# may-/joeys2t

Measured on AMD Instinct MI355X. Metric: audio frames/sec (train step, 80-mel, 15 s utt, bs32 per GPU), higher is better.
Workload: dtype bf16; 1 GPU; configs/librispeech_100h.yaml ASR train step on synthetic 16 kHz waveforms; global_batch=32, frames_per_utt=1498, encoder_len=375, lengths=fixed 15 s, vocab=5000, batch_multiplier=1, parallelism=dp1, launch=hipGraph replay

## Files before the change

include/joeys2t_hip.h:

```cpp
#ifndef JOEYS2T_HIP_H
#define JOEYS2T_HIP_H

#include <stdint.h>

#ifdef __cplusplus
extern "C" {
#endif

typedef void* js2t_stream;

enum { JS2T_F32 = 0, JS2T_BF16 = 1, JS2T_FP8_E4M3 = 2  };
enum { JS2T_ACT_NONE = 0, JS2T_ACT_RELU = 1, JS2T_ACT_GELU = 2, JS2T_ACT_SWISH = 3, JS2T_ACT_TANH = 4, JS2T_ACT_HARDSWISH = 5 };
enum { JS2T_OK = 0, JS2T_ERR_INVALID = -1, JS2T_ERR_LAUNCH = -2, JS2T_ERR_UNSUPPORTED = -3 };

int js2t_abi_version(void);
const char* js2t_last_error(void);

typedef struct js2t_gemm_desc {
  int32_t M, N, K;
  int32_t batch, batch_inner;
  int32_t dtype_ab, dtype_c;
  int32_t trans_a, trans_b;
  const void* A; int64_t lda, a_stride_o, a_stride_i;
  const void* B; int64_t ldb, b_stride_o, b_stride_i;
  void* C;       int64_t ldc, c_stride_o, c_stride_i;
  float alpha;
  const float* alpha_dev;
  const float* bias;
  int32_t act;
  void* preact;
  float dropout_p;
  const uint64_t* rng_state;
  uint32_t rng_stream;
  const void* residual;
  int64_t ldr;
  float res_scale;
  const void* gate;
  int64_t ldg;
  float gate_scale;
  float beta;
  int32_t conv, conv_tin, conv_tout, conv_c, conv_stride, conv_pad;
  int32_t split_k;
  float* a_rowsum;
  const float* ln_partial;
  float ln_eps;
  float* ln_mean;
  float* ln_rstd;
  float* rs_partial;
  uint8_t* c8;
  int64_t ldc8;
  float* c8_state;
  const float* c8_mul;
  float* c8_scale_out;
  float* fp8_state;
  const void* dot_src;
  int64_t ld_dot;
  float* dot_partial;
  float* sumsq_partial;
} js2t_gemm_desc;

int js2t_gemm(const js2t_gemm_desc* d, js2t_stream stream);
#define JS2T_GEMM_GROUP_MAX 32
int js2t_gemm_grouped(const js2t_gemm_desc* d, int32_t count, const void* const* A, const void* const* B, void* const* C,
                      float* const* a_rowsum, js2t_stream stream);
int64_t js2t_gemm_grouped_blocks(int32_t M, int32_t N, int32_t count);
void js2t_gemm_force_regstage(int on);
void js2t_gemm_force_w256(int on);
void js2t_gemm_p192_mode(int mode);
void js2t_gemm_wg256_mode(int mode);
void js2t_gemm_p192_ring(int nst);
void js2t_gemm_panel_mode(int mode);


int js2t_axpby(const void* x, float a, const void* y, float b, void* out, int64_t n, int dt, js2t_stream stream);

int js2t_cast(const void* src, int src_dt, void* dst, int dst_dt, int64_t n, js2t_stream stream);

int js2t_fold_ln_weights(const int64_t* table, int32_t n_entries, int32_t max_rows, js2t_stream stream);

int js2t_absmax(const void* x, int dt, int64_t n, float* out, js2t_stream stream);
int js2t_quantize_fp8(const void* x, int dt, void* y, int64_t n, const float* amax, const float* mul, float* scale_out,
                      js2t_stream stream);
int js2t_quantize_fp8_delayed(const void* x, int dt, void* y, int64_t n, float* state, const float* mul, float* scale_out,
                              js2t_stream stream);

int js2t_glu_fwd(const void* x, void* y, int64_t rows, int64_t C, int dt, js2t_stream stream);
int js2t_glu_bwd(const void* x, const void* dy, void* dx, int64_t rows, int64_t C, int dt, js2t_stream stream);
int js2t_glu_fwd_crop(const void* x, void* y, int64_t rows, int64_t C, int64_t T, const int64_t* valid_t, int dt, js2t_stream stream);
int js2t_glu_bwd_crop(const void* x, const void* dy, void* dx, int64_t rows, int64_t C, int64_t T, const int64_t* valid_t, int dt,
                      js2t_stream stream);

int js2t_transpose_groups(const void* src, void* dst, const int64_t* table, int32_t n_groups, int64_t total_tiles, js2t_stream stream);

int js2t_add_pe_dropout(const void* x, const float* pe, const void* extra, void* y, int64_t B, int64_t T,
                        int64_t D, int dt, float p, const uint64_t* rng_state, uint32_t rng_stream,
                        js2t_stream stream);

int js2t_dropout_bwd(const void* dy, void* dx, int64_t rows, int64_t cols, int dt, float p,
                     const uint64_t* rng_state, uint32_t rng_stream, js2t_stream stream);

int js2t_act_bwd(const void* dh, const void* z, void* dz, int64_t n, int act, int dt, float scale,
                 js2t_stream stream);

int js2t_embed_fwd(const int64_t* ids, const void* table, int table_dt, void* out, int out_dt,
                   int64_t n_ids, int64_t D, int64_t vocab, float scale, js2t_stream stream);
int js2t_embed_bwd(const int64_t* ids, const void* dout, int dout_dt, float* dtable, int64_t n_ids,
                   int64_t D, int64_t vocab, float scale, int64_t pad_idx, js2t_stream stream);

int64_t js2t_colsum_partial_rows(int64_t rows);
int js2t_colsum(const void* x, int dt, float* out, float* partial, int64_t rows, int64_t cols, int accumulate,
                js2t_stream stream);

int js2t_pack_rows(const void* src, void* dst, const int32_t* seg, int32_t B, int32_t T, int64_t rows_out, int64_t row_bytes,
                   int pack, js2t_stream stream);

int js2t_conv_weight_pack(const float* w, void* wp, int wp_dt, int64_t cout, int64_t cin, int64_t k,
                          js2t_stream stream);
int js2t_conv_weight_unpack_grad(const float* dwp_t, float* dw, int64_t cout, int64_t cin, int64_t k,
                                 int accumulate, js2t_stream stream);
int js2t_im2col(const void* x, void* col, int64_t B, int64_t tin, int64_t tout, int64_t C, int64_t K,
                int64_t stride, int64_t pad, int dt, js2t_stream stream);
int js2t_col2im(const void* dcol, void* dx, int64_t B, int64_t tin, int64_t tout, int64_t C, int64_t K,
                int64_t stride, int64_t pad, int dt, js2t_stream stream);

int js2t_subsample_lengths_mask(const int64_t* lengths, int64_t* out_lengths, uint8_t* mask, int64_t B,
                                int64_t T_out, const int32_t* kernel_sizes, int32_t n_layers,
                                js2t_stream stream);

int js2t_layernorm_fwd(const void* x, const float* gamma, const float* beta, void* y, float* mean,
                       float* rstd, int64_t rows, int64_t D, float eps, int dt, js2t_stream stream);
int js2t_layernorm_fwd_fp8(const void* x, const float* gamma, const float* beta, void* y, void* y8, float* q_state,
                           const float* q_mul, float* q_scale_out, float* mean, float* rstd, int64_t rows, int64_t D, float eps,
                           int dt, js2t_stream stream);
int js2t_layernorm_bwd(const void* dy, const void* x, const float* gamma, const float* mean,
                       const float* rstd, void* dx, const void* add, float add_scale, float* dgamma,
                       float* dbeta, float* partial, int accumulate, int64_t rows, int64_t D, int dt,
                       js2t_stream stream);
int js2t_layernorm_bwd_dropout(const void* dy, const void* x, const float* gamma, const float* mean,
                               const float* rstd, void* dx, const void* add, float add_scale, float* dgamma,
                               float* dbeta, float* partial, int accumulate, int64_t rows, int64_t D, int dt,
                               void* dx_dropped, float drop_p, const uint64_t* rng_state, uint32_t rng_stream,
                               int32_t acc_copies, int64_t acc_copy_stride, js2t_stream stream);
int js2t_layernorm_bwd_fused(const void* dy, const void* x, const float* gamma, const float* mean,
                             const float* rstd, void* dx, const void* add, float add_scale, float* dgamma,
                             float* dbeta, float* partial, int accumulate, int64_t rows, int64_t D, int dt,
                             void* dx_dropped, float drop_p, const uint64_t* rng_state, uint32_t rng_stream,
                             int32_t acc_copies, int64_t acc_copy_stride, const float* beta, void* n_out, js2t_stream stream);
int js2t_fold_copies(float* ws, const int64_t* table, int32_t n_entries, int32_t copies, int64_t copy_stride,
                     js2t_stream stream);

int js2t_softmax_fwd(const void* S, const uint8_t* mask, void* P, void* Pd, int64_t B, int64_t H,
                     int64_t Tq, int64_t Tk, int64_t ld, int64_t mask_sb, int64_t mask_sq, int dt,
                     float p, const uint64_t* rng_state, uint32_t rng_stream, js2t_stream stream);
int js2t_softmax_bwd(const void* P, const void* dPd, void* dS, int64_t Z, int64_t Tq, int64_t Tk,
                     int64_t ld, int dt, float p, const uint64_t* rng_state, uint32_t rng_stream,
                     js2t_stream stream);
int js2t_attn_head_mean(const void* P, float* out, int64_t B, int64_t H, int64_t Tq, int64_t Tk,
                        int64_t ld, int dt, js2t_stream stream);

int js2t_rel_bias_add(void* S, const float* rel_bias, int64_t B, int64_t H, int64_t Tq, int64_t Tk, int64_t ld, int32_t R,
                      int dt, js2t_stream stream);
int js2t_rel_bias_grad(const void* dS, float* d_rel_bias, int64_t B, int64_t H, int64_t Tq, int64_t Tk, int64_t ld, int32_t R,
                       int dt, js2t_stream stream);


int js2t_row_lse(const void* x, float* lse, int64_t* argmax, int64_t rows, int64_t V, int dt, js2t_stream stream);

int js2t_ctc_collapse(const int64_t* best, const int64_t* in_len, int64_t* out_ids, int64_t* out_len, int64_t B,
                      int64_t T, int64_t blank, int64_t pad, js2t_stream stream);
int js2t_log_softmax(const void* x, int dt, void* y, int y_dt, int64_t rows, int64_t V, js2t_stream stream);

int js2t_xent_fwd(const void* logits, int dt, const int64_t* trg, float* loss_rows, float* correct_rows,
                  float* lse, int64_t rows, int64_t V, int64_t pad_idx, float smoothing, js2t_stream stream);
int js2t_xent_bwd(const void* logits, int dt, const int64_t* trg, const float* lse, const float* g_dev,
                  float scale, void* dlogits, int64_t rows, int64_t V, int64_t pad_idx, float smoothing,
                  js2t_stream stream);
int js2t_xent_bwd_as(const void* logits, int dt, const int64_t* trg, const float* lse, const float* g_dev, float scale,
                     void* dlogits, int out_dt, int64_t rows, int64_t V, int64_t pad_idx, float smoothing, js2t_stream stream);

int js2t_train_stats(double* stats6, const float* total, const float* nll, const float* ctc, const int64_t* n_correct,
                     double inv_norm, double nseqs, double ntokens, float* norm_out, js2t_stream stream);

int js2t_sum_f32(const float* x, int64_t n, float* out, js2t_stream stream);

int js2t_ctc_alpha(const void* logits, int dt, const float* lse, const int64_t* targets, const int64_t* in_len,
                   const int64_t* tgt_len, float* alpha, float* beta, float* nll, float* loss_rows, int64_t B, int64_t T,
                   int64_t V, int64_t Lmax, int64_t blank, int zero_infinity, const int32_t* row_offsets, js2t_stream stream);
int js2t_ctc_bwd(const void* logits, int dt, const float* lse, const int64_t* targets, const int64_t* in_len,
                 const int64_t* tgt_len, const float* alpha, float* beta, const float* nll, const float* g_dev,
                 float scale, void* dlogits, int64_t B, int64_t T, int64_t V, int64_t Lmax, int64_t blank,
                 int zero_infinity, int beta_ready, const int32_t* row_offsets, int64_t packed_rows, js2t_stream stream);

int js2t_attn_decode(const void* q, int64_t ldq, const void* k, const void* v, int64_t ldkv, const int32_t* idx, int32_t idx_ld,
                     int32_t Tmax, int32_t len, const int32_t* len_dev, const uint8_t* key_mask, void* out, int64_t ldo, int32_t rows,
                     int32_t H, int32_t dh, float scale, int32_t group, int dt, js2t_stream stream);

int js2t_dwconv_outer_fwd(const void* x, const float* w, const float* bias, void* y, int64_t L, int64_t N, int64_t C, int K, int dt,
                          js2t_stream stream);
int js2t_dwconv_outer_bwd(const void* dy, const void* x, const float* w, void* dx, float* dw, int64_t L, int64_t N, int64_t C, int K,
                          int dt, js2t_stream stream);
int js2t_bn_act_fwd(const void* x, const float* gamma, const float* beta, float* running_mean, float* running_var, float* mean,
                    float* invstd, void* y, float* ws, int64_t rows, int64_t C, float eps, float momentum, int train, int act, int dt,
                    js2t_stream stream);
int js2t_bn_act_bwd(const void* dy, const void* x, const float* gamma, const float* beta, const float* mean, const float* invstd,
                    void* dx, float* dgamma, float* dbeta, float* ws, int64_t rows, int64_t C, int train, int act, int dt,
                    js2t_stream stream);


int js2t_fbank(const float* wave, const int64_t* sample_off, const int64_t* frame_off, int32_t U,
               int64_t total_frames, const float* window, const float* tw_re, const float* tw_im,
               const int32_t* mel_start, const int32_t* mel_len, const int32_t* mel_woff, const float* mel_w,
               float* out, int32_t win_len, int32_t shift, int32_t n_fft, int32_t n_mel, float scale, float preemph,
               float log_floor, js2t_stream stream);

int js2t_cmvn_stats(const float* feat, const int64_t* frame_off, int32_t U, int32_t F, float* mean, float* istd,
                    float* fill, int32_t norm_means, int32_t norm_vars, int64_t max_frames, js2t_stream stream);
int64_t js2t_cmvn_stats_workspace(int32_t U, int32_t F);
int js2t_cmvn_stats_ws(const float* feat, const int64_t* frame_off, int32_t U, int32_t F, float* mean, float* istd, float* fill,
                       int32_t norm_means, int32_t norm_vars, int64_t max_frames, double* workspace, js2t_stream stream);

int js2t_feature_finalize(const float* feat, const int64_t* frame_off, const float* mean, const float* istd,
                          const float* fill, const int32_t* masks, void* out, int out_dt, int64_t U, int64_t Tmax,
                          int32_t F, float pad_value, js2t_stream stream);
int js2t_feature_finalize_crop(const float* feat, const int64_t* frame_off, const float* mean, const float* istd,
                               const float* fill, const int32_t* masks, void* out, int out_dt, int64_t U, int64_t Tmax,
                               int32_t F, float pad_value, const int64_t* crop_t, js2t_stream stream);

int js2t_feature_transform(float* feat, const int64_t* frame_off, int32_t U, int32_t F, const float* mean, const float* istd,
                           const float* fill, const int32_t* masks, int32_t n_freq, int32_t n_time, js2t_stream stream);

typedef struct js2t_ctx_s* js2t_ctx;
enum {
  JS2T_CTX_DETERMINISTIC = 0,
  JS2T_CTX_GEMM_P192_MODE = 1,
  JS2T_CTX_GEMM_P192_RING = 2,
  JS2T_CTX_GEMM_WG256_MODE = 3,
  JS2T_CTX_GEMM_PANEL_MODE = 4,
  JS2T_CTX_NKEYS = 5
};
js2t_ctx js2t_ctx_create(void);
void js2t_ctx_destroy(js2t_ctx ctx);
int js2t_ctx_set(js2t_ctx ctx, int32_t key, int32_t value);
int js2t_ctx_get(js2t_ctx ctx, int32_t key);
js2t_ctx js2t_ctx_bind(js2t_ctx ctx);
int js2t_ctx_effective(int32_t key);
void js2t_set_deterministic(int on);
int js2t_get_deterministic(void);


int64_t js2t_sumsq_partials(int64_t n);
int js2t_grad_norm_clip(const float* g, int64_t n, float max_norm, float* partial, float* out2, js2t_stream stream);
int js2t_sumsq_ranges(const float* g, const int64_t* table, int32_t n_ranges, int64_t n_blocks, float* partial, js2t_stream stream);
int js2t_norm_clip(const float* partial, int64_t n_partial, float max_norm, float* out2, js2t_stream stream);

int js2t_adamw(float* p, float* g, float* exp_avg, float* exp_avg_sq, void* lp_bf16, int64_t n, float lr,
               float beta1, float beta2, float eps, float weight_decay, int64_t step, const float* gscale_dev,
               float gscale, int zero_grad, const float* lr_dev, const int64_t* step_dev, js2t_stream stream);

int js2t_adamw_items(float* p, float* g, float* exp_avg, float* exp_avg_sq, void* lp_bf16, void* lp_t_bf16,
                     const int64_t* items, int32_t n_items, int64_t n_units, const int64_t* folds, float lr, float beta1,
                     float beta2, float eps, float weight_decay, int64_t step, const float* gscale_dev, float gscale,
                     int zero_grad, const float* lr_dev, const int64_t* step_dev, js2t_stream stream);
void js2t_adamw_items_geometry(int32_t* flat_unit, int32_t* rows, int32_t* cols);

int js2t_beam_step(const float* logits, const float* beam_log_probs, float* out_scores, int64_t* out_ids,
                   float* out_lse, int64_t n_batch, int32_t beam, int64_t V, const int32_t* forbid_ids,
// ... 59 lines not shown
```

joeys2t_amd/builders.py:

```python
from typing import Callable

from torch import nn


class ConfigurationError(Exception):
    """Custom exception for misspecifications of configuration (reference config.py:22)."""


class _Tanh(nn.Module):
    def forward(self, x):
        raise RuntimeError("placeholder activation module: the HIP GEMM epilogue applies tanh")


_ACTIVATIONS = {"relu": nn.ReLU, "gelu": nn.GELU, "tanh": _Tanh, "swish": nn.SiLU}


def build_activation(activation: str = "relu") -> Callable:
    try:
        return _ACTIVATIONS[activation]
    except KeyError:
        raise ConfigurationError("Invalid activation function. Valid options: " + ", ".join(repr(k) for k in _ACTIVATIONS) + ".") from None


import ctypes as _C
# ... 23 lines not shown

def _off(t, lo: int):
    return None if t is None else _C.c_void_p(t.data_ptr() + lo * t.element_size())


import os as _os

FUSED_UPDATE = _os.environ.get("JS2T_FUSED_UPDATE", "1") != "0"


class SumsqCollector:

    def __init__(self, grad: torch.Tensor, total: int):
        from joeys2t_amd._lib import lib
        self.grad, self.total = grad, total
        self.per_block = int(total // max(1, lib().js2t_sumsq_partials(_C.c_int64(total)))) or 1
        cap = 2 * int(lib().js2t_sumsq_partials(_C.c_int64(total))) + 8192
        self.partial = torch.zeros((cap, ), dtype=torch.float32, device=grad.device)
        self.pos, self.covered = 0, []
        self._tables: Dict[tuple, tuple] = {}

    def reset(self):
        self.pos, self.covered = 0, []

    def segment(self, n_blocks: int, spans):
        if self.pos + n_blocks > self.partial.numel():
            raise RuntimeError("SumsqCollector: partial buffer exhausted")
        seg = self.partial[self.pos:self.pos + n_blocks]
        self.pos += n_blocks
        self.covered.extend(spans)
        return seg

    def finish(self, max_norm: float, out2: torch.Tensor):
        from joeys2t_amd import ops
        from joeys2t_amd._lib import check, lib
        from joeys2t_amd.runtime import RangeSet
        key = (self.pos, tuple(sorted(self.covered)))
        hit = self._tables.get(key)
        if hit is None:
            if torch.cuda.is_current_stream_capturing():
                raise RuntimeError("SumsqCollector: a new coverage pattern during capture - run one eager step first")
            rest = RangeSet([(0, self.total)]).minus(self.covered)
            rows, pb = [], self.pos
            for lo, hi in rest:
                rows.append([lo, hi - lo, pb])
                pb += int(lib().js2t_sumsq_partials(_C.c_int64(hi - lo)))
            if pb > self.partial.numel():
                raise RuntimeError("SumsqCollector: partial buffer exhausted")
            table = torch.tensor(rows, dtype=torch.int64, device=self.grad.device) if rows else None
            hit = self._tables[key] = (table, len(rows), pb - self.pos, pb)
        table, n_ranges, n_blocks, n_partial = hit
        if n_ranges:
            check(lib().js2t_sumsq_ranges(ops._p(self.grad), ops._p(table), _C.c_int32(n_ranges), _C.c_int64(n_blocks), ops._p(self.partial),
                                          ops._stream()), "js2t_sumsq_ranges")
        check(lib().js2t_norm_clip(ops._p(self.partial), _C.c_int64(n_partial), _C.c_float(max_norm), ops._p(out2), ops._stream()),
              "js2t_norm_clip")
        self.reset()


class FlatAdamW:

    def __init__(self, store, lr: float = 3e-4, betas=(0.9, 0.999), eps: float = 1e-8, weight_decay: float = 0.0):
        self.store = store
        self.param_groups = [{"lr": float(lr), "betas": tuple(betas), "eps": float(eps), "weight_decay": float(weight_decay)}]
        self.exp_avg = torch.zeros_like(store.flat)
        self.exp_avg_sq = torch.zeros_like(store.flat)
        self.t = 0
        self._retired_plans = []
        self.plan_generation = 0
        from joeys2t_amd._lib import lib
        n = store.total
        self._partial = torch.empty((max(1, lib().js2t_sumsq_partials(_C.c_int64(n))), ), dtype=torch.float32,
                                    device=store.device)
        self.norm_clip = torch.ones((2, ), dtype=torch.float32, device=store.device)
        self.lr_dev = torch.full((1, ), float(lr), dtype=torch.float32, device=store.device)
        self.step_dev = torch.zeros((1, ), dtype=torch.int64, device=store.device)
        self.device_schedule = False
        self.update_ranges = trainable_ranges(store)
        self._plan_key, self._plan = None, None
        self.keep = None
        self.collector: Optional[SumsqCollector] = None


    def clip_and_step(self, max_norm: Optional[float], grad_scale: float = 1.0, zero_grad: bool = True):
        from joeys2t_amd import ops
        from joeys2t_amd._lib import check, lib
        st, g = self.store, self.param_groups[0]
        coef = None
        if max_norm is not None and max_norm > 0:
            if self.collector is not None and self.collector.covered:
                self.collector.finish(max_norm, self.norm_clip)
            else:
                check(lib().js2t_grad_norm_clip(ops._p(st.flat_grad), _C.c_int64(st.total), _C.c_float(max_norm),
                                                ops._p(self._partial), ops._p(self.norm_clip), ops._stream()), "js2t_grad_norm_clip")
            coef = self.norm_clip[1:2]
        if self.collector is not None:
            self.collector.reset()
        self.t += 1
        lp = st.flat_lp
        lr_dev = step_dev = None
        if self.device_schedule:
            self.step_dev.add_(1)
            lr_dev, step_dev = self.lr_dev, self.step_dev
        plan = self._fused_plan()
        if plan is not None:
            args = (_C.c_float(g["lr"]), _C.c_float(g["betas"][0]), _C.c_float(g["betas"][1]), _C.c_float(g["eps"]),
                    _C.c_float(g["weight_decay"]), _C.c_int64(self.t), ops._p(coef), _C.c_float(grad_scale), int(zero_grad),
                    ops._p(lr_dev), ops._p(step_dev), ops._stream())
            for table, n_items, n_units in plan["launches"]:
                check(lib().js2t_adamw_items(ops._p(st.flat), ops._p(st.flat_grad), ops._p(self.exp_avg), ops._p(self.exp_avg_sq),
                                             ops._p(lp), ops._p(st.flat_lp_t if lp is not None else None), ops._p(table),
                                             _C.c_int32(n_items), _C.c_int64(n_units), ops._p(plan["folds"]), *args), "js2t_adamw_items")
            ops.WEIGHT_VERSION += 1
            st.dirty = lp is None and st.dirty
            if plan["left_folds"] is not None:
                ops.fold_ln_weights(plan["left_folds"], plan["left_folds"].shape[0], plan["left_max_rows"])
            return
        for lo, hi in self.update_ranges:
            check(lib().js2t_adamw(_off(st.flat, lo), _off(st.flat_grad, lo), _off(self.exp_avg, lo), _off(self.exp_avg_sq, lo),
                                   _off(lp, lo), _C.c_int64(hi - lo), _C.c_float(g["lr"]), _C.c_float(g["betas"][0]),
                                   _C.c_float(g["betas"][1]), _C.c_float(g["eps"]), _C.c_float(g["weight_decay"]), _C.c_int64(self.t),
                                   ops._p(coef), _C.c_float(grad_scale), int(zero_grad), ops._p(lr_dev), ops._p(step_dev),
                                   ops._stream()), "js2t_adamw")
        ops.WEIGHT_VERSION += 1
        st.dirty = lp is None and st.dirty
        if lp is not None and st.flat_lp_t is not None:
            st.refresh_t()
        if lp is not None:
            st.refresh_folds()

    def _fused_plan(self):
        st = self.store
        if not FUSED_UPDATE or self.update_ranges != [(0, st.total)]:
            return None
        key = (len(st._fold_rows), st.flat_lp is not None, st.flat_lp_t is not None, None if self.keep is None else self.keep.version)
        if self._plan_key == key:
            return self._plan
        if torch.cuda.is_current_stream_capturing():
            raise RuntimeError("FlatAdamW: the store changed (new LayerNorm folds / shadows) after the last eager update: "
                               "run one eager step before capturing")
        if self._plan is not None:
            self._retired_plans.append(self._plan)
            self.plan_generation += 1
        self._plan_key, self._plan = key, None
        from joeys2t_amd._lib import lib
        geo = [_C.c_int32() for _ in range(3)]
        lib().js2t_adamw_items_geometry(*[_C.byref(v) for v in geo])
        flat_unit, unit_rows, unit_cols = (int(v.value) for v in geo)
        mats = sorted((off, R, Cc) for off, R, Cc, _ in st._tgroups)
        if any(Cc % 4 or off % 4 for off, R, Cc in mats):
            return None
        base = st.flat.data_ptr()
        fold_of, left = {}, []
        for i, row in enumerate(st._fold_rows):
            hit = [(off, R, Cc) for off, R, Cc in mats if base + 4 * off == row[0] and R == row[6] and Cc == row[7]]
            if hit and row[7] <= unit_cols and hit[0][0] not in fold_of:
                fold_of[hit[0][0]] = i
            else:
                left.append(row)
        small, big, pos = [], [], 0
        for off, R, Cc in mats:
            if off > pos:
                small.append([0, pos, off - pos, 1, 0, -1, 0, 0])
            kept = int(self.keep is not None and self.keep.contains(off, off + R * Cc))
            big.append([1, off, R, Cc, 0, fold_of.get(off, -1), kept, 0])
            pos = off + R * Cc
        if st.total > pos:
            small.append([0, pos, st.total - pos, 1, 0, -1, 0, 0])
        launches = []
        for items in (small, big):
            if not items:
                continue
            units = 0
            for it in items:
                it[4] = units
                units += -(-it[2] // flat_unit) if it[0] == 0 else -(-it[2] // unit_rows) * -(-it[3] // unit_cols)
            launches.append((torch.tensor(items, dtype=torch.int64, device=st.device), len(items), units))
        folds = torch.tensor(st._fold_rows, dtype=torch.int64, device=st.device) if st._fold_rows else None
        self._plan = {"launches": launches, "folds": folds,
                      "left_folds": torch.tensor(left, dtype=torch.int64, device=st.device) if left else None,
                      "left_max_rows": max((r[6] for r in left), default=0)}
        return self._plan

    def state_dict(self) -> Dict:
        return {"t": self.t, "exp_avg": self.exp_avg, "exp_avg_sq": self.exp_avg_sq, "param_groups": self.param_groups}
# ... 73 lines not shown
```

joeys2t_amd/csrc/elementwise.hip:

```cpp
#include "common.hpp"

namespace {

constexpr int EW_THREADS = 256;
inline int ew_grid(int64_t work_items) {
  int64_t g = (work_items + EW_THREADS - 1) / EW_THREADS;
  if (g < 1) g = 1;
  if (g > 4096) g = 4096;
  return (int)g;
}

template <typename T> struct vec4;
template <> struct vec4<float> {
  static __device__ __forceinline__ void ld(const float* p, float (&v)[4]) {
    const float4 x = *(const float4*)p; v[0] = x.x; v[1] = x.y; v[2] = x.z; v[3] = x.w;
  }
  static __device__ __forceinline__ void st(float* p, const float (&v)[4]) {
    *(float4*)p = make_float4(v[0], v[1], v[2], v[3]);
  }
};
template <> struct vec4<uint16_t> {
  static __device__ __forceinline__ void ld(const uint16_t* p, float (&v)[4]) {
    const uint2 x = *(const uint2*)p;
    v[0] = __uint_as_float(x.x << 16); v[1] = __uint_as_float(x.x & 0xffff0000u);
    v[2] = __uint_as_float(x.y << 16); v[3] = __uint_as_float(x.y & 0xffff0000u);
  }
  static __device__ __forceinline__ void st(uint16_t* p, const float (&v)[4]) {
    uint2 x;
    x.x = pack_bf16x2(v[0], v[1]);
    x.y = pack_bf16x2(v[2], v[3]);
    *(uint2*)p = x;
  }
};

template <typename S, typename D>
__global__ void cast_kernel(const S* __restrict__ src, D* __restrict__ dst, int64_t n) {
  const int64_t n4 = n >> 2;
  for (int64_t i = blockIdx.x * (int64_t)blockDim.x + threadIdx.x; i < n4; i += (int64_t)gridDim.x * blockDim.x) {
    float v[4];
    vec4<S>::ld(src + 4 * i, v);
    vec4<D>::st(dst + 4 * i, v);
  }
  for (int64_t i = (n4 << 2) + blockIdx.x * (int64_t)blockDim.x + threadIdx.x; i < n; i += (int64_t)gridDim.x * blockDim.x)
    io<D>::st(dst + i, io<S>::ld(src + i));
}

template <typename T>
__global__ void axpby_kernel(const T* __restrict__ x, float a, const T* __restrict__ y, float b, T* __restrict__ out,
                             int64_t n) {
  for (int64_t i = blockIdx.x * (int64_t)blockDim.x + threadIdx.x; i < n; i += (int64_t)gridDim.x * blockDim.x) {
    float v = a * io<T>::ld(x + i);
    if (y) v += b * io<T>::ld(y + i);
    io<T>::st(out + i, v);
  }
}

template <typename T>
__global__ void glu_fwd_kernel(const T* __restrict__ x, T* __restrict__ y, int64_t rows, int64_t C, int64_t T_,
                               const int64_t* __restrict__ valid_t) {
  const int64_t total = rows * C, vt = valid_t ? *valid_t : T_;
  for (int64_t i = blockIdx.x * (int64_t)blockDim.x + threadIdx.x; i < total; i += (int64_t)gridDim.x * blockDim.x) {
    const int64_t r = i / C, c = i - r * C;
    const float a = io<T>::ld(x + r * 2 * C + c), b = io<T>::ld(x + r * 2 * C + C + c);
    io<T>::st(y + i, (r % T_) < vt ? a / (1.f + __expf(-b)) : 0.f);
  }
}
template <typename T>
__global__ void glu_bwd_kernel(const T* __restrict__ x, const T* __restrict__ dy, T* __restrict__ dx, int64_t rows,
                               int64_t C, int64_t T_, const int64_t* __restrict__ valid_t) {
  const int64_t total = rows * C, vt = valid_t ? *valid_t : T_;
  for (int64_t i = blockIdx.x * (int64_t)blockDim.x + threadIdx.x; i < total; i += (int64_t)gridDim.x * blockDim.x) {
    const int64_t r = i / C, c = i - r * C;
    const float a = io<T>::ld(x + r * 2 * C + c), b = io<T>::ld(x + r * 2 * C + C + c);
    const float g = (r % T_) < vt ? io<T>::ld(dy + i) : 0.f;
    const float s = 1.f / (1.f + __expf(-b));
    io<T>::st(dx + r * 2 * C + c, g * s);
    io<T>::st(dx + r * 2 * C + C + c, g * a * s * (1.f - s));
  }
}

template <typename T>
__global__ void add_pe_dropout_kernel(const T* __restrict__ x, const float* __restrict__ pe, const T* __restrict__ extra,
                                      T* __restrict__ y, int64_t B, int64_t T_, int64_t D, float p,
                                      const uint64_t* rng, uint32_t stream) {
  const int64_t D4 = D >> 2, total = B * T_ * D4;
  const float sc = p > 0.f ? 1.f / (1.f - p) : 1.f;
  const uint32_t dkey = p > 0.f ? dropout_key(rng, stream) : 0u;
  for (int64_t i = blockIdx.x * (int64_t)blockDim.x + threadIdx.x; i < total; i += (int64_t)gridDim.x * blockDim.x) {
    const int64_t row = i / D4, c4 = i - row * D4, t = row % T_;
    float v[4], e[4];
    vec4<T>::ld(x + row * D + 4 * c4, v);
    if (pe) {
      const float4 pv = *(const float4*)(pe + t * D + 4 * c4);
      v[0] += pv.x; v[1] += pv.y; v[2] += pv.z; v[3] += pv.w;
    }
    if (extra) {
      vec4<T>::ld(extra + row * D + 4 * c4, e);
#pragma unroll
      for (int k = 0; k < 4; ++k) v[k] += e[k];
    }
    if (p > 0.f) {
      const uint32_t keep = dropout_keep4_key(dkey, (uint32_t)row, (uint32_t)c4, p);
#pragma unroll
      for (int k = 0; k < 4; ++k) v[k] = ((keep >> k) & 1u) ? v[k] * sc : 0.f;
    }
    vec4<T>::st(y + row * D + 4 * c4, v);
  }
}

template <typename T>
__global__ void dropout_bwd_kernel(const T* __restrict__ dy, T* __restrict__ dx, int64_t rows, int64_t cols, float p,
                                   const uint64_t* rng, uint32_t stream) {
  const int64_t c4n = (cols + 3) >> 2, total = rows * c4n;
  const float sc = 1.f / (1.f - p);
  const uint32_t dkey = dropout_key(rng, stream);
  for (int64_t i = blockIdx.x * (int64_t)blockDim.x + threadIdx.x; i < total; i += (int64_t)gridDim.x * blockDim.x) {
    const int64_t row = i / c4n, c4 = i - row * c4n;
    const uint32_t keep = dropout_keep4_key(dkey, (uint32_t)row, (uint32_t)c4, p);
#pragma unroll
    for (int k = 0; k < 4; ++k) {
      const int64_t c = 4 * c4 + k;
      if (c < cols) {
        const float g = io<T>::ld(dy + row * cols + c);
        io<T>::st(dx + row * cols + c, ((keep >> k) & 1u) ? g * sc : 0.f);
      }
    }
  }
}

template <typename T>
__global__ void act_bwd_kernel(const T* __restrict__ dh, const T* __restrict__ z, T* __restrict__ dz, int64_t n, int act,
                               float scale) {
  for (int64_t i = blockIdx.x * (int64_t)blockDim.x + threadIdx.x; i < n; i += (int64_t)gridDim.x * blockDim.x)
    io<T>::st(dz + i, io<T>::ld(dh + i) * act_grad(io<T>::ld(z + i), act) * scale);
}

template <typename TT, typename TO>
__global__ void embed_fwd_kernel(const int64_t* __restrict__ ids, const TT* __restrict__ table, TO* __restrict__ out,
                                 int64_t n_ids, int64_t D, int64_t vocab, float scale) {
  const int64_t total = n_ids * D;
  for (int64_t i = blockIdx.x * (int64_t)blockDim.x + threadIdx.x; i < total; i += (int64_t)gridDim.x * blockDim.x) {
    const int64_t r = i / D, c = i - r * D;
    const int64_t id = ids[r];
    const float v = (id >= 0 && id < vocab) ? io<TT>::ld(table + id * D + c) * scale : 0.f;
    io<TO>::st(out + i, v);
  }
}
template <typename T>
__global__ void embed_bwd_kernel(const int64_t* __restrict__ ids, const T* __restrict__ dout, float* __restrict__ dtable,
                                 int64_t n_ids, int64_t D, int64_t vocab, float scale, int64_t pad_idx) {
  const int64_t total = n_ids * D;
  for (int64_t i = blockIdx.x * (int64_t)blockDim.x + threadIdx.x; i < total; i += (int64_t)gridDim.x * blockDim.x) {
    const int64_t r = i / D, c = i - r * D;
    const int64_t id = ids[r];
    if (id < 0 || id >= vocab || id == pad_idx) continue;
    atomicAdd(dtable + id * D + c, scale * io<T>::ld(dout + i));
  }
}

template <typename T>
__global__ __launch_bounds__(256) void embed_bwd_ordered_kernel(const int64_t* __restrict__ ids, const T* __restrict__ dout,
                                                                float* __restrict__ dtable, int64_t n_ids, int64_t D, int64_t vocab,
                                                                float scale, int64_t pad_idx) {
  __shared__ int earlier;
  const int64_t r = blockIdx.x, id = ids[r];
  if (id < 0 || id >= vocab || id == pad_idx) return;
  if (threadIdx.x == 0) earlier = 0;
  __syncthreads();
  for (int64_t q = threadIdx.x; q < r; q += blockDim.x)
    if (ids[q] == id) earlier = 1;
  __syncthreads();
  if (earlier) return;
  for (int64_t c = threadIdx.x; c < D; c += blockDim.x) {
    float acc = dtable[id * D + c];
    for (int64_t q = r; q < n_ids; ++q)
      if (ids[q] == id) acc += scale * io<T>::ld(dout + q * D + c);
    dtable[id * D + c] = acc;
  }
}

constexpr int CS_ROWS_PER_BLOCK = 64;
template <typename T>
__global__ __launch_bounds__(256) void colsum_partial_kernel(const T* __restrict__ x, float* __restrict__ partial, int64_t rows,
                                                             int64_t cols) {
  __shared__ float sh[4][64];
  const int cl = threadIdx.x & 63, sub = threadIdx.x >> 6;
  const int64_t c = (int64_t)blockIdx.x * 64 + cl;
  const int64_t r0 = (int64_t)blockIdx.y * CS_ROWS_PER_BLOCK, r1 = min(rows, r0 + CS_ROWS_PER_BLOCK);
  float s = 0.f;
  if (c < cols)
    for (int64_t r = r0 + sub; r < r1; r += 4) s += io<T>::ld(x + r * cols + c);
  sh[sub][cl] = s;
  __syncthreads();
  if (sub == 0 && c < cols) partial[(int64_t)blockIdx.y * cols + c] = (sh[0][cl] + sh[1][cl]) + (sh[2][cl] + sh[3][cl]);
}
__global__ __launch_bounds__(256) void colsum_partial_vec_kernel(const uint16_t* __restrict__ x, float* __restrict__ partial,
                                                                 int64_t rows, int64_t cols) {
  __shared__ float sh[4][64][9];
  const int cl = threadIdx.x & 63, sub = threadIdx.x >> 6;
  const int64_t c = ((int64_t)blockIdx.x * 64 + cl) * 8;
  const int64_t r0 = (int64_t)blockIdx.y * CS_ROWS_PER_BLOCK, r1 = min(rows, r0 + CS_ROWS_PER_BLOCK);
  float s[8] = {0.f, 0.f, 0.f, 0.f, 0.f, 0.f, 0.f, 0.f};
  if (c < cols)
    for (int64_t r = r0 + sub; r < r1; r += 4) {
      const uint4 v = *(const uint4*)(x + r * cols + c);
      const uint32_t vv[4] = {v.x, v.y, v.z, v.w};
#pragma unroll
      for (int i = 0; i < 4; ++i) {
        s[2 * i] += __uint_as_float(vv[i] << 16);
        s[2 * i + 1] += __uint_as_float(vv[i] & 0xffff0000u);
      }
    }
#pragma unroll
  for (int i = 0; i < 8; ++i) sh[sub][cl][i] = s[i];
  __syncthreads();
  if (sub == 0 && c < cols) {
#pragma unroll
    for (int i = 0; i < 8; ++i)
      partial[(int64_t)blockIdx.y * cols + c + i] = (sh[0][cl][i] + sh[1][cl][i]) + (sh[2][cl][i] + sh[3][cl][i]);
  }
}
__global__ __launch_bounds__(256) void colsum_final_kernel(const float* __restrict__ partial, float* __restrict__ out, int64_t nparts,
                                                           int64_t cols, int accumulate) {
  __shared__ float sh[4][64];
  const int cl = threadIdx.x & 63, sub = threadIdx.x >> 6;
  const int64_t c = (int64_t)blockIdx.x * 64 + cl;
  float s0 = 0.f, s1 = 0.f;
  if (c < cols) {
    int64_t p = sub;
    for (; p + 4 < nparts; p += 8) {
      s0 += partial[p * cols + c];
      s1 += partial[(p + 4) * cols + c];
    }
    for (; p < nparts; p += 4) s0 += partial[p * cols + c];
  }
  sh[sub][cl] = s0 + s1;
  __syncthreads();
  if (sub == 0 && c < cols) {
    const float tot = (sh[0][cl] + sh[1][cl]) + (sh[2][cl] + sh[3][cl]);
    out[c] = accumulate ? out[c] + tot : tot;
  }
}

template <typename D>
__global__ void conv_pack_kernel(const float* __restrict__ w, D* __restrict__ wp, int64_t cout, int64_t cin, int64_t k) {
  const int64_t total = cout * cin * k;
  for (int64_t i = blockIdx.x * (int64_t)blockDim.x + threadIdx.x; i < total; i += (int64_t)gridDim.x * blockDim.x) {
    const int64_t o = i / (k * cin), rem = i - o * k * cin, kw = rem / cin, c = rem - kw * cin;
    io<D>::st(wp + i, w[(o * cin + c) * k + kw]);
  }
}
__global__ void conv_unpack_grad_kernel(const float* __restrict__ dwp_t, float* __restrict__ dw, int64_t cout, int64_t cin,
                                        int64_t k, int accumulate) {
  const int64_t total = cout * cin * k;
  for (int64_t i = blockIdx.x * (int64_t)blockDim.x + threadIdx.x; i < total; i += (int64_t)gridDim.x * blockDim.x) {
    const int64_t o = i / (cin * k), rem = i - o * cin * k, c = rem / k, kw = rem - c * k;
    const float v = dwp_t[(kw * cin + c) * cout + o];
    dw[i] = accumulate ? dw[i] + v : v;
  }
// ... 85 lines not shown
    if (table[mid * 4 + 3] <= bid) lo = mid; else hi = mid - 1;
  }
  const int64_t off = table[lo * 4], R = table[lo * 4 + 1], Cc = table[lo * 4 + 2], t0 = table[lo * 4 + 3];
  const int64_t tiles_c = (Cc + 63) >> 6;
  const int64_t tr = (bid - t0) / tiles_c, tc = (bid - t0) - tr * tiles_c;
  if (((R | Cc | off) & 7) == 0 && ((((uintptr_t)src) | ((uintptr_t)dst)) & 15) == 0) {
#pragma unroll
    for (int k = 0; k < 2; ++k) {
      const int o = threadIdx.x + 256 * k, r = o >> 3, c8 = (o & 7) << 3;
      const int64_t rr = tr * 64 + r, cc = tc * 64 + c8;
      if (rr < R && cc < Cc) {
        const uint4 q = *(const uint4*)(src + off + rr * Cc + cc);
        uint32_t* d = (uint32_t*)&tile[r][c8];
        d[0] = q.x, d[1] = q.y, d[2] = q.z, d[3] = q.w;
      }
    }
    __syncthreads();
#pragma unroll
    for (int k = 0; k < 2; ++k) {
      const int o = threadIdx.x + 256 * k, c = o >> 3, r8 = (o & 7) << 3;
      const int64_t cc = tc * 64 + c, rr = tr * 64 + r8;
      if (rr < R && cc < Cc) {
        uint32_t w[4];
#pragma unroll
        for (int j = 0; j < 4; ++j) w[j] = (uint32_t)tile[r8 + 2 * j][c] | ((uint32_t)tile[r8 + 2 * j + 1][c] << 16);
        *(uint4*)(dst + off + cc * R + rr) = make_uint4(w[0], w[1], w[2], w[3]);
      }
    }
    return;
  }
  const int tx = threadIdx.x & 63, ty = threadIdx.x >> 6;
  for (int r = ty; r < 64; r += 4) {
    const int64_t rr = tr * 64 + r, cc = tc * 64 + tx;
    if (rr < R && cc < Cc) tile[r][tx] = src[off + rr * Cc + cc];
  }
  __syncthreads();
  for (int c = ty; c < 64; c += 4) {
    const int64_t cc = tc * 64 + c, rr = tr * 64 + tx;
    if (rr < R && cc < Cc) dst[off + cc * R + rr] = tile[tx][c];
  }
}

}

#define DISPATCH_DT(dt, T, ...)                                  \
  do {                                                           \
    if ((dt) == JS2T_F32) { typedef float T; __VA_ARGS__; }      \
    else if ((dt) == JS2T_BF16) { typedef uint16_t T; __VA_ARGS__; } \
    else { js2t_set_error("bad dtype %d", (int)(dt)); return JS2T_ERR_INVALID; } \
  } while (0)

extern "C" int js2t_cast(const void* src, int src_dt, void* dst, int dst_dt, int64_t n, js2t_stream stream) {
  if (n == 0) return JS2T_OK;
  JS2T_CHECK(src && dst && n > 0, "cast: bad arguments");
  hipStream_t s = (hipStream_t)stream;
  const int g = ew_grid(n / 4 + 1);
  DISPATCH_DT(src_dt, S, DISPATCH_DT(dst_dt, D, hipLaunchKernelGGL((cast_kernel<S, D>), dim3(g), dim3(EW_THREADS), 0, s,
                                                                    (const S*)src, (D*)dst, n)));
  JS2T_LAUNCH_CHECK();
  return JS2T_OK;
}

extern "C" int js2t_axpby(const void* x, float a, const void* y, float b, void* out, int64_t n, int dt, js2t_stream stream) {
  if (n == 0) return JS2T_OK;
  JS2T_CHECK(x && out && n > 0, "axpby: bad arguments");
  DISPATCH_DT(dt, T, hipLaunchKernelGGL((axpby_kernel<T>), dim3(ew_grid(n)), dim3(EW_THREADS), 0, (hipStream_t)stream,
                                        (const T*)x, a, (const T*)y, b, (T*)out, n));
  JS2T_LAUNCH_CHECK();
  return JS2T_OK;
}

extern "C" int js2t_glu_fwd_crop(const void* x, void* y, int64_t rows, int64_t C, int64_t T_, const int64_t* valid_t, int dt,
                                 js2t_stream stream) {
  if (rows * C == 0) return JS2T_OK;
  JS2T_CHECK(x && y && rows > 0 && C > 0 && T_ > 0 && rows % T_ == 0, "glu_fwd: bad arguments");
  DISPATCH_DT(dt, T, hipLaunchKernelGGL((glu_fwd_kernel<T>), dim3(ew_grid(rows * C)), dim3(EW_THREADS), 0,
                                        (hipStream_t)stream, (const T*)x, (T*)y, rows, C, T_, valid_t));
  JS2T_LAUNCH_CHECK();
  return JS2T_OK;
}
extern "C" int js2t_glu_fwd(const void* x, void* y, int64_t rows, int64_t C, int dt, js2t_stream stream) {
  return js2t_glu_fwd_crop(x, y, rows, C, rows > 0 ? rows : 1, nullptr, dt, stream);
}
extern "C" int js2t_glu_bwd_crop(const void* x, const void* dy, void* dx, int64_t rows, int64_t C, int64_t T_, const int64_t* valid_t,
                                 int dt, js2t_stream stream) {
  if (rows * C == 0) return JS2T_OK;
  JS2T_CHECK(x && dy && dx && rows > 0 && C > 0 && T_ > 0 && rows % T_ == 0, "glu_bwd: bad arguments");
  DISPATCH_DT(dt, T, hipLaunchKernelGGL((glu_bwd_kernel<T>), dim3(ew_grid(rows * C)), dim3(EW_THREADS), 0,
                                        (hipStream_t)stream, (const T*)x, (const T*)dy, (T*)dx, rows, C, T_, valid_t));
  JS2T_LAUNCH_CHECK();
  return JS2T_OK;
}
extern "C" int js2t_glu_bwd(const void* x, const void* dy, void* dx, int64_t rows, int64_t C, int dt, js2t_stream stream) {
  return js2t_glu_bwd_crop(x, dy, dx, rows, C, rows > 0 ? rows : 1, nullptr, dt, stream);
}

extern "C" int js2t_add_pe_dropout(const void* x, const float* pe, const void* extra, void* y, int64_t B, int64_t T_,
                                   int64_t D, int dt, float p, const uint64_t* rng_state, uint32_t rng_stream,
                                   js2t_stream stream) {
  if (B * T_ * D == 0) return JS2T_OK;
  JS2T_CHECK(x && y, "add_pe_dropout: null pointer");
  JS2T_CHECK(D % 4 == 0, "add_pe_dropout: D must be a multiple of 4 (got %lld)", (long long)D);
  JS2T_CHECK(p >= 0.f && p < 1.f && (p == 0.f || rng_state), "add_pe_dropout: bad dropout arguments");
  DISPATCH_DT(dt, T, hipLaunchKernelGGL((add_pe_dropout_kernel<T>), dim3(ew_grid(B * T_ * D / 4)), dim3(EW_THREADS), 0,
                                        (hipStream_t)stream, (const T*)x, pe, (const T*)extra, (T*)y, B, T_, D, p,
                                        rng_state, rng_stream));
  JS2T_LAUNCH_CHECK();
  return JS2T_OK;
}

extern "C" int js2t_dropout_bwd(const void* dy, void* dx, int64_t rows, int64_t cols, int dt, float p,
                                const uint64_t* rng_state, uint32_t rng_stream, js2t_stream stream) {
  if (rows * cols == 0) return JS2T_OK;
  JS2T_CHECK(dy && dx && rng_state && p > 0.f && p < 1.f, "dropout_bwd: bad arguments");
  DISPATCH_DT(dt, T, hipLaunchKernelGGL((dropout_bwd_kernel<T>), dim3(ew_grid(rows * ((cols + 3) / 4))), dim3(EW_THREADS),
                                        0, (hipStream_t)stream, (const T*)dy, (T*)dx, rows, cols, p, rng_state, rng_stream));
  JS2T_LAUNCH_CHECK();
  return JS2T_OK;
}

extern "C" int js2t_act_bwd(const void* dh, const void* z, void* dz, int64_t n, int act, int dt, float scale,
                            js2t_stream stream) {
  if (n == 0) return JS2T_OK;
  JS2T_CHECK(dh && z && dz && n > 0, "act_bwd: bad arguments");
  DISPATCH_DT(dt, T, hipLaunchKernelGGL((act_bwd_kernel<T>), dim3(ew_grid(n)), dim3(EW_THREADS), 0, (hipStream_t)stream,
                                        (const T*)dh, (const T*)z, (T*)dz, n, act, scale));
  JS2T_LAUNCH_CHECK();
  return JS2T_OK;
}

extern "C" int js2t_embed_fwd(const int64_t* ids, const void* table, int table_dt, void* out, int out_dt, int64_t n_ids,
                              int64_t D, int64_t vocab, float scale, js2t_stream stream) {
  if (n_ids * D == 0) return JS2T_OK;
  JS2T_CHECK(ids && table && out, "embed_fwd: null pointer");
  DISPATCH_DT(table_dt, TT, DISPATCH_DT(out_dt, TO, hipLaunchKernelGGL((embed_fwd_kernel<TT, TO>), dim3(ew_grid(n_ids * D)),
                                                                       dim3(EW_THREADS), 0, (hipStream_t)stream, ids,
                                                                       (const TT*)table, (TO*)out, n_ids, D, vocab, scale)));
  JS2T_LAUNCH_CHECK();
  return JS2T_OK;
}
extern "C" int js2t_embed_bwd(const int64_t* ids, const void* dout, int dout_dt, float* dtable, int64_t n_ids, int64_t D,
                              int64_t vocab, float scale, int64_t pad_idx, js2t_stream stream) {
  if (n_ids * D == 0) return JS2T_OK;
  JS2T_CHECK(ids && dout && dtable, "embed_bwd: null pointer");
  if (g_js2t_deterministic) {
    DISPATCH_DT(dout_dt, T, hipLaunchKernelGGL((embed_bwd_ordered_kernel<T>), dim3((unsigned)n_ids), dim3(256), 0, (hipStream_t)stream, ids,
                                               (const T*)dout, dtable, n_ids, D, vocab, scale, pad_idx));
    JS2T_LAUNCH_CHECK();
    return JS2T_OK;
  }
  DISPATCH_DT(dout_dt, T, hipLaunchKernelGGL((embed_bwd_kernel<T>), dim3(ew_grid(n_ids * D)), dim3(EW_THREADS), 0,
                                             (hipStream_t)stream, ids, (const T*)dout, dtable, n_ids, D, vocab, scale, pad_idx));
  JS2T_LAUNCH_CHECK();
  return JS2T_OK;
}

extern "C" int64_t js2t_colsum_partial_rows(int64_t rows) { return (rows + CS_ROWS_PER_BLOCK - 1) / CS_ROWS_PER_BLOCK; }

extern "C" int js2t_colsum(const void* x, int dt, float* out, float* partial, int64_t rows, int64_t cols, int accumulate,
                           js2t_stream stream) {
  if (cols == 0) return JS2T_OK;
  if (rows == 0) {
    JS2T_CHECK(out, "colsum: bad arguments");
    if (!accumulate) {
      hipError_t e = hipMemsetAsync(out, 0, sizeof(float) * cols, (hipStream_t)stream);
      JS2T_CHECK(e == hipSuccess, "colsum: memset failed: %s", hipGetErrorString(e));
    }
    return JS2T_OK;
  }
  JS2T_CHECK(x && out && partial && rows > 0, "colsum: bad arguments");
  const int64_t nparts = js2t_colsum_partial_rows(rows);
  JS2T_CHECK(nparts <= 65535, "colsum: too many rows");
  hipStream_t s = (hipStream_t)stream;
  if (dt == JS2T_BF16 && cols % 8 == 0 && (((uintptr_t)x) & 15) == 0) {
    hipLaunchKernelGGL(colsum_partial_vec_kernel, dim3(cdiv(cols, 512), (unsigned)nparts), dim3(256), 0, s, (const uint16_t*)x,
                       partial, rows, cols);
  } else {
    const dim3 g1(cdiv(cols, 64), (unsigned)nparts);
    DISPATCH_DT(dt, T, hipLaunchKernelGGL((colsum_partial_kernel<T>), g1, dim3(256), 0, s, (const T*)x, partial, rows, cols));
  }
  JS2T_LAUNCH_CHECK();
  hipLaunchKernelGGL(colsum_final_kernel, dim3(cdiv(cols, 64)), dim3(256), 0, s, partial, out, nparts, cols, accumulate);
  JS2T_LAUNCH_CHECK();
  return JS2T_OK;
}

extern "C" int js2t_conv_weight_pack(const float* w, void* wp, int wp_dt, int64_t cout, int64_t cin, int64_t k,
                                     js2t_stream stream) {
  JS2T_CHECK(w && wp && cout > 0 && cin > 0 && k > 0, "conv_weight_pack: bad arguments");
  DISPATCH_DT(wp_dt, D, hipLaunchKernelGGL((conv_pack_kernel<D>), dim3(ew_grid(cout * cin * k)), dim3(EW_THREADS), 0,
                                           (hipStream_t)stream, w, (D*)wp, cout, cin, k));
  JS2T_LAUNCH_CHECK();
  return JS2T_OK;
}
extern "C" int js2t_conv_weight_unpack_grad(const float* dwp_t, float* dw, int64_t cout, int64_t cin, int64_t k,
                                            int accumulate, js2t_stream stream) {
  JS2T_CHECK(dwp_t && dw && cout > 0 && cin > 0 && k > 0, "conv_weight_unpack_grad: bad arguments");
  hipLaunchKernelGGL(conv_unpack_grad_kernel, dim3(ew_grid(cout * cin * k)), dim3(EW_THREADS), 0, (hipStream_t)stream, dwp_t,
                     dw, cout, cin, k, accumulate);
  JS2T_LAUNCH_CHECK();
  return JS2T_OK;
}
extern "C" int js2t_col2im(const void* dcol, void* dx, int64_t B, int64_t tin, int64_t tout, int64_t C, int64_t K,
                           int64_t stride, int64_t pad, int dt, js2t_stream stream) {
  if (B * tin * C == 0) return JS2T_OK;
  JS2T_CHECK(dcol && dx && stride > 0 && K > 0, "col2im: bad arguments");
  if (dt == JS2T_BF16 && (C & 7) == 0 && ((((uintptr_t)dcol) | ((uintptr_t)dx)) & 15) == 0) {
    hipLaunchKernelGGL(col2im_vec_kernel, dim3(ew_grid(B * tin * (C >> 3))), dim3(EW_THREADS), 0, (hipStream_t)stream,
                       (const uint16_t*)dcol, (uint16_t*)dx, B, tin, tout, C, K, stride, pad);
    JS2T_LAUNCH_CHECK();
    return JS2T_OK;
  }
  DISPATCH_DT(dt, T, hipLaunchKernelGGL((col2im_kernel<T>), dim3(ew_grid(B * tin * C)), dim3(EW_THREADS), 0,
                                        (hipStream_t)stream, (const T*)dcol, (T*)dx, B, tin, tout, C, K, stride, pad));
  JS2T_LAUNCH_CHECK();
  return JS2T_OK;
}

extern "C" int js2t_im2col(const void* x, void* col, int64_t B, int64_t tin, int64_t tout, int64_t C, int64_t K, int64_t stride,
                           int64_t pad, int dt, js2t_stream stream) {
  if (B * tout * C * K == 0) return JS2T_OK;
  JS2T_CHECK(x && col && stride > 0 && K > 0 && tin > 0, "im2col: bad arguments");
  JS2T_CHECK(dt == JS2T_F32 || dt == JS2T_BF16, "im2col: bad dtype");
  const int vec = dt == JS2T_BF16 ? 8 : 4;
  JS2T_CHECK(C % vec == 0 && ((((uintptr_t)x) | ((uintptr_t)col)) & 15) == 0, "im2col: channels must fill 16-byte pieces, buffers 16-byte aligned");
  const int64_t work = B * tout * K * (C / vec);
  if (dt == JS2T_BF16)
    hipLaunchKernelGGL((im2col_kernel<uint16_t, 8>), dim3(ew_grid(work)), dim3(EW_THREADS), 0, (hipStream_t)stream, (const uint16_t*)x,
                       (uint16_t*)col, B, tin, tout, C, K, stride, pad);
  else
    hipLaunchKernelGGL((im2col_kernel<float, 4>), dim3(ew_grid(work)), dim3(EW_THREADS), 0, (hipStream_t)stream, (const float*)x,
                       (float*)col, B, tin, tout, C, K, stride, pad);
  JS2T_LAUNCH_CHECK();
  return JS2T_OK;
}

namespace {
// ... 239 lines not shown
```

joeys2t_amd/csrc/loss.hip:

```cpp
#include "common.hpp"

namespace {

constexpr int LB = 256;

__device__ __forceinline__ float logaddexp(float a, float b) {
  if (a == -INFINITY) return b;
  if (b == -INFINITY) return a;
  const float m = fmaxf(a, b);
  return m + log1pf(__expf(-fabsf(a - b)));
}

__device__ __forceinline__ float logaddexp_fast(float a, float b) {
  const float m = fmaxf(a, b);
  const float d = -fabsf(a - b);
  const float r = m + __logf(1.f + __expf(d));
  return (m == -INFINITY) ? -INFINITY : r;
}

template <typename T>
__global__ __launch_bounds__(LB) void row_lse_kernel(const T* __restrict__ x, float* __restrict__ lse,
                                                     int64_t* __restrict__ argmax, int64_t rows, int64_t V) {
  __shared__ float red[LB / 64];
  __shared__ int redi[LB / 64];
// ... 185 lines not shown
  sx = wave_sum(sx);
  int cand = (m == bmx) ? mi : 0x7fffffff;
#pragma unroll
  for (int o = 32; o > 0; o >>= 1) cand = min(cand, __shfl_xor(cand, o, 64));
  if (lane == 0) {
    const int64_t g = trg[r];
    const float lse = bmx + __logf(s);
    lse_out[r] = lse;
    float loss = 0.f, ok = 0.f;
    if (g != pad && g >= 0 && g < V) {
      const float lpg = xr[g] - lse;
      if (eps > 0.f) {
        const float u = eps / (float)(V - 2);
        const float lpp = (pad >= 0 && pad < V) ? xr[pad] - lse : 0.f;
        const float sum_lp = sx - (float)V * lse;
        const float cent = (1.f - eps) * __logf(1.f - eps) + eps * __logf(u);
        loss = cent - ((1.f - eps) * lpg + u * (sum_lp - lpg - lpp));
      } else {
        loss = -lpg;
      }
      ok = (cand == (int)g) ? 1.f : 0.f;
    }
    loss_rows[r] = loss;
    correct_rows[r] = ok;
  }
}
template <typename TO>
__global__ __launch_bounds__(256) void xent_bwd_flat_kernel(const float* __restrict__ x, const int64_t* __restrict__ trg,
                                                            const float* __restrict__ lse, const float* __restrict__ g_dev, float scale,
                                                            TO* __restrict__ dx, int rows, int n8, int64_t V, int64_t pad, float eps) {
  const int64_t chunk = (int64_t)blockIdx.x * 256 + threadIdx.x;
  if (chunk >= (int64_t)rows * n8) return;
  const int r = (int)(chunk / n8), c = (int)(chunk - (int64_t)r * n8);
  const int64_t g = trg[r];
  const bool dead = g == pad || g < 0 || g >= V;
  float o[8] = {0.f, 0.f, 0.f, 0.f, 0.f, 0.f, 0.f, 0.f};
  if (!dead) {
    const float4 qa = ((const float4*)x)[2 * chunk], qb = ((const float4*)x)[2 * chunk + 1];
    const float gs = scale * (g_dev ? *g_dev : 1.f), l = lse[r];
    const float u = eps > 0.f ? eps / (float)(V - 2) : 0.f, tg = eps > 0.f ? 1.f - eps : 1.f;
    const float f[8] = {qa.x, qa.y, qa.z, qa.w, qb.x, qb.y, qb.z, qb.w};
    const int gi = (int)g - 8 * c, pi = (pad >= 0 && pad < V) ? (int)pad - 8 * c : -1;
#pragma unroll
    for (int i = 0; i < 8; ++i) o[i] = gs * (__expf(f[i] - l) - (i == gi ? tg : (i == pi ? 0.f : u)));
  }
  if constexpr (sizeof(TO) == 4) {
    ((float4*)dx)[2 * chunk] = make_float4(o[0], o[1], o[2], o[3]);
    ((float4*)dx)[2 * chunk + 1] = make_float4(o[4], o[5], o[6], o[7]);
  } else {
    ((uint4*)dx)[chunk] = make_uint4(pack_bf16x2(o[0], o[1]), pack_bf16x2(o[2], o[3]), pack_bf16x2(o[4], o[5]), pack_bf16x2(o[6], o[7]));
  }
}

template <typename T, typename TO = T>
__global__ __launch_bounds__(LB) void xent_bwd_kernel(const T* __restrict__ x, const int64_t* __restrict__ trg,
                                                      const float* __restrict__ lse, const float* __restrict__ g_dev,
                                                      float scale, TO* __restrict__ dx, int64_t rows, int64_t V, int64_t pad,
                                                      float eps) {
  const int64_t r = blockIdx.x;
  const int64_t g = trg[r];
  const float gs = scale * (g_dev ? *g_dev : 1.f);
  const T* xr = x + r * V;
  TO* dr = dx + r * V;
  if (g == pad || g < 0 || g >= V) {
    for (int64_t v = threadIdx.x; v < V; v += LB) io<TO>::st(dr + v, 0.f);
    return;
  }
  const float l = lse[r];
  const float u = eps > 0.f ? eps / (float)(V - 2) : 0.f;
  const float tg = eps > 0.f ? 1.f - eps : 1.f;
  for (int64_t v = threadIdx.x; v < V; v += LB) {
    const float sm = __expf(io<T>::ld(xr + v) - l);
    const float t = (v == g) ? tg : ((v == pad) ? 0.f : u);
    io<TO>::st(dr + v, gs * (sm - t));
  }
}

__global__ __launch_bounds__(1024) void sum_f32_kernel(const float* __restrict__ x, int64_t n, float* __restrict__ out) {
  __shared__ float red[16];
  float s = 0.f;
  for (int64_t i = threadIdx.x; i < n; i += 1024) s += x[i];
  s = block_sum(s, red);
  if (threadIdx.x == 0) out[0] = s;
}

constexpr int CTC_THREADS = 256;
constexpr int CTC_MAX_S = 1024;
constexpr int CTC_CHUNK_FLOATS = 8192;

template <typename T, bool BACKWARD>
__device__ __forceinline__ void ctc_recursion_body(
    float (&a)[2][CTC_MAX_S + 2], int (&ext)[CTC_MAX_S], float (&em)[CTC_CHUNK_FLOATS],
    const T* __restrict__ x, const float* __restrict__ lse, const int64_t* __restrict__ targets,
    const int64_t* __restrict__ in_len, const int64_t* __restrict__ tgt_len, float* __restrict__ out ,
    float* __restrict__ nll, int64_t Tmax, int64_t V, int64_t Lmax, int64_t Smax, int64_t blank, const int32_t* __restrict__ rowoff) {
  const int b = blockIdx.x, tid = threadIdx.x;
  const int64_t Tb = min(in_len[b], Tmax);
  const int L = (int)min(tgt_len[b], Lmax);
  const int S = 2 * L + 1;
  const int64_t r0 = rowoff ? (int64_t)rowoff[b] : (int64_t)b * Tmax;
  for (int s = tid; s < S; s += CTC_THREADS) ext[s] = (s & 1) ? (int)targets[b * Lmax + (s >> 1)] : (int)blank;
  float* ob = out + (int64_t)b * Tmax * Smax;
  for (int64_t i = Tb * Smax + tid; i < Tmax * Smax; i += CTC_THREADS) ob[i] = -INFINITY;
  __syncthreads();
  if (Tb <= 0) {
    if (!BACKWARD && tid == 0) nll[b] = INFINITY;
    return;
  }
  const int chunk_T = max(1, min(64, CTC_CHUNK_FLOATS / S));
  int cur = 0;
  for (int64_t c0 = 0; c0 < Tb; c0 += chunk_T) {
    const int nt = (int)min((int64_t)chunk_T, Tb - c0);
    for (int i = tid; i < nt * S; i += CTC_THREADS) {
      const int tt = i / S, s = i - tt * S;
      const int64_t t = BACKWARD ? (Tb - 1 - (c0 + tt)) : (c0 + tt);
      const int lab = ext[s];
      const float v = (lab >= 0 && lab < V) ? io<T>::ld(x + (r0 + t) * V + lab) - lse[r0 + t] : -INFINITY;
      em[i] = v;
    }
    __syncthreads();
    for (int tt = 0; tt < nt; ++tt) {
      const int64_t step = c0 + tt;
      const int64_t t = BACKWARD ? (Tb - 1 - step) : step;
      const float* prev = a[cur ^ 1];
      float* now = a[cur];
      for (int s = tid; s < S; s += CTC_THREADS) {
        const float e = em[tt * S + s];
        float v;
        if (step == 0) {
          const bool start = BACKWARD ? (s >= S - 2) : (s < 2);
          v = start ? e : -INFINITY;
        } else if (!BACKWARD) {
          float acc = prev[s];
          if (s >= 1) acc = logaddexp(acc, prev[s - 1]);
          if (s >= 2 && ext[s] != (int)blank && ext[s] != ext[s - 2]) acc = logaddexp(acc, prev[s - 2]);
          v = acc + e;
        } else {
          float acc = prev[s];
          if (s + 1 < S) acc = logaddexp(acc, prev[s + 1]);
          if (s + 2 < S && ext[s + 2] != (int)blank && ext[s + 2] != ext[s]) acc = logaddexp(acc, prev[s + 2]);
          v = acc + e;
        }
        now[s] = v;
        ob[t * Smax + s] = v;
      }
      __syncthreads();
      cur ^= 1;
    }
  }
  if (!BACKWARD && tid == 0) {
    const float* last = a[cur ^ 1];
    float ll = last[S - 1];
    if (S > 1) ll = logaddexp(ll, last[S - 2]);
    nll[b] = -ll;
  }
}

template <typename T, bool BACKWARD>
__global__ __launch_bounds__(CTC_THREADS) void ctc_recursion_kernel(
    const T* __restrict__ x, const float* __restrict__ lse, const int64_t* __restrict__ targets,
    const int64_t* __restrict__ in_len, const int64_t* __restrict__ tgt_len, float* __restrict__ out, float* __restrict__ nll,
    int64_t Tmax, int64_t V, int64_t Lmax, int64_t Smax, int64_t blank, const int32_t* __restrict__ rowoff) {
  __shared__ float a[2][CTC_MAX_S + 2];
  __shared__ int ext[CTC_MAX_S];
  __shared__ float em[CTC_CHUNK_FLOATS];
  ctc_recursion_body<T, BACKWARD>(a, ext, em, x, lse, targets, in_len, tgt_len, out, nll, Tmax, V, Lmax, Smax, blank, rowoff);
// ... 272 lines not shown
  if (dt == JS2T_BF16 && (V & 7) == 0 && V <= 8 * LB * RL_CH && (((uintptr_t)x) & 15) == 0) {
    hipLaunchKernelGGL(row_lse_vec_kernel, dim3((unsigned)rows), dim3(LB), 0, (hipStream_t)stream, (const uint16_t*)x, lse, argmax, rows, V);
    JS2T_LAUNCH_CHECK();
    return JS2T_OK;
  }
  DISPATCH_DT(dt, T, hipLaunchKernelGGL((row_lse_kernel<T>), dim3((unsigned)rows), dim3(LB), 0, (hipStream_t)stream,
                                        (const T*)x, lse, argmax, rows, V));
  JS2T_LAUNCH_CHECK();
  return JS2T_OK;
}

extern "C" int js2t_ctc_collapse(const int64_t* best, const int64_t* in_len, int64_t* out_ids, int64_t* out_len, int64_t B, int64_t T,
                                 int64_t blank, int64_t pad, js2t_stream stream) {
  if (B == 0) return JS2T_OK;
  JS2T_CHECK(best && in_len && out_ids && out_len && B > 0 && T > 0, "ctc_collapse: bad arguments");
  hipLaunchKernelGGL(ctc_collapse_kernel, dim3((unsigned)B), dim3(64), 0, (hipStream_t)stream, best, in_len, out_ids, out_len, T, blank,
                     pad);
  JS2T_LAUNCH_CHECK();
  return JS2T_OK;
}

extern "C" int js2t_log_softmax(const void* x, int dt, void* y, int y_dt, int64_t rows, int64_t V, js2t_stream stream) {
  if (rows == 0) return JS2T_OK;
  JS2T_CHECK(x && y && rows > 0 && V > 0, "log_softmax: bad arguments");
  DISPATCH_DT(dt, T, DISPATCH_DT(y_dt, TO, hipLaunchKernelGGL((log_softmax_kernel<T, TO>), dim3((unsigned)rows), dim3(LB), 0,
                                                              (hipStream_t)stream, (const T*)x, (TO*)y, rows, V)));
  JS2T_LAUNCH_CHECK();
  return JS2T_OK;
}

extern "C" int js2t_xent_fwd(const void* logits, int dt, const int64_t* trg, float* loss_rows, float* correct_rows, float* lse,
                             int64_t rows, int64_t V, int64_t pad_idx, float smoothing, js2t_stream stream) {
  if (rows == 0) return JS2T_OK;
  JS2T_CHECK(logits && trg && loss_rows && correct_rows && lse && V > 2, "xent_fwd: bad arguments");
  if (dt == JS2T_F32 && (V & 3) == 0 && V < (int64_t(1) << 31) && (((uintptr_t)logits) & 15) == 0) {
    hipLaunchKernelGGL(xent_fwd_wave_kernel, dim3((unsigned)cdiv(rows, 4)), dim3(256), 0, (hipStream_t)stream, (const float*)logits, trg,
                       loss_rows, correct_rows, lse, rows, V, pad_idx, smoothing);
    JS2T_LAUNCH_CHECK();
    return JS2T_OK;
  }
  DISPATCH_DT(dt, T, hipLaunchKernelGGL((xent_fwd_kernel<T>), dim3((unsigned)rows), dim3(LB), 0, (hipStream_t)stream,
                                        (const T*)logits, trg, loss_rows, correct_rows, lse, rows, V, pad_idx, smoothing));
  JS2T_LAUNCH_CHECK();
  return JS2T_OK;
}

extern "C" int js2t_xent_bwd(const void* logits, int dt, const int64_t* trg, const float* lse, const float* g_dev, float scale,
                             void* dlogits, int64_t rows, int64_t V, int64_t pad_idx, float smoothing, js2t_stream stream) {
  if (rows == 0) return JS2T_OK;
  JS2T_CHECK(logits && trg && lse && dlogits && V > 2, "xent_bwd: bad arguments");
  if (dt == JS2T_F32 && (V & 7) == 0 && V < (int64_t(1) << 31) && rows < (int64_t(1) << 31) && rows * (V >> 3) < (int64_t(1) << 31) * 256 &&
      ((((uintptr_t)logits) | ((uintptr_t)dlogits)) & 15) == 0) {
    hipLaunchKernelGGL((xent_bwd_flat_kernel<float>), dim3((unsigned)cdiv(rows * (V >> 3), 256)), dim3(256), 0, (hipStream_t)stream,
                       (const float*)logits, trg, lse, g_dev, scale, (float*)dlogits, (int)rows, (int)(V >> 3), V, pad_idx, smoothing);
    JS2T_LAUNCH_CHECK();
    return JS2T_OK;
  }
  DISPATCH_DT(dt, T, hipLaunchKernelGGL((xent_bwd_kernel<T>), dim3((unsigned)rows), dim3(LB), 0, (hipStream_t)stream,
                                        (const T*)logits, trg, lse, g_dev, scale, (T*)dlogits, rows, V, pad_idx, smoothing));
  JS2T_LAUNCH_CHECK();
  return JS2T_OK;
}

extern "C" int js2t_xent_bwd_as(const void* logits, int dt, const int64_t* trg, const float* lse, const float* g_dev, float scale,
                                void* dlogits, int out_dt, int64_t rows, int64_t V, int64_t pad_idx, float smoothing, js2t_stream stream) {
  if (out_dt == dt) return js2t_xent_bwd(logits, dt, trg, lse, g_dev, scale, dlogits, rows, V, pad_idx, smoothing, stream);
  if (rows == 0) return JS2T_OK;
  JS2T_CHECK(logits && trg && lse && dlogits && V > 2, "xent_bwd_as: bad arguments");
  JS2T_CHECK(dt == JS2T_F32 && out_dt == JS2T_BF16, "xent_bwd_as: f32 logits -> bf16 gradient, or equal types");
  if ((V & 7) == 0 && V < (int64_t(1) << 31) && rows < (int64_t(1) << 31) && rows * (V >> 3) < (int64_t(1) << 31) * 256 &&
      ((((uintptr_t)logits) | ((uintptr_t)dlogits)) & 15) == 0) {
    hipLaunchKernelGGL((xent_bwd_flat_kernel<uint16_t>), dim3((unsigned)cdiv(rows * (V >> 3), 256)), dim3(256), 0, (hipStream_t)stream,
                       (const float*)logits, trg, lse, g_dev, scale, (uint16_t*)dlogits, (int)rows, (int)(V >> 3), V, pad_idx, smoothing);
    JS2T_LAUNCH_CHECK();
    return JS2T_OK;
  }
  hipLaunchKernelGGL((xent_bwd_kernel<float, uint16_t>), dim3((unsigned)rows), dim3(LB), 0, (hipStream_t)stream, (const float*)logits, trg,
                     lse, g_dev, scale, (uint16_t*)dlogits, rows, V, pad_idx, smoothing);
  JS2T_LAUNCH_CHECK();
  return JS2T_OK;
}

__global__ void train_stats_kernel(double* __restrict__ stats, const float* total, const float* nll, const float* ctc,
                                   const int64_t* n_correct, double inv_norm, double nseqs, double ntokens, float* norm_out) {
  if (threadIdx.x != 0 || blockIdx.x != 0) return;
  const double t = (double)total[0] * inv_norm;
  stats[0] += t;
  if (nll) stats[1] += (double)nll[0] * inv_norm;
  if (ctc) stats[2] += (double)ctc[0] * inv_norm;
  if (n_correct) stats[3] += (double)n_correct[0];
  stats[4] += nseqs;
  stats[5] += ntokens;
  if (norm_out) norm_out[0] = (float)t;
}
extern "C" int js2t_train_stats(double* stats6, const float* total, const float* nll, const float* ctc, const int64_t* n_correct,
                                double inv_norm, double nseqs, double ntokens, float* norm_out, js2t_stream stream) {
  JS2T_CHECK(stats6 && total, "train_stats: null pointer");
  hipLaunchKernelGGL(train_stats_kernel, dim3(1), dim3(64), 0, (hipStream_t)stream, stats6, total, nll, ctc, n_correct, inv_norm, nseqs,
                     ntokens, norm_out);
  JS2T_LAUNCH_CHECK();
  return JS2T_OK;
}

extern "C" int js2t_sum_f32(const float* x, int64_t n, float* out, js2t_stream stream) {
  JS2T_CHECK(x && out && n >= 0, "sum_f32: bad arguments");
  hipLaunchKernelGGL(sum_f32_kernel, dim3(1), dim3(1024), 0, (hipStream_t)stream, x, n, out);
  JS2T_LAUNCH_CHECK();
  return JS2T_OK;
}

extern "C" int js2t_ctc_alpha(const void* logits, int dt, const float* lse, const int64_t* targets, const int64_t* in_len,
                              const int64_t* tgt_len, float* alpha, float* beta, float* nll, float* loss_rows, int64_t B,
                              int64_t T_, int64_t V, int64_t Lmax, int64_t blank, int zero_infinity, const int32_t* row_offsets,
                              js2t_stream stream) {
  if (B == 0) return JS2T_OK;
  JS2T_CHECK(logits && lse && targets && in_len && tgt_len && alpha && nll && loss_rows, "ctc_alpha: null pointer");
  JS2T_CHECK(2 * Lmax + 1 <= CTC_MAX_S, "ctc_alpha: target length %lld exceeds %d", (long long)Lmax, (CTC_MAX_S - 1) / 2);
  const int64_t Smax = 2 * Lmax + 1;
  hipStream_t s = (hipStream_t)stream;
  if (Smax <= CTCW_S) {
    DISPATCH_DT(dt, T, hipLaunchKernelGGL((ctc_wave_kernel<T>), dim3((unsigned)B, beta ? 2 : 1), dim3(256), 0, s, (const T*)logits, lse,
                                          targets, in_len, tgt_len, alpha, beta, nll, T_, V, Lmax, Smax, blank, row_offsets));
  } else if (beta) {
    DISPATCH_DT(dt, T, hipLaunchKernelGGL((ctc_both_kernel<T>), dim3((unsigned)B, 2), dim3(CTC_THREADS), 0, s, (const T*)logits, lse,
                                          targets, in_len, tgt_len, alpha, beta, nll, T_, V, Lmax, Smax, blank, row_offsets));
  } else {
    DISPATCH_DT(dt, T, hipLaunchKernelGGL((ctc_recursion_kernel<T, false>), dim3((unsigned)B), dim3(CTC_THREADS), 0, s,
                                          (const T*)logits, lse, targets, in_len, tgt_len, alpha, nll, T_, V, Lmax, Smax, blank, row_offsets));
  }
  JS2T_LAUNCH_CHECK();
  hipLaunchKernelGGL(ctc_loss_rows_kernel, dim3(cdiv(B, 256)), dim3(256), 0, s, nll, loss_rows, B, zero_infinity);
  JS2T_LAUNCH_CHECK();
  return JS2T_OK;
}

extern "C" int js2t_ctc_bwd(const void* logits, int dt, const float* lse, const int64_t* targets, const int64_t* in_len,
                            const int64_t* tgt_len, const float* alpha, float* beta, const float* nll, const float* g_dev,
                            float scale, void* dlogits, int64_t B, int64_t T_, int64_t V, int64_t Lmax, int64_t blank,
                            int zero_infinity, int beta_ready, const int32_t* row_offsets, int64_t packed_rows, js2t_stream stream) {
  if (B == 0) return JS2T_OK;
  JS2T_CHECK(logits && lse && targets && in_len && tgt_len && alpha && beta && nll && dlogits, "ctc_bwd: null pointer");
  JS2T_CHECK(2 * Lmax + 1 <= CTC_MAX_S, "ctc_bwd: target length %lld exceeds %d", (long long)Lmax, (CTC_MAX_S - 1) / 2);
  JS2T_CHECK(V * 4 <= 160 * 1024 - 10 * 1024, "ctc_bwd: vocabulary %lld too large for the LDS-staged gradient row", (long long)V);
  const int64_t Smax = 2 * Lmax + 1;
  hipStream_t s = (hipStream_t)stream;
  if (!beta_ready) {
    DISPATCH_DT(dt, T, hipLaunchKernelGGL((ctc_recursion_kernel<T, true>), dim3((unsigned)B), dim3(CTC_THREADS), 0, s,
                                          (const T*)logits, lse, targets, in_len, tgt_len, beta, (float*)nullptr, T_, V, Lmax,
                                          Smax, blank, row_offsets));
    JS2T_LAUNCH_CHECK();
  }
  const size_t lds = (size_t)V * sizeof(float);
  if (dt == JS2T_F32) {
    if (lds > 48 * 1024) hipFuncSetAttribute((const void*)ctc_grad_kernel<float>, hipFuncAttributeMaxDynamicSharedMemorySize, (int)lds);
    hipLaunchKernelGGL((ctc_grad_kernel<float>), dim3((unsigned)(B * T_)), dim3(LB), lds, s, (const float*)logits, lse, alpha,
                       beta, nll, targets, in_len, tgt_len, g_dev, scale, (float*)dlogits, T_, V, Lmax, Smax, blank,
                       zero_infinity, g_js2t_deterministic, row_offsets, packed_rows);
  } else {
    if (lds > 48 * 1024) hipFuncSetAttribute((const void*)ctc_grad_kernel<uint16_t>, hipFuncAttributeMaxDynamicSharedMemorySize, (int)lds);
    hipLaunchKernelGGL((ctc_grad_kernel<uint16_t>), dim3((unsigned)(B * T_)), dim3(LB), lds, s, (const uint16_t*)logits, lse,
                       alpha, beta, nll, targets, in_len, tgt_len, g_dev, scale, (uint16_t*)dlogits, T_, V, Lmax, Smax, blank,
                       zero_infinity, g_js2t_deterministic, row_offsets, packed_rows);
  }
  JS2T_LAUNCH_CHECK();
  return JS2T_OK;
}
```

joeys2t_amd/decoders.py:

```python
from typing import Optional

import torch
from torch import Tensor, nn

from joeys2t_amd import functional as Fn
from joeys2t_amd.helpers import freeze_params, subsequent_mask
from joeys2t_amd.runtime import runtime_of
from joeys2t_amd.transformer_layers import PositionalEncoding, TransformerDecoderLayer


class Decoder(nn.Module):

    @property
    def output_size(self):
        return self._output_size


PACK_MEMORY = True


class TransformerDecoder(Decoder):
    def __init__(self, num_layers: int = 4, num_heads: int = 8, hidden_size: int = 512, ff_size: int = 2048,
                 dropout: float = 0.1, emb_dropout: float = 0.1, vocab_size: int = 1, freeze: bool = False, **kwargs):
        super().__init__()
        self._hidden_size = hidden_size
        self._output_size = vocab_size
        self.layers = nn.ModuleList([
            TransformerDecoderLayer(size=hidden_size, ff_size=ff_size, num_heads=num_heads, dropout=dropout,
                                    alpha=kwargs.get("alpha", 1.0), layer_norm=kwargs.get("layer_norm", "post"),
                                    activation=kwargs.get("activation", "relu")) for _ in range(num_layers)
        ])
        self.pe = PositionalEncoding(hidden_size)
        self.layer_norm = nn.LayerNorm(hidden_size, eps=1e-6) if kwargs.get("layer_norm", "post") == "pre" else None
        self.emb_dropout = nn.Dropout(p=emb_dropout)
        self.output_layer = nn.Linear(hidden_size, vocab_size, bias=False)
        if freeze:
            freeze_params(self)
        self.ctc_output_layer = None
        encoder_output_size = kwargs.get("encoder_output_size_for_ctc", None)
        if encoder_output_size is not None:
            self.ctc_output_layer = nn.Linear(encoder_output_size, vocab_size, bias=False)

    def _cross_kv_params(self):
        atts = [layer.src_trg_att for layer in self.layers]
        return ([p for a in atts for p in (a.k_layer.weight, a.v_layer.weight)],
                [p for a in atts for p in (a.k_layer.bias, a.v_layer.bias)])

    def fuse_groups(self):
        return list(self._cross_kv_params())

    def memory_kv(self, memory: Tensor) -> Optional[Tensor]:
        rt = runtime_of(self)
        if not Fn.GROUP_MEMORY_KV or len(self.layers) < 2 or rt.store is None or memory.dim() != 3:
            return None
        ws, bs = self._cross_kv_params()
        if any(b is None for b in bs):
            return None
        w, b = rt.store.view(ws, rt.compute_dtype), rt.store.view(bs, torch.float32)
        if w is None or b is None:
            return None
        memory = rt.act_in(memory)
        need_grad = torch.is_grad_enabled() and (memory.requires_grad or any(p.requires_grad for p in ws + bs))
        if need_grad and not Fn.chain_active():
            return None
        wts = {"w_kv": w, "b_kv": b, "w_kv_t": rt.weight_t(ws), "sink": rt.sinks({"w_kv": ws, "b_kv": bs}), "notify": rt.grads_ready}
        return Fn.MemoryKVFn.apply(memory, wts, *ws, *bs)

    def project(self, layer: nn.Linear, x: Tensor, out_dtype) -> Tensor:
        rt = runtime_of(self)
        x = rt.act_in(x)
        bias = None if layer.bias is None else layer.bias
        smap = {"w": [layer.weight]}
        if bias is not None:
            smap["b"] = [bias]
        sk = rt.sinks(smap)
        if sk is not None:
            sk["_w_t"] = rt.weight_t([layer.weight])
        return Fn.LinearFn.apply(x, rt.weight([layer.weight]), layer.weight, bias, out_dtype, sk, rt.grads_ready)

    def forward(self, trg_embed: Tensor, encoder_output: Tensor, encoder_hidden: Tensor, src_mask: Tensor,
                unroll_steps: int, hidden: Tensor, trg_mask: Tensor, **kwargs):
        assert trg_mask is not None, "trg_mask required for Transformer"
        rt = runtime_of(self)
        x = self.pe(trg_embed, extra=kwargs.get("trg_prompt_mask", None), dropout=self.emb_dropout.p,
                    training=self.training)
        L = trg_embed.size(1)
        trg_mask = (trg_mask & subsequent_mask(L, device=trg_mask.device)).contiguous()
        last_layer = len(self.layers) - 1
        return_attention = kwargs.get("return_attention", False)
        att = None
        mem_pack = kwargs.get("memory_pack")
        kv_all = None
        if (mem_pack is not None and not return_attention and Fn.USE_FLASH and rt.compute_dtype == torch.bfloat16 and PACK_MEMORY and
                encoder_output.dim() == 3 and (mem_pack.B, mem_pack.T) == tuple(encoder_output.shape[:2]) and
                (self._hidden_size // self.layers[0].src_trg_att.num_heads) in (64, 128)):
            kv_all = self.memory_kv(Fn.PackRowsFn.apply(rt.act_in(encoder_output), mem_pack))
        if kv_all is None:
            mem_pack = None
            kv_all = self.memory_kv(encoder_output)
        d2 = 2 * self._hidden_size
        for i, layer in enumerate(self.layers):
            x, att = layer(x=x, memory=encoder_output, src_mask=src_mask, trg_mask=trg_mask,
                           return_attention=(return_attention and i == last_layer),
                           memory_kv=None if kv_all is None else (kv_all, i * d2), mem_pack=mem_pack)
        if self.layer_norm is not None:
            sk = rt.sinks({"g": [self.layer_norm.weight], "b": [self.layer_norm.bias]})
            x = Fn.LayerNormFn.apply(x, self.layer_norm.weight, self.layer_norm.bias, None if sk is None else (sk["g"], sk["b"], sk.get("_copies")),
                                     rt.grads_ready)
        out = self.project(self.output_layer, x[:, -1:].contiguous() if kwargs.get("last_only", False) else x, torch.float32)
        ctc_output = None
        if self.ctc_output_layer is not None and kwargs.get("compute_ctc", True):
            ctc_pack = kwargs.get("ctc_pack")
            ctc_in = encoder_output if ctc_pack is None else Fn.PackRowsFn.apply(rt.act_in(encoder_output), ctc_pack)
            ctc_output = self.project(self.ctc_output_layer, ctc_in, rt.compute_dtype)
        return out, x, att, None, ctc_output

    def __repr__(self):
        return (f"{self.__class__.__name__}(num_layers={len(self.layers)}, "
                f"num_heads={self.layers[0].trg_trg_att.num_heads}, alpha={self.layers[0].alpha}, "
                f'layer_norm="{self.layers[0]._layer_norm_position}", ctc_layer={self.ctc_output_layer is not None})')
```

joeys2t_amd/encoders.py:

```python
import os
from typing import List, Tuple

import torch
from torch import Tensor, nn

from joeys2t_amd import functional as Fn
from joeys2t_amd import ops
from joeys2t_amd.helpers import freeze_params, lengths_to_padding_mask, pad
from joeys2t_amd.runtime import runtime_of
from joeys2t_amd.transformer_layers import ConformerEncoderLayer, PositionalEncoding, TransformerEncoderLayer


PACK_RAGGED = os.environ.get("JS2T_PACKED_ENCODER", "1") != "0"
PACK_MIN_SAVING = 0.04
PACK_ROUND = 64
_PACK_CACHE: dict = {}


class Encoder(nn.Module):

    @property
    def output_size(self):
        return self._output_size


class Conv1dSubsampler(nn.Module):

    def __init__(self, in_channels: int, mid_channels: int, out_channels: int = None, kernel_sizes: List[int] = (3, 3)):
        super().__init__()
        self.kernel_sizes = list(kernel_sizes)
        self.n_layers = len(self.kernel_sizes)
        self.conv_layers = nn.ModuleList(
            nn.Conv1d(in_channels if i == 0 else mid_channels // 2,
                      mid_channels if i < self.n_layers - 1 else out_channels * 2, k, stride=2, padding=k // 2)
            for i, k in enumerate(self.kernel_sizes))

    def get_out_seq_lens_tensor(self, in_seq_lens_tensor: Tensor) -> Tensor:
        out = in_seq_lens_tensor.long()
        for k in self.kernel_sizes:
            out = torch.div(out + 2 * (k // 2) - k, 2, rounding_mode="floor") + 1
        return out

    def out_len(self, t_in: int) -> int:
        for k in self.kernel_sizes:
            t_in = Fn.conv_out_len(t_in, k)
        return t_in

    def forward(self, src_tokens: Tensor, src_lengths: Tensor, crop: Tensor = None) -> Tuple[Tensor, Tensor, Tensor]:
        rt = runtime_of(self)
        if not src_lengths.is_cuda:
            max_len = int(src_lengths.max())
            assert max_len > 0, "empty batch!"
            if src_tokens.size(1) != max_len:
                src_tokens = src_tokens[:, :max_len, :]
            src_lengths = src_lengths.to(src_tokens.device)
        x = rt.act_in(src_tokens.contiguous())
        for i, conv in enumerate(self.conv_layers):
            valid = crop[i:i + 1] if (crop is not None and i + 1 < self.n_layers) else None
            x = Fn.Conv1dGluFn.apply(x, conv.weight, conv.bias, rt.compute_dtype,
                                     rt.sinks({"w": [conv.weight], "b": [conv.bias]}), rt.grads_ready, valid)
        out_lens, mask = ops.subsample_lengths_mask(src_lengths, x.size(1), self.kernel_sizes)
        mask.js2t_row_sums = out_lens
        return x, out_lens, mask


class TransformerEncoder(Encoder):

    def __init__(self, hidden_size: int = 512, ff_size: int = 2048, num_layers: int = 8, num_heads: int = 4,
                 dropout: float = 0.1, emb_dropout: float = 0.1, freeze: bool = False, **kwargs):
        super().__init__()
        self._output_size = hidden_size
        self.layers = nn.ModuleList([
            TransformerEncoderLayer(size=hidden_size, ff_size=ff_size, num_heads=num_heads, dropout=dropout,
                                    alpha=kwargs.get("alpha", 1.0), layer_norm=kwargs.get("layer_norm", "pre"),
                                    activation=kwargs.get("activation", "relu")) for _ in range(num_layers)
        ])
        self.pe = PositionalEncoding(hidden_size)
        self.emb_dropout = nn.Dropout(p=emb_dropout)
        self.layer_norm = nn.LayerNorm(hidden_size, eps=1e-6) if kwargs.get("layer_norm", "post") == "pre" else None
        if freeze:
            freeze_params(self)
        self.subsample = kwargs.get("subsample", False)
        if self.subsample:
            self.subsampler = Conv1dSubsampler(kwargs["in_channels"], kwargs["conv_channels"], hidden_size,
                                               kwargs.get("conv_kernel_sizes", [3, 3]))
            self.pad_index = kwargs.get("pad_index", 1)
            assert self.pad_index is not None

    def forward(self, src_embed: Tensor, src_length: Tensor, mask: Tensor = None, **kwargs):
        if self.subsample:
            src_embed, src_length, ss_mask = self.subsampler(src_embed, src_length, kwargs.get("src_crop", None))
            if mask is None:
                mask = ss_mask
        if mask is None:
            mask = lengths_to_padding_mask(src_length, src_embed.size(1)).unsqueeze(1)
        x = self.pe(src_embed, extra=kwargs.get("src_prompt_mask", None), dropout=self.emb_dropout.p,
                    training=self.training)
        pack = self._packing(x, mask, kwargs)
        self.last_pack = pack
        if pack is not None:
            x = Fn.PackRowsFn.apply(x, pack)
        for layer in self.layers:
            x = layer(x, mask) if pack is None else layer(x, mask, pack=pack)
        if self.layer_norm is not None:
            rt = runtime_of(self)
            sk = rt.sinks({"g": [self.layer_norm.weight], "b": [self.layer_norm.bias]})
            x = Fn.LayerNormFn.apply(x, self.layer_norm.weight, self.layer_norm.bias, None if sk is None else (sk["g"], sk["b"], sk.get("_copies")),
                                     rt.grads_ready)
        if pack is not None:
            x = Fn.UnpackRowsFn.apply(x, pack)
        if kwargs.get("repad", False) and "src_max_len" in kwargs and self.subsample:
            x, mask = self._repad(x, mask, kwargs["src_max_len"])
        assert src_length.size() == (x.size(0), ), (src_length.size(), x.size())
        assert mask.size() == (x.size(0), 1, x.size(1)), (mask.size(), x.size())
        return x, None, mask

    def _packing(self, x: Tensor, mask: Tensor, kwargs):
        if not (PACK_RAGGED and self.subsample and type(self) is TransformerEncoder and x.is_cuda and x.dtype == torch.bfloat16 and Fn.USE_FLASH):
            return None
        B, T, d = x.shape
        dh = d // self.layers[0].src_src_att.num_heads
        if dh not in (64, 128) or (d * 2) % 16 or mask is None or tuple(mask.shape) != (B, 1, T):
            return None
        pack = kwargs.get("src_pack", None)
        if pack is None:
            host = kwargs.get("src_length_host", None)
            if host is None or len(host) != B:
                return None
            lens = [min(self.subsampler.out_len(int(n)), T) for n in host]
            if sum(lens) > (1.0 - PACK_MIN_SAVING) * B * T:
                return None
            key = (tuple(lens), T, str(x.device))
            pack = _PACK_CACHE.get(key)
            if pack is None:
                if torch.cuda.is_current_stream_capturing():
                    return None
                pack = ops.PackedRows.from_lengths(lens, T, x.device, round_to=PACK_ROUND)
                if len(_PACK_CACHE) >= 16:
                    _PACK_CACHE.pop(next(iter(_PACK_CACHE)))
                _PACK_CACHE[key] = pack
        if pack.B != B or pack.T != T:
            raise ops.Js2tError(f"packed encoder: {pack.B} x {pack.T} prepared for a [{B}, {T}, {d}] batch")
        return pack

    def _repad(self, x, mask, src_max_len):
        src_max_len = self.subsampler.out_len(int(src_max_len))
        return pad(x, src_max_len, pad_index=self.pad_index, dim=1), pad(mask, src_max_len, pad_index=self.pad_index, dim=-1)

    def __repr__(self):
        return (f"{self.__class__.__name__}(num_layers={len(self.layers)}, "
                f"num_heads={self.layers[0].src_src_att.num_heads}, alpha={self.layers[0].alpha}, "
                f'layer_norm="{self.layers[0]._layer_norm_position}", subsample={self.subsample})')


class ConformerEncoder(TransformerEncoder):

    def __init__(self, hidden_size: int = 512, ff_size: int = 2048, num_layers: int = 8, num_heads: int = 4, dropout: float = 0.1,
                 emb_dropout: float = 0.1, freeze: bool = False, **kwargs):
        super().__init__()
        self._output_size = hidden_size
        self.layers = nn.ModuleList([
            ConformerEncoderLayer(size=hidden_size, ff_size=ff_size, num_heads=num_heads, dropout=dropout,
                                  alpha=kwargs.get("alpha", 1.0), layer_norm=kwargs.get("layer_norm", "pre"),
                                  depthwise_conv_kernel_size=kwargs.get("depthwise_conv_kernel_size", 31),
                                  rel_pos_clip=kwargs.get("rel_pos_clip")) for _ in range(num_layers)
        ])
        self.pe = PositionalEncoding(hidden_size)
        self.emb_dropout = nn.Dropout(p=emb_dropout)
        self.linear = nn.Linear(hidden_size, hidden_size)
        if freeze:
            freeze_params(self)
        self.subsampler = Conv1dSubsampler(kwargs["in_channels"], kwargs["conv_channels"], hidden_size,
                                           kwargs.get("conv_kernel_sizes", [3, 3]))
        self.pad_index = kwargs.get("pad_index", 1)
        assert self.pad_index is not None

    def forward(self, src_embed: Tensor, src_length: Tensor, mask: Tensor = None, **kwargs):
        rt = runtime_of(self)
        x, src_length, mask = self.subsampler(src_embed, src_length)
        x = self.pe(x)
# ... 13 lines not shown
```

joeys2t_amd/functional.py:

```python
import math
from typing import List, Optional

import os

import torch

from joeys2t_amd import ops
from joeys2t_amd.ops import DropoutRng

LN_EPS = 1e-6


def _row_major_2d(t: torch.Tensor) -> torch.Tensor:
    if t.dim() != 2 or t.stride(1) != 1:
        raise ops.Js2tError(f"expected a row-major 2-D tensor, got shape {tuple(t.shape)} strides {t.stride()}")
    return t


FP8_FORWARD = os.environ.get("JS2T_FP8_FORWARD", "0") == "1"
FP8_SEPARATE_PASS = os.environ.get("JS2T_FP8_SEPARATE_PASS", "0") == "1"
_FP8_WEIGHTS = {}
_FP8_STATES = {}
FP8_DELAYED = os.environ.get("JS2T_FP8_DELAYED", "1") != "0"

# ... 674 lines not shown
    @staticmethod
    def backward(ctx, dy):
        x2, gamma, mean, rstd = ctx.saved_tensors
        dy2 = dy.reshape(x2.shape)
        if not dy2.is_contiguous():
            dy2 = dy2.contiguous()
        sink = ctx.sink
        dx, dg, db = ops.layernorm_bwd(dy2, x2, gamma, mean, rstd, grad_out=None if sink is None else sink[:2],
                                       copies=sink[2] if sink is not None and len(sink) > 2 else None)
        if ctx.sink is not None:
            if ctx.notify is not None:
                ctx.notify(ctx.leaves)
            dg = db = None
        return dx.view(ctx.shape), dg, db, None, None


class CutFn(torch.autograd.Function):

    @staticmethod
    def forward(ctx, x):
        return x.view_as(x)

    @staticmethod
    def backward(ctx, dy):
        return dy


class LinearFn(torch.autograd.Function):

    @staticmethod
    def forward(ctx, x, w_compute, weight, bias, out_dtype, sink=None, notify=None):
        shape = x.shape
        x2 = x.reshape(-1, shape[-1])
        y = linear_fwd(x2, w_compute, bias, out_dtype=out_dtype)
        ctx.x2, ctx.w = x2, w_compute
        ctx.has_bias = bias is not None
        ctx.shape = shape
        ctx.sink, ctx.notify, ctx.leaves = sink, notify, (weight, bias)
        if y.dtype != x2.dtype and any(ctx.needs_input_grad):
            if len(LOGIT_GRAD_DTYPE) > 16:
                LOGIT_GRAD_DTYPE.clear()
            LOGIT_GRAD_DTYPE[y.data_ptr()] = x2.dtype
            ctx.y_ptr = y.data_ptr()
        return y.view(*shape[:-1], w_compute.shape[0])

    @staticmethod
    def backward(ctx, dy):
        x2, w = ctx.x2, ctx.w
        ready = LOGIT_GRAD_READY.pop(ctx.y_ptr, None) if getattr(ctx, "y_ptr", None) is not None else None
        if ready is not None:
            d_lp, ph = ready
            is_placeholder = dy.data_ptr() == ph.data_ptr() and dy.shape == ph.shape and all(st == 0 for st in dy.stride())
            if is_placeholder and d_lp.dtype == x2.dtype:
                dy = d_lp.view(dy.shape)
            else:
                raise ops.Js2tError("LinearFn.backward: the loss handed its logit gradient over in the projection's compute type, but autograd "
                                    "delivered a different tensor - the logits have another consumer or a copy sits between projection and loss")
        dy2 = dy.reshape(-1, dy.shape[-1])
        if not dy2.is_contiguous():
            dy2 = dy2.contiguous()
        if dy2.dtype != x2.dtype:
            dy2 = ops.cast(dy2, x2.dtype)
        sink = ctx.sink or {}
        dx, dw, db = linear_bwd(dy2, x2, w, need_dx=ctx.needs_input_grad[0], need_dw=ctx.needs_input_grad[2],
                                need_db=ctx.has_bias and ctx.needs_input_grad[3], dw_out=sink.get("w"), db_out=sink.get("b"),
                                queue=sink.get("_wq"), w_t=sink.get("_w_t"))
        if sink and ctx.notify is not None:
            ctx.notify(ctx.leaves)
        return (None if dx is None else dx.view(ctx.shape)), None, dw, db, None, None, None


class AddPeDropoutFn(torch.autograd.Function):

    @staticmethod
    def forward(ctx, x, pe, extra, p, rng):
        site = rng.next_site() if (rng is not None and p > 0) else 0
        y = ops.add_pe_dropout(x.contiguous(), pe, None if extra is None else extra.contiguous(), p, rng, site)
        ctx.p, ctx.rng, ctx.site = p, rng, site
        ctx.has_extra = extra is not None
        return y

    @staticmethod
    def backward(ctx, dy):
        dx = ops.dropout_bwd(dy, ctx.p, ctx.rng, ctx.site) if ctx.p > 0 else dy
        return dx, None, (dx if ctx.has_extra else None), None, None


class EmbedFn(torch.autograd.Function):

    @staticmethod
    def forward(ctx, ids, table, scale, pad_idx, out_dtype, sink=None, notify=None):
        ctx.ids, ctx.scale, ctx.pad_idx, ctx.vocab = ids, scale, pad_idx, table.shape[0]
        ctx.sink, ctx.notify, ctx.leaf = sink, notify, table
        return ops.embed_fwd(ids, table, scale, out_dtype)

    @staticmethod
    def backward(ctx, dout):
        dt = ops.embed_bwd(ctx.ids, dout, ctx.vocab, ctx.scale, ctx.pad_idx, out=ctx.sink)
        if ctx.sink is not None:
            if ctx.notify is not None:
                ctx.notify((ctx.leaf, ))
            dt = None
        return None, dt, None, None, None, None, None


class AxpbyFn(torch.autograd.Function):

    @staticmethod
    def forward(ctx, x, a, y, b):
        ctx.ab = (a, b)
        return ops.axpby(x.contiguous(), a, y.contiguous(), b)

    @staticmethod
    def backward(ctx, g):
        a, b = ctx.ab
        g = g.contiguous()

        def part(c, wanted):
            return None if not wanted else (g if c == 1.0 else ops.axpby(g, c))

        return part(a, ctx.needs_input_grad[0]), None, part(b, ctx.needs_input_grad[2]), None


class ConvModuleFn(torch.autograd.Function):

    @staticmethod
    def forward(ctx, x, w1, b1, wd, bd, gamma, beta, running_mean, running_var, w2, b2, p, rng, training, compute_dtype,
                w1_lp=None, w2_lp=None, sink=None, notify=None):
        B, T, Cc = x.shape
        x2 = x.reshape(B * T, Cc)
        if x2.dtype != compute_dtype:
            x2 = ops.cast(x2, compute_dtype)
        w1c = w1.reshape(w1.shape[0], Cc)
        w2c = w2.reshape(w2.shape[0], -1)
        if compute_dtype != torch.float32:
            w1c = w1_lp.reshape(w1.shape[0], Cc) if w1_lp is not None else ops.cast(w1c, compute_dtype)
            w2c = w2_lp.reshape(w2.shape[0], -1) if w2_lp is not None else ops.cast(w2c, compute_dtype)
        h = linear_fwd(x2, w1c, b1)
        u = ops.glu_fwd(h)
        wd2 = wd.reshape(wd.shape[0], wd.shape[-1]).contiguous()
        v = ops.dwconv_outer_fwd(u.view(B, T, -1), wd2, bd)
        v2 = v.view(B * T, -1)
        z, mean, invstd = ops.bn_act_fwd(v2, gamma, beta, running_mean, running_var, 1e-5, 0.1, training, "hardswish")
        site = rng.next_site() if (training and p > 0) else 0
        y = linear_fwd(z, w2c, b2, dropout_p=p if training else 0.0, rng=rng, site=site)
        ctx.saved = (x2, w1c, h, u, wd2, v2, gamma, beta, mean, invstd, z, w2c)
        ctx.cfg = (B, T, Cc, p if training else 0.0, rng, site, training, x.dtype)
        ctx.sink, ctx.notify, ctx.leaves = sink, notify, (w1, b1, w2, b2)
        return y.view(B, T, -1).to(x.dtype) if y.dtype != x.dtype else y.view(B, T, -1)

    @staticmethod
    def backward(ctx, dy):
        x2, w1c, h, u, wd2, v2, gamma, beta, mean, invstd, z, w2c = ctx.saved
        B, T, Cc, p, rng, site, training, in_dtype = ctx.cfg
        dy2 = dy.reshape(B * T, -1)
        if dy2.dtype != z.dtype:
            dy2 = ops.cast(dy2.contiguous(), z.dtype)
        if not dy2.is_contiguous():
            dy2 = dy2.contiguous()
        if p > 0:
            dy2 = ops.dropout_bwd(dy2, p, rng, site)
        sink = ctx.sink or {}

        def sv(name, like):
            t = sink.get(name)
            return None if t is None else t.view(like.shape)

        dz, dw2, db2 = linear_bwd(dy2, z, w2c, dw_out=sv("w2", w2c), db_out=sink.get("b2"), queue=sink.get("_wq"))
        dv, dgamma, dbeta = ops.bn_act_bwd(dz, v2, gamma, beta, mean, invstd, training, "hardswish")
        du, dwd = ops.dwconv_outer_bwd(dv.view(B, T, -1), u.view(B, T, -1), wd2)
        dbd = ops.colsum(dv)
        dh = ops.glu_bwd(h, du.view(B * T, -1))
        dx, dw1, db1 = linear_bwd(dh, x2, w1c, dw_out=sv("w1", w1c), db_out=sink.get("b1"), queue=sink.get("_wq"))
        if sink and ctx.notify is not None:
            ctx.notify(ctx.leaves)
        dx = dx.view(B, T, Cc)
        if dx.dtype != in_dtype:
            dx = dx.to(in_dtype)
        return (dx, None if dw1 is None else dw1.view(dw1.shape[0], Cc, 1), db1, dwd.view(dwd.shape[0], 1, -1), dbd, dgamma, dbeta, None, None,
                None if dw2 is None else dw2.view(dw2.shape[0], -1, 1), db2, None, None, None, None, None, None, None, None)


def conv_out_len(t_in: int, k: int, stride: int = 2) -> int:
    return (t_in + 2 * (k // 2) - (k - 1) - 1) // stride + 1


class Conv1dGluFn(torch.autograd.Function):

    @staticmethod
    def forward(ctx, x, weight, bias, compute_dtype, sink=None, notify=None, valid_t=None):
        ctx.sink, ctx.notify, ctx.leaves = sink, notify, (weight, bias)
        ctx.valid_t = valid_t
        B, T, Cin = x.shape
        Cout, _, K = weight.shape
        stride, pad = 2, K // 2
        Tout = conv_out_len(T, K, stride)
        x = x.contiguous()
        wp = ops.conv_weight_pack(weight, compute_dtype)
        M = B * Tout
        pre = torch.empty((M, Cout), dtype=compute_dtype, device=x.device)
        conv = (T, Tout, Cin, stride, pad)
        vec = 8 if x.dtype == torch.bfloat16 else 4
        if Cin % vec == 0:
            col = ops.im2col(x, K, stride, pad, Tout)
            ops.gemm(col, wp, pre, M=M, N=Cout, K=K * Cin, lda=K * Cin, ldb=K * Cin, ldc=Cout, bias=bias)
        else:
            col = None
            ops.gemm(x, wp, pre, M=M, N=Cout, K=K * Cin, lda=stride * Cin, ldb=K * Cin, ldc=Cout, bias=bias, conv=conv)
        y = ops.glu_fwd(pre, Tout, valid_t)
        ctx.x, ctx.wp, ctx.pre, ctx.conv, ctx.col = (x if col is None else None), wp, pre, conv, col
        ctx.dims = (B, T, Cin, Cout, K, Tout)
        return y.view(B, Tout, Cout // 2)

    @staticmethod
    def backward(ctx, dy):
        B, T, Cin, Cout, K, Tout = ctx.dims
        M = B * Tout
        x, wp, pre, conv = ctx.x, ctx.wp, ctx.pre, ctx.conv
        dy2 = dy.reshape(M, Cout // 2)
        if not dy2.is_contiguous():
            dy2 = dy2.contiguous()
        dpre = ops.glu_bwd(pre, dy2, Tout, ctx.valid_t)
        sink = ctx.sink or {}
        db = ops.colsum(dpre, out=sink.get("b"), accumulate=True) if sink else ops.colsum(dpre)
        sk = wgrad_split(K * Cin, Cout, M)
        dwp_t = (torch.zeros if sk > 1 else torch.empty)((K * Cin, Cout), dtype=torch.float32, device=dpre.device)
        if ctx.col is not None:
            ops.gemm(ctx.col, dpre, dwp_t, M=K * Cin, N=Cout, K=M, lda=K * Cin, ldb=Cout, ldc=Cout, trans_a=True, trans_b=True, split_k=sk)
        else:
            ops.gemm(x, dpre, dwp_t, M=K * Cin, N=Cout, K=M, lda=conv[3] * Cin, ldb=Cout, ldc=Cout, trans_a=True, trans_b=True,
                     conv=conv, split_k=sk)
        dw = ops.conv_weight_unpack_grad(dwp_t, Cout, Cin, K, out=sink.get("w"))
        if sink:
            if ctx.notify is not None:
                ctx.notify(ctx.leaves)
            dw = db = None
        dx = None
        if ctx.needs_input_grad[0]:
            dcol = torch.empty((M, K * Cin), dtype=pre.dtype, device=pre.device)
            ops.gemm(dpre, wp, dcol, M=M, N=K * Cin, K=Cout, lda=Cout, ldb=K * Cin, ldc=K * Cin, trans_b=True)
            dx = ops.col2im(dcol, B, T, Tout, Cin, K, conv[3], conv[4])
        return dx, dw, db, None, None, None, None
```

joeys2t_amd/loss.py:

```python
from typing import Tuple

import torch
from torch import Tensor, nn

from joeys2t_amd import ops


_NAN = {}


class _XentFn(torch.autograd.Function):
    @staticmethod
    def forward(ctx, logits, trg, pad_index, smoothing):
        V = logits.shape[-1]
        l2 = logits.reshape(-1, V)
        if not l2.is_contiguous():
            l2 = l2.contiguous()
        t1 = trg.reshape(-1).contiguous()
        loss_rows, correct_rows, lse = ops.xent_fwd(l2, t1, pad_index, smoothing)
        ctx.l2, ctx.t1, ctx.lse = l2, t1, lse
        ctx.pad_index, ctx.smoothing, ctx.shape = pad_index, smoothing, logits.shape
        loss = ops.sum_f32(loss_rows)
        n_correct = ops.sum_f32(correct_rows)
        ctx.mark_non_differentiable(n_correct)
        return loss, n_correct

    @staticmethod
    def backward(ctx, g, _g2):
        g = g.contiguous().float()
        from joeys2t_amd import functional as Fn
        want = Fn.LOGIT_GRAD_DTYPE.pop(ctx.l2.data_ptr(), None)
        if want is not None and want != ctx.l2.dtype and ctx.l2.dtype == torch.float32:
            d = ops.xent_bwd(ctx.l2, ctx.t1, ctx.lse, g, 1.0, ctx.pad_index, ctx.smoothing, out_dtype=want)
            nan = _NAN.get(ctx.l2.device)
            if nan is None:
                nan = _NAN[ctx.l2.device] = torch.full((), float("nan"), dtype=ctx.l2.dtype, device=ctx.l2.device)
            ph = nan.expand(ctx.shape)
            if len(Fn.LOGIT_GRAD_READY) > 16:
                Fn.LOGIT_GRAD_READY.clear()
            Fn.LOGIT_GRAD_READY[ctx.l2.data_ptr()] = (d, ph)
            return ph, None, None, None
        d = ops.xent_bwd(ctx.l2, ctx.t1, ctx.lse, g, 1.0, ctx.pad_index, ctx.smoothing)
        return d.view(ctx.shape), None, None, None


class _CtcFn(torch.autograd.Function):

    @staticmethod
    def forward(ctx, logits, targets, in_len, tgt_len, blank, zero_infinity, pack=None):
        ctx.pack, ctx.shape = pack, tuple(logits.shape)
        if pack is None:
            B, T, V = logits.shape
            l3 = logits.contiguous()
        else:
            V = logits.shape[-1]
            B, T = pack.B, pack.T
            l3 = logits.reshape(-1, V).contiguous()
        from joeys2t_amd import functional as Fn
        Fn.LOGIT_GRAD_DTYPE.pop(logits.data_ptr(), None)
        targets = targets.contiguous()
        in_len = in_len.to(torch.int64).contiguous()
        tgt_len = tgt_len.to(torch.int64).contiguous()
        lse, _ = ops.row_lse(l3.view(-1, V))
        alpha, nll, loss_rows, beta = ops.ctc_alpha(l3, lse, targets, in_len, tgt_len, blank, zero_infinity,
                                                    with_beta=logits.requires_grad, pack=pack)
        ctx.saved = (l3, lse, targets, in_len, tgt_len, alpha, nll, beta)
        ctx.blank, ctx.zero_infinity = blank, zero_infinity
        return ops.sum_f32(loss_rows)

    @staticmethod
    def backward(ctx, g):
        l3, lse, targets, in_len, tgt_len, alpha, nll, beta = ctx.saved
        g = g.contiguous().float()
        d = ops.ctc_bwd(l3, lse, targets, in_len, tgt_len, alpha, nll, g, 1.0, ctx.blank, ctx.zero_infinity, beta=beta, pack=ctx.pack)
        return d.view(ctx.shape), None, None, None, None, None, None


class XentLoss(nn.Module):

    def __init__(self, pad_index: int, smoothing: float = 0.0):
        super().__init__()
        self.smoothing = smoothing
        self.pad_index = pad_index
        self.require_ctc_layer = False
        self.takes_logits = True

    def xent(self, logits: Tensor, trg: Tensor) -> Tuple[Tensor, Tensor]:
        return _XentFn.apply(logits, trg, int(self.pad_index), float(max(self.smoothing, 0.0)))

    def forward(self, logits: Tensor, **kwargs) -> Tuple[Tensor]:
        assert "trg" in kwargs
        loss, _ = self.xent(logits, kwargs["trg"])
        return (loss, )

    def __repr__(self):
        return f"{self.__class__.__name__}(criterion=hip_ls_xent, smoothing={self.smoothing})"


class XentCTCLoss(XentLoss):

    def __init__(self, pad_index: int, bos_index: int, smoothing: float = 0.0, zero_infinity: bool = True,
                 ctc_weight: float = 0.3):
        super().__init__(pad_index=pad_index, smoothing=smoothing)
        self.require_ctc_layer = True
        self.bos_index = bos_index
        self.ctc_weight = ctc_weight
        self.zero_infinity = zero_infinity

    def ctc(self, ctc_logits: Tensor, trg: Tensor, input_lengths: Tensor, target_lengths: Tensor, pack=None) -> Tensor:
        return _CtcFn.apply(ctc_logits, trg, input_lengths, target_lengths, int(self.bos_index), bool(self.zero_infinity), pack)

    def forward(self, logits: Tensor, **kwargs) -> Tuple[Tensor, Tensor, Tensor]:
        assert "trg" in kwargs and "trg_length" in kwargs and "src_mask" in kwargs and "ctc_logits" in kwargs
        xent_loss, _ = self.xent(logits, kwargs["trg"])
        in_len = kwargs.get("ctc_input_lengths")
        if in_len is None:
            in_len = kwargs["src_mask"].squeeze(1).sum(dim=1)
        ctc_loss = self.ctc(kwargs["ctc_logits"], kwargs["trg"], in_len, kwargs["trg_length"])
        total_loss = ops.LinComb2Fn.apply(xent_loss, ctc_loss, 1.0 - self.ctc_weight, self.ctc_weight)
        return total_loss, xent_loss, ctc_loss

    def __repr__(self):
        return (f"{self.__class__.__name__}(criterion=hip_ls_xent, smoothing={self.smoothing}, "
                f"ctc=hip_ctc, ctc_weight={self.ctc_weight})")
```

joeys2t_amd/model.py:

```python
from typing import Dict, Optional, Tuple

import torch
from torch import Tensor, nn

from joeys2t_amd import ops
from joeys2t_amd.builders import ConfigurationError
from joeys2t_amd.decoders import Decoder, TransformerDecoder
from joeys2t_amd.embeddings import Embeddings
from joeys2t_amd.encoders import ConformerEncoder, Encoder, TransformerEncoder
from joeys2t_amd.initialization import initialize_model
from joeys2t_amd.loss import XentCTCLoss, XentLoss
from joeys2t_amd.runtime import ParamStore, Runtime, install_runtime


def _mask_row_sums(src_mask: Tensor) -> Tensor:
    known = getattr(src_mask, "js2t_row_sums", None)
    return known if known is not None else src_mask.squeeze(1).sum(dim=1)


PACK_CTC = True


class Model(nn.Module):
    def __init__(self, encoder: Encoder, decoder: Decoder, src_embed: nn.Module, trg_embed: Embeddings, src_vocab,
                 trg_vocab, task: str = "S2T") -> None:
        super().__init__()
        self.src_embed = src_embed
        self.trg_embed = trg_embed
        self.encoder = encoder
        self.decoder = decoder
        self.src_vocab = src_vocab
        self.trg_vocab = trg_vocab
        self.pad_index = trg_vocab.pad_index
        self.bos_index = trg_vocab.bos_index
        self.eos_index = trg_vocab.eos_index
        self.sep_index = trg_vocab.sep_index
        self.unk_index = trg_vocab.unk_index
        self.specials = [trg_vocab.lookup(t) for t in trg_vocab.specials]
        self.lang_tags = [trg_vocab.lookup(t) for t in trg_vocab.lang_tags]
        self._loss_function = None
        self.task = task
        if self.task == "S2T":
            assert isinstance(self.encoder, TransformerEncoder)
            assert isinstance(self.decoder, TransformerDecoder)
        self._rt_obj: Optional[Runtime] = None
        self._cut_tensor = None
        self.overlap_ctc = False

    def finalize(self, device, compute_dtype: torch.dtype = torch.float32, seed: int = 42) -> "Model":
        device = torch.device(device)
        if device.type != "cuda":
            raise ops.Js2tError("Model.finalize: the HIP path needs a cuda (ROCm) device")
        if compute_dtype not in (torch.float32, torch.bfloat16):
            raise ops.Js2tError(f"compute dtype must be float32 or bfloat16, got {compute_dtype}")
        for name, buf in list(self.named_buffers()):
            mod = self
            *path, leaf = name.split(".")
            for part in path:
                mod = getattr(mod, part)
            mod._buffers[leaf] = buf.to(device)
        rt = Runtime(device, compute_dtype)
        rt.store = ParamStore(self, device)
        rt.rng.seed(seed)
        install_runtime(self, rt)
        object.__setattr__(self, "_rt_obj", rt)
        if compute_dtype == torch.bfloat16:
            rt.store.refresh(force=True)
        return self

    def load_state_dict(self, state_dict, strict: bool = True, **kwargs):
        out = super().load_state_dict(state_dict, strict=strict, **kwargs)
        ops.WEIGHT_VERSION += 1
        if self._rt_obj is not None and self._rt_obj.store is not None:
            self._rt_obj.store.mark_dirty()
        return out

    @property
    def runtime(self) -> Runtime:
        if self._rt_obj is None:
            raise ops.Js2tError("Model.finalize(device, compute_dtype) must be called before use")
        return self._rt_obj

    def _prepare_step(self):
        rt = self.runtime
        if rt.compute_dtype == torch.bfloat16:
            rt.store.refresh(force=self.training and rt.store.auto_refresh)

    @property
    def loss_function(self):
        return self._loss_function

    @loss_function.setter
    def loss_function(self, cfg: Tuple):
        loss_type, label_smoothing, ctc_weight = cfg
        if loss_type == "crossentropy-ctc":
            loss_function = XentCTCLoss(pad_index=self.pad_index, bos_index=self.bos_index,
                                        smoothing=label_smoothing, ctc_weight=ctc_weight)
        elif loss_type == "crossentropy":
            loss_function = XentLoss(pad_index=self.pad_index, smoothing=label_smoothing)
            self.decoder.ctc_output_layer = None
        else:
            raise ConfigurationError(f"unknown loss type {loss_type}")
        self._loss_function = loss_function

    _ctc_pack = None

    def forward(self, return_type: str = None, **kwargs) -> Tuple[Tensor, Tensor, Tensor, Tensor]:
        if return_type is None:
            raise ValueError("Please specify return_type: {`loss`, `loss_probs`, `encode`, `decode`, `decode_ctc`}.")
        self._prepare_step()
        if not torch.is_grad_enabled():
            from joeys2t_amd import functional as _Fn
            _Fn.reset_handover()
        if return_type.startswith("loss"):
            assert self.loss_function is not None
            assert "trg" in kwargs and "trg_mask" in kwargs
            lf = self.loss_function
            ctc_loss = None
            if (self.overlap_ctc and return_type == "loss" and lf.require_ctc_layer and kwargs["src"].is_cuda and
                    getattr(self.decoder, "ctc_output_layer", None) is not None):
                out, ctc_out, src_mask, ctc_loss = self._encode_decode_ctc_aside(lf, **kwargs)
            else:
                out, ctc_out, src_mask = self._encode_decode(pack_ctc=(return_type == "loss" and lf.require_ctc_layer), **kwargs)
            xent_loss, n_correct = lf.xent(out, kwargs["trg"])
            ret = [None, None, None, None]
            if lf.require_ctc_layer and isinstance(ctc_out, Tensor):
                if ctc_loss is None:
                    in_len = _mask_row_sums(src_mask)
                    ctc_loss = lf.ctc(ctc_out, kwargs["trg"], in_len, kwargs["trg_length"], pack=self._ctc_pack)
                else:
                    torch.cuda.current_stream().wait_stream(self.runtime.side_stream())
                    ctc_loss.record_stream(torch.cuda.current_stream())
                ret[0] = ops.LinComb2Fn.apply(xent_loss, ctc_loss, 1.0 - lf.ctc_weight, lf.ctc_weight)
                ret[1], ret[2] = xent_loss, ctc_loss
            else:
                ret[0] = xent_loss
            ret[3] = n_correct.long()
            if return_type == "loss_probs":
                ret[1] = ops.log_softmax(out.detach())
                ret[2] = ops.log_softmax(ctc_out.detach()) if isinstance(ctc_out, Tensor) else None
            return tuple(ret)
        if return_type == "encode":
            encoder_output, encoder_hidden, src_mask = self._encode(**kwargs)
            return encoder_output, encoder_hidden, src_mask, None
        if return_type == "decode":
            kwargs.setdefault("compute_ctc", False)
            outputs, hidden, att_probs, att_vectors, _ = self._decode(**kwargs)
            return outputs, hidden, att_probs, att_vectors
        if return_type == "decode_ctc":
            outputs, hidden, att_probs, _, ctc_out = self._decode(**kwargs)
            return outputs, hidden, att_probs, ctc_out
        raise ValueError(f"unknown return_type {return_type}")

    def _ctc_packing(self, encoder_output):
        pk = getattr(self.encoder, "last_pack", None)
        if (PACK_CTC and pk is not None and self.runtime.compute_dtype == torch.bfloat16 and encoder_output.dim() == 3 and
                (pk.B, pk.T) == tuple(encoder_output.shape[:2])):
            return pk
        return None

    def _encode_decode(self, src: Tensor, trg_input: Tensor, src_mask: Tensor, src_length: Tensor, trg_mask: Tensor = None,
                       pack_ctc: bool = False, **kwargs):
        encoder_output, encoder_hidden, src_mask = self._encode(src=src, src_length=src_length, src_mask=src_mask, **kwargs)
        encoder_output = self._mark_cut(encoder_output)
        self._ctc_pack = self._ctc_packing(encoder_output) if pack_ctc else None
        decoder_output, _, _, _, ctc_output = self._decode(encoder_output=encoder_output, encoder_hidden=encoder_hidden,
                                                           src_mask=src_mask, trg_input=trg_input,
                                                           unroll_steps=trg_input.size(1), trg_mask=trg_mask,
                                                           memory_pack=getattr(self.encoder, "last_pack", None),
                                                           ctc_pack=self._ctc_pack, **kwargs)
        return decoder_output, ctc_output, src_mask

    def _encode_decode_ctc_aside(self, lf, src: Tensor, trg_input: Tensor, src_mask: Tensor, src_length: Tensor, trg_mask: Tensor = None,
                                 **kwargs):
        encoder_output, encoder_hidden, src_mask = self._encode(src=src, src_length=src_length, src_mask=src_mask, **kwargs)
        encoder_output = self._mark_cut(encoder_output)
        cur, side = torch.cuda.current_stream(), self.runtime.side_stream()
        side.wait_stream(cur)
        pk = self._ctc_packing(encoder_output)
        with torch.cuda.stream(side):
            if pk is not None:
                from joeys2t_amd.functional import PackRowsFn
                enc_p = PackRowsFn.apply(self.runtime.act_in(encoder_output), pk)
                ctc_out = self.decoder.project(self.decoder.ctc_output_layer, enc_p, self.runtime.compute_dtype)
            else:
                ctc_out = self.decoder.project(self.decoder.ctc_output_layer, encoder_output, self.runtime.compute_dtype)
            in_len = _mask_row_sums(src_mask)
            ctc_loss = lf.ctc(ctc_out, kwargs["trg"], in_len, kwargs["trg_length"], pack=pk)
        for tns in (encoder_output, src_mask, kwargs["trg"], kwargs["trg_length"]):
            tns.record_stream(side)
        decoder_output, _, _, _, _ = self._decode(encoder_output=encoder_output, encoder_hidden=encoder_hidden, src_mask=src_mask,
                                                  trg_input=trg_input, unroll_steps=trg_input.size(1), trg_mask=trg_mask,
                                                  compute_ctc=False, memory_pack=getattr(self.encoder, "last_pack", None), **kwargs)
        return decoder_output, ctc_out, src_mask, ctc_loss

    def _mark_cut(self, encoder_output: Tensor) -> Tensor:
        self._cut_tensor = None
        if torch.is_grad_enabled() and encoder_output.requires_grad:
            from joeys2t_amd.functional import CutFn
            encoder_output = self._cut_tensor = CutFn.apply(encoder_output)
        return encoder_output

    def _encode(self, src: Tensor, src_length: Tensor, src_mask: Tensor, **_kwargs):
        assert _kwargs.get("task", self.task) == self.task, (_kwargs.get("task"), self.task)
        if _kwargs.get("src_prompt_mask", None) is not None and isinstance(self.src_embed, Embeddings):
            _kwargs["src_prompt_mask"] = self.src_embed(_kwargs["src_prompt_mask"])
        return self.encoder(self.src_embed(src), src_length, src_mask, **_kwargs)

    def _decode(self, encoder_output: Tensor, encoder_hidden: Tensor, src_mask: Tensor, trg_input: Tensor,
                unroll_steps: int, decoder_hidden: Tensor = None, att_vector: Tensor = None, trg_mask: Tensor = None,
                **_kwargs):
        if _kwargs.get("trg_prompt_mask", None) is not None:
            assert self.sep_index is not None and self.sep_index in self.specials, "This model doesn't support prompting!"
            _kwargs["trg_prompt_mask"] = self.trg_embed(_kwargs["trg_prompt_mask"])
        return self.decoder(trg_embed=self.trg_embed(trg_input), encoder_output=encoder_output,
                            encoder_hidden=encoder_hidden, src_mask=src_mask, unroll_steps=unroll_steps,
                            hidden=decoder_hidden, prev_att_vector=att_vector, trg_mask=trg_mask, **_kwargs)

    def __repr__(self) -> str:
        return (f"{self.__class__.__name__}(task={self.task},\n\tencoder={self.encoder},\n\tdecoder={self.decoder},\n"
                f"\tsrc_embed={self.src_embed},\n\ttrg_embed={self.trg_embed},\n\tloss_function={self.loss_function})")


class DataParallelWrapper(nn.Module):

    def __init__(self, module: nn.Module):
        super().__init__()
        if not hasattr(module, "module"):
            raise AssertionError("DataParallelWrapper wraps a data-parallel module (something with a `.module`)")
        self.module = module

    @property
    def _model(self) -> nn.Module:
        return self._modules["module"].module

    def __getattr__(self, name):
        wrapper = self._modules["module"]
        for lookup in (lambda: nn.Module.__getattr__(self, name), lambda: getattr(wrapper, name), lambda: getattr(wrapper.module, name)):
            try:
                return lookup()
            except AttributeError:
                continue
        raise AttributeError(f"neither {type(self).__name__}, {type(wrapper).__name__} nor {type(wrapper.module).__name__} has {name!r}")

    def forward(self, *args, **kwargs):
        return self.module(*args, **kwargs)

    def state_dict(self, *args, **kwargs):
        return self._model.state_dict(*args, **kwargs)

    def load_state_dict(self, *args, **kwargs):
        return self._model.load_state_dict(*args, **kwargs)


def build_model(cfg: Dict = None, src_vocab=None, trg_vocab=None) -> Model:
    enc_cfg, dec_cfg = dict(cfg["encoder"]), dict(cfg["decoder"])
    task = "MT" if src_vocab is not None else "S2T"
    trg_pad_index = trg_vocab.pad_index
    if task == "MT":
        src_pad_index = src_vocab.pad_index
        src_embed = Embeddings(**enc_cfg["embeddings"], vocab_size=len(src_vocab), padding_idx=src_pad_index)
        if enc_cfg["embeddings"]["embedding_dim"] != enc_cfg["hidden_size"]:
            raise ConfigurationError("for transformer, emb_size must be the same as hidden_size.")
    else:
        src_pad_index = trg_pad_index
        src_embed = nn.Identity()
    if cfg.get("tied_embeddings", False):
        if task != "MT" or src_vocab != trg_vocab:
            raise ConfigurationError("Embedding cannot be tied since vocabularies differ.")
        trg_embed = src_embed
    else:
# ... 31 lines not shown
```

joeys2t_amd/ops.py:

```python
import ctypes as C
import math
from typing import Optional, Sequence

import torch

from joeys2t_amd._lib import ACT_CODES, BF16, F32, AttnDesc, GemmDesc, Js2tError, check, lib

FP8 = 2
_DT = {torch.float32: F32, torch.bfloat16: BF16, torch.float8_e4m3fn: FP8}


def dt_code(t_or_dtype) -> int:
    dtype = t_or_dtype.dtype if torch.is_tensor(t_or_dtype) else t_or_dtype
    try:
        return _DT[dtype]
    except KeyError:
        raise Js2tError(f"unsupported dtype {dtype}: the HIP path computes in float32 or bfloat16") from None


def _dev(*tensors):
    for t in tensors:
        if t is not None and not t.is_cuda:
            raise Js2tError(
                "joeys2t_amd ops run on the GPU through libjoeys2t_hip.so only; got a CPU tensor "
                "(there is no CPU fallback in the product path)"
            )


def _stream() -> C.c_void_p:
    return C.c_void_p(torch.cuda.current_stream().cuda_stream)


def _p(t: Optional[torch.Tensor]):
    return None if t is None else C.c_void_p(t.data_ptr())


class DropoutRng:

    def __init__(self, device, seed: int = 42):
        self.state = torch.tensor([seed, 0], dtype=torch.int64, device=device)
        self._site = 0

    def begin_step(self):
        self._site = 0

    def advance(self):
        self.state[1:2].add_(1)

    def next_site(self) -> int:
        self._site += 1
        return self._site

    def seed(self, seed: int):
        self.state[0] = seed
        self.state[1] = 0


_rngs = {}


def dropout_rng(device) -> DropoutRng:
    device = torch.device(device)
    key = (device.type, device.index if device.index is not None else torch.cuda.current_device())
    if key not in _rngs:
        _rngs[key] = DropoutRng(device)
    return _rngs[key]


GEMM_TIMER = None


def _takes_p192(d) -> bool:
    if d.trans_a or d.trans_b or d.conv or d.split_k > 1 or d.batch != 1 or d.dtype_c != BF16:
        return False
    if (d.N & 7) or d.N < 128 or (d.K & 7) or d.K < 192 or d.preact or d.beta != 0.0 or d.act not in (0, 1) or (d.residual and d.gate):
        return False
    if d.bias and (d.bias & 15):
        return False
    if ((d.C or 0) & 15) or (d.ldc & 7) or (d.residual and ((d.ldr & 7) or (d.residual & 15))) or (d.gate and ((d.ldg & 7) or (d.gate & 15))):
        return False
    return -(-d.M // 192) * -(-d.N // 128) >= 200


LN_FOLD_WIDTH = 512


def row_partials(M: int, device) -> torch.Tensor:
    return torch.empty((M, LN_FOLD_WIDTH // 64, 2), dtype=torch.float32, device=device)


def gemm(A, B, C_out, *, M, N, K, lda, ldb, ldc, trans_a=False, trans_b=False, batch=1, batch_inner=1,
         a_strides=(0, 0), b_strides=(0, 0), c_strides=(0, 0), a_off=0, b_off=0, c_off=0, alpha=1.0,
         alpha_dev=None, bias=None, act=None, preact=None, dropout_p=0.0, rng: Optional[DropoutRng] = None,
         rng_stream=0, residual=None, ldr=0, res_scale=1.0, gate=None, ldg=0, gate_scale=1.0, beta=0.0,
         conv=None, split_k=1, a_rowsum=None, ln=None, rs_partial=None, fp8_state=None, c8=None, dot=None):
    _dev(A, B, C_out, bias, preact, residual, gate, alpha_dev, a_rowsum, rs_partial)
    if C_out is None and c8 is None:
        raise Js2tError("gemm: no output")
    if A.dtype != B.dtype:
        raise Js2tError(f"gemm: A/B dtype mismatch {A.dtype} vs {B.dtype}")
    c_dtype = torch.bfloat16 if C_out is None else C_out.dtype
    d = GemmDesc()
    d.M, d.N, d.K = int(M), int(N), int(K)
    d.batch, d.batch_inner = int(batch), int(batch_inner)
    d.dtype_ab, d.dtype_c = dt_code(A), dt_code(c_dtype)
    d.trans_a, d.trans_b = int(bool(trans_a)), int(bool(trans_b))
    esa, esc = A.element_size(), (2 if C_out is None else C_out.element_size())
    d.A = A.data_ptr() + a_off * esa
    d.lda, d.a_stride_o, d.a_stride_i = int(lda), int(a_strides[0]), int(a_strides[1])
    d.B = B.data_ptr() + b_off * esa
    d.ldb, d.b_stride_o, d.b_stride_i = int(ldb), int(b_strides[0]), int(b_strides[1])
    d.C = None if C_out is None else C_out.data_ptr() + c_off * esc
    d.ldc, d.c_stride_o, d.c_stride_i = int(ldc), int(c_strides[0]), int(c_strides[1])
    d.alpha = float(alpha)
    d.alpha_dev = None if alpha_dev is None else alpha_dev.data_ptr()
    if bias is not None:
        if bias.dtype != torch.float32:
            raise Js2tError("gemm: bias must be float32")
        d.bias = bias.data_ptr()
    d.act = ACT_CODES[act]
    if preact is not None:
        if preact.dtype != c_dtype:
            raise Js2tError("gemm: preact dtype must match C")
        d.preact = preact.data_ptr() + c_off * esc
    d.dropout_p = float(dropout_p)
    if dropout_p > 0.0:
        if rng is None:
            raise Js2tError("gemm: dropout needs a DropoutRng")
        d.rng_state = rng.state.data_ptr()
        d.rng_stream = int(rng_stream)
    if residual is not None:
        if residual.dtype != c_dtype:
            raise Js2tError("gemm: residual dtype must match C")
        d.residual, d.ldr, d.res_scale = residual.data_ptr(), int(ldr), float(res_scale)
    if gate is not None:
        if gate.dtype != c_dtype:
            raise Js2tError("gemm: gate dtype must match C")
        d.gate, d.ldg, d.gate_scale = gate.data_ptr(), int(ldg), float(gate_scale)
    d.beta = float(beta)
    if conv is not None:
        d.conv = 1
        d.conv_tin, d.conv_tout, d.conv_c, d.conv_stride, d.conv_pad = (int(v) for v in conv)
    d.split_k = int(split_k)
    d.a_rowsum = None if a_rowsum is None else a_rowsum.data_ptr()
    if ln is not None:
        part, eps, mean_out, rstd_out = ln
        _dev(part, mean_out, rstd_out)
        if part.dtype != torch.float32 or part.numel() != M * 16 or not part.is_contiguous():
            raise Js2tError("gemm: ln needs partial sums f32[M, 8, 2]")
        d.ln_partial, d.ln_eps = part.data_ptr(), float(eps)
# ... 27 lines not shown
        if d.dtype_ab == FP8:
            key = "gemm_fp8_p192_kernel<0,0,0>"
        elif d.dtype_ab == BF16:
            fam = "gemm_bf16_kernel" if d.conv else ("gemm_bf16_p192_kernel" if _takes_p192(d) else "gemm_bf16_dma_kernel")
            key = f"{fam}<{int(d.trans_a)},{int(d.trans_b)},{int(d.split_k > 1)}>"
        else:
            key = "gemm_generic_kernel"
        GEMM_TIMER.wrap(key, 2.0 * d.M * d.N * d.K * d.batch, lambda: check(lib().js2t_gemm(C.byref(d), _stream()), "js2t_gemm"),
                        nbytes=d.batch * (esa * (d.M * d.K + d.N * d.K) + esc * d.M * d.N))
    else:
        check(lib().js2t_gemm(C.byref(d), _stream()), "js2t_gemm")
    return C_out


def gemm_grouped(As, Bs, Cs, *, M, N, K, lda, ldb, ldc, split_k=1, beta=0.0, alpha=1.0, a_rowsums=None, sumsq_partial=None):
    n = len(As)
    if not (n == len(Bs) == len(Cs)) or (a_rowsums is not None and len(a_rowsums) != n):
        raise Js2tError("gemm_grouped: list lengths differ")
    if n == 0:
        return
    _dev(*As, *Bs, *Cs, *(a_rowsums or ()))
    if any(t.dtype != torch.bfloat16 for t in (*As, *Bs)) or any(c.dtype != Cs[0].dtype for c in Cs):
        raise Js2tError("gemm_grouped: bf16 operands and one output dtype required")
    d = GemmDesc()
    d.M, d.N, d.K = int(M), int(N), int(K)
    d.batch, d.batch_inner = 1, 1
    d.dtype_ab, d.dtype_c = BF16, dt_code(Cs[0])
    d.trans_a, d.trans_b = 1, 1
    d.lda, d.ldb, d.ldc = int(lda), int(ldb), int(ldc)
    d.alpha, d.beta, d.split_k = float(alpha), float(beta), int(split_k)
    d.res_scale = d.gate_scale = 1.0
    if sumsq_partial is not None:
        _dev(sumsq_partial)
        if sumsq_partial.dtype != torch.float32 or sumsq_partial.numel() < grouped_blocks(d.M, d.N, n):
            raise Js2tError("gemm_grouped: sumsq_partial must be f32[grouped_blocks(M, N, count)]")
        d.sumsq_partial = sumsq_partial.data_ptr()
    arr = C.c_void_p * n
    pa, pb, pc = arr(*[t.data_ptr() for t in As]), arr(*[t.data_ptr() for t in Bs]), arr(*[t.data_ptr() for t in Cs])
    pr = None if a_rowsums is None else arr(*[t.data_ptr() for t in a_rowsums])
    if GEMM_TIMER is not None:
        GEMM_TIMER.wrap(f"js2t_gemm_grouped<split_k {'>' if d.split_k > 1 else '='} 1> (gemm_bf16_wg256_kernel | gemm_bf16_dma_grouped_kernel)",
                        2.0 * d.M * d.N * d.K * n,
                        lambda: check(lib().js2t_gemm_grouped(C.byref(d), n, pa, pb, pc, pr, _stream()), "js2t_gemm_grouped"),
                        nbytes=n * (2 * (d.M * d.K + d.N * d.K) + Cs[0].element_size() * d.M * d.N * (2 if d.beta else 1)))
    else:
        check(lib().js2t_gemm_grouped(C.byref(d), n, pa, pb, pc, pr, _stream()), "js2t_gemm_grouped")


def grouped_blocks(M: int, N: int, count: int) -> int:
    return int(lib().js2t_gemm_grouped_blocks(int(M), int(N), int(count)))


def cast(src: torch.Tensor, dtype: torch.dtype, out: Optional[torch.Tensor] = None) -> torch.Tensor:
    _dev(src, out)
    src = src.contiguous()
    if out is None:
        out = torch.empty(src.shape, dtype=dtype, device=src.device)
    check(lib().js2t_cast(_p(src), dt_code(src), _p(out), dt_code(out), C.c_int64(src.numel()), _stream()), "js2t_cast")
    return out


def axpby(x, a: float, y=None, b: float = 0.0):
    _dev(x, y)
    out = torch.empty_like(x)
    check(lib().js2t_axpby(_p(x), C.c_float(a), _p(y), C.c_float(b), _p(out), C.c_int64(x.numel()), dt_code(x), _stream()),
          "js2t_axpby")
    return out


def transpose_groups(src, dst, table, n_groups: int, total_tiles: int):
    _dev(src, dst, table)
    check(lib().js2t_transpose_groups(_p(src), _p(dst), _p(table), int(n_groups), C.c_int64(total_tiles), _stream()), "js2t_transpose_groups")


def glu_fwd(x: torch.Tensor, T: Optional[int] = None, valid_t: Optional[torch.Tensor] = None) -> torch.Tensor:
    _dev(x, valid_t)
    rows, c2 = x.shape[0], x.shape[1]
    y = torch.empty((rows, c2 // 2), dtype=x.dtype, device=x.device)
    check(lib().js2t_glu_fwd_crop(_p(x), _p(y), C.c_int64(rows), C.c_int64(c2 // 2), C.c_int64(T if valid_t is not None else max(rows, 1)),
                                  _p(valid_t), dt_code(x), _stream()), "js2t_glu_fwd")
    return y


def glu_bwd(x: torch.Tensor, dy: torch.Tensor, T: Optional[int] = None, valid_t: Optional[torch.Tensor] = None) -> torch.Tensor:
    _dev(x, dy, valid_t)
    dx = torch.empty_like(x)
    check(lib().js2t_glu_bwd_crop(_p(x), _p(dy), _p(dx), C.c_int64(x.shape[0]), C.c_int64(x.shape[1] // 2),
                                  C.c_int64(T if valid_t is not None else max(x.shape[0], 1)), _p(valid_t), dt_code(x), _stream()), "js2t_glu_bwd")
    return dx


def add_pe_dropout(x, pe, extra, p, rng: Optional[DropoutRng], site: int):
    _dev(x, pe, extra)
    B, T, D = x.shape
    y = torch.empty_like(x)
    check(lib().js2t_add_pe_dropout(_p(x), _p(pe), _p(extra), _p(y), C.c_int64(B), C.c_int64(T), C.c_int64(D), dt_code(x),
                                    C.c_float(p), _p(rng.state) if p > 0 else None, C.c_uint32(site), _stream()),
          "js2t_add_pe_dropout")
    return y


def dropout_bwd(dy, p, rng: DropoutRng, site: int):
    _dev(dy)
    dy = dy.contiguous()
    cols = dy.shape[-1]
    rows = dy.numel() // cols
    dx = torch.empty_like(dy)
    check(lib().js2t_dropout_bwd(_p(dy), _p(dx), C.c_int64(rows), C.c_int64(cols), dt_code(dy), C.c_float(p),
                                 _p(rng.state), C.c_uint32(site), _stream()), "js2t_dropout_bwd")
    return dx


def act_bwd(dh, z, act: str, scale: float = 1.0):
    _dev(dh, z)
    dz = torch.empty_like(dh)
    check(lib().js2t_act_bwd(_p(dh), _p(z), _p(dz), C.c_int64(dh.numel()), ACT_CODES[act], dt_code(dh), C.c_float(scale),
                             _stream()), "js2t_act_bwd")
    return dz


def embed_fwd(ids, table, scale: float, out_dtype):
    _dev(ids, table)
    ids = ids.contiguous()
    D, V = table.shape[1], table.shape[0]
    out = torch.empty((*ids.shape, D), dtype=out_dtype, device=table.device)
    check(lib().js2t_embed_fwd(_p(ids), _p(table), dt_code(table), _p(out), dt_code(out), C.c_int64(ids.numel()),
                               C.c_int64(D), C.c_int64(V), C.c_float(scale), _stream()), "js2t_embed_fwd")
    return out


def embed_bwd(ids, dout, vocab: int, scale: float, pad_idx: int, out: Optional[torch.Tensor] = None):
    _dev(ids, dout, out)
    ids, dout = ids.contiguous(), dout.contiguous()
    D = dout.shape[-1]
    dtable = out if out is not None else torch.zeros((vocab, D), dtype=torch.float32, device=dout.device)
    check(lib().js2t_embed_bwd(_p(ids), _p(dout), dt_code(dout), _p(dtable), C.c_int64(ids.numel()), C.c_int64(D),
                               C.c_int64(vocab), C.c_float(scale), C.c_int64(-1 if pad_idx is None else pad_idx), _stream()),
          "js2t_embed_bwd")
    return dtable


def colsum(x2d: torch.Tensor, out: Optional[torch.Tensor] = None, accumulate: bool = False) -> torch.Tensor:
    _dev(x2d, out)
    rows, cols = x2d.shape
    if out is None:
        out = torch.empty((cols,), dtype=torch.float32, device=x2d.device)
        accumulate = False
    nparts = lib().js2t_colsum_partial_rows(rows)
    partial = torch.empty((max(nparts, 1) * cols,), dtype=torch.float32, device=x2d.device)
    check(lib().js2t_colsum(_p(x2d), dt_code(x2d), _p(out), _p(partial), C.c_int64(rows), C.c_int64(cols), int(accumulate),
                            _stream()), "js2t_colsum")
    return out


def conv_weight_pack(w: torch.Tensor, dtype) -> torch.Tensor:
    _dev(w)
    cout, cin, k = w.shape
    wp = torch.empty((cout, k * cin), dtype=dtype, device=w.device)
    check(lib().js2t_conv_weight_pack(_p(w.contiguous()), _p(wp), dt_code(wp), C.c_int64(cout), C.c_int64(cin), C.c_int64(k),
                                      _stream()), "js2t_conv_weight_pack")
    return wp


def conv_weight_unpack_grad(dwp_t: torch.Tensor, cout: int, cin: int, k: int, out: Optional[torch.Tensor] = None) -> torch.Tensor:
    _dev(dwp_t, out)
    acc = out is not None
    dw = out if acc else torch.empty((cout, cin, k), dtype=torch.float32, device=dwp_t.device)
    check(lib().js2t_conv_weight_unpack_grad(_p(dwp_t), _p(dw), C.c_int64(cout), C.c_int64(cin), C.c_int64(k), int(acc),
                                             _stream()), "js2t_conv_weight_unpack_grad")
    return dw


def im2col(x3d, K, stride, pad, tout):
    _dev(x3d)
    B, tin, Cc = x3d.shape
    x3d = x3d.contiguous()
    col = torch.empty((B * tout, K * Cc), dtype=x3d.dtype, device=x3d.device)
    check(lib().js2t_im2col(_p(x3d), _p(col), C.c_int64(B), C.c_int64(tin), C.c_int64(tout), C.c_int64(Cc), C.c_int64(K),
                            C.c_int64(stride), C.c_int64(pad), dt_code(x3d), _stream()), "js2t_im2col")
    return col


def col2im(dcol, B, tin, tout, Cc, K, stride, pad):
    _dev(dcol)
    dx = torch.empty((B, tin, Cc), dtype=dcol.dtype, device=dcol.device)
    check(lib().js2t_col2im(_p(dcol), _p(dx), C.c_int64(B), C.c_int64(tin), C.c_int64(tout), C.c_int64(Cc), C.c_int64(K),
                            C.c_int64(stride), C.c_int64(pad), dt_code(dcol), _stream()), "js2t_col2im")
    return dx


def subsample_lengths_mask(lengths: torch.Tensor, t_out: int, kernel_sizes: Sequence[int]):
    _dev(lengths)
    B = lengths.shape[0]
    lengths = lengths.to(torch.int64).contiguous()
    out_len = torch.empty((B,), dtype=torch.int64, device=lengths.device)
    mask = torch.empty((B, 1, t_out), dtype=torch.bool, device=lengths.device)
    ks = (C.c_int32 * len(kernel_sizes))(*kernel_sizes)
    check(lib().js2t_subsample_lengths_mask(_p(lengths), _p(out_len), _p(mask), C.c_int64(B), C.c_int64(t_out), ks,
                                            C.c_int32(len(kernel_sizes)), _stream()), "js2t_subsample_lengths_mask")
    return out_len, mask


def layernorm_fwd(x, gamma, beta, eps: float):
    _dev(x, gamma, beta)
    D = x.shape[-1]
    rows = x.numel() // D
    y = torch.empty_like(x)
    mean = torch.empty((rows,), dtype=torch.float32, device=x.device)
    rstd = torch.empty((rows,), dtype=torch.float32, device=x.device)
    check(lib().js2t_layernorm_fwd(_p(x), _p(gamma), _p(beta), _p(y), _p(mean), _p(rstd), C.c_int64(rows), C.c_int64(D),
                                   C.c_float(eps), dt_code(x), _stream()), "js2t_layernorm_fwd")
    return y, mean, rstd


def layernorm_fwd_fp8(x, gamma, beta, eps: float, state: torch.Tensor, mul: Optional[torch.Tensor] = None, want_y: bool = True):
    _dev(x, gamma, beta, state, mul)
    D = x.shape[-1]
    rows = x.numel() // D
    y = torch.empty_like(x) if want_y else None
    y8 = torch.empty(x.shape, dtype=torch.float8_e4m3fn, device=x.device)
    mean = torch.empty((rows,), dtype=torch.float32, device=x.device)
# ... 160 lines not shown
    if mask is not None:
        if mask.dtype != torch.bool or mask.dim() != 3 or mask.shape[2] != Tk or not mask.is_contiguous():
            raise Js2tError(f"softmax: mask must be contiguous bool [B, 1|Tq, Tk], got {tuple(mask.shape)} {mask.dtype}")
        mask_sq = 0 if mask.shape[1] == 1 else Tk
        if mask.shape[1] not in (1, Tq):
            raise Js2tError(f"softmax: mask query dim {mask.shape[1]} != 1 or {Tq}")
        mask_sb = 0 if mask.shape[0] == 1 else mask.shape[1] * Tk
        if mask.shape[0] not in (1, B):
            raise Js2tError(f"softmax: mask batch dim {mask.shape[0]} != 1 or {B}")
    check(lib().js2t_softmax_fwd(_p(S), _p(mask), _p(P), _p(Pd), C.c_int64(B), C.c_int64(H), C.c_int64(Tq), C.c_int64(Tk),
                                 C.c_int64(ld), C.c_int64(mask_sb), C.c_int64(mask_sq), dt_code(S), C.c_float(p),
                                 _p(rng.state) if p > 0 else None, C.c_uint32(site), _stream()), "js2t_softmax_fwd")
    return P, Pd


def softmax_bwd(P, dPd, Z, Tq, Tk, ld, p, rng: Optional[DropoutRng], site: int):
    _dev(P, dPd)
    dS = torch.empty_like(P)
    check(lib().js2t_softmax_bwd(_p(P), _p(dPd), _p(dS), C.c_int64(Z), C.c_int64(Tq), C.c_int64(Tk), C.c_int64(ld),
                                 dt_code(P), C.c_float(p), _p(rng.state) if p > 0 else None, C.c_uint32(site), _stream()),
          "js2t_softmax_bwd")
    return dS


def attn_head_mean(P, B, H, Tq, Tk, ld):
    _dev(P)
    out = torch.empty((B, Tq, Tk), dtype=torch.float32, device=P.device)
    check(lib().js2t_attn_head_mean(_p(P), _p(out), C.c_int64(B), C.c_int64(H), C.c_int64(Tq), C.c_int64(Tk), C.c_int64(ld),
                                    dt_code(P), _stream()), "js2t_attn_head_mean")
    return out


def rel_bias_add(S, rel_bias, B, H, Tq, Tk, ld):
    _dev(S, rel_bias)
    R = (rel_bias.shape[1] - 1) // 2
    check(lib().js2t_rel_bias_add(_p(S), _p(rel_bias), C.c_int64(B), C.c_int64(H), C.c_int64(Tq), C.c_int64(Tk), C.c_int64(ld),
                                  C.c_int32(R), dt_code(S), _stream()), "js2t_rel_bias_add")
    return S


def rel_bias_grad(dS, d_rel_bias, B, H, Tq, Tk, ld):
    _dev(dS, d_rel_bias)
    R = (d_rel_bias.shape[1] - 1) // 2
    check(lib().js2t_rel_bias_grad(_p(dS), _p(d_rel_bias), C.c_int64(B), C.c_int64(H), C.c_int64(Tq), C.c_int64(Tk), C.c_int64(ld),
                                   C.c_int32(R), dt_code(dS), _stream()), "js2t_rel_bias_grad")


def round_up(x: int, m: int) -> int:
    return (x + m - 1) // m * m


def row_lse(x2d: torch.Tensor, want_argmax: bool = False):
    _dev(x2d)
    rows, V = x2d.shape
    lse = torch.empty((rows,), dtype=torch.float32, device=x2d.device)
    am = torch.empty((rows,), dtype=torch.int64, device=x2d.device) if want_argmax else None
    check(lib().js2t_row_lse(_p(x2d), _p(lse), _p(am), C.c_int64(rows), C.c_int64(V), dt_code(x2d), _stream()), "js2t_row_lse")
    return lse, am


def ctc_collapse(best: torch.Tensor, in_len: torch.Tensor, blank: int, pad: int):
    _dev(best, in_len)
    B, T = best.shape
    best = best.contiguous()
    in_len = in_len.to(torch.int64).contiguous()
    out = torch.empty((B, T), dtype=torch.int64, device=best.device)
    n = torch.empty((B,), dtype=torch.int64, device=best.device)
    check(lib().js2t_ctc_collapse(_p(best), _p(in_len), _p(out), _p(n), C.c_int64(B), C.c_int64(T), C.c_int64(blank), C.c_int64(pad),
                                  _stream()), "js2t_ctc_collapse")
    return out, n


def log_softmax(x: torch.Tensor, out_dtype=torch.float32) -> torch.Tensor:
    _dev(x)
    x = x.contiguous()
    V = x.shape[-1]
    rows = x.numel() // V
    y = torch.empty(x.shape, dtype=out_dtype, device=x.device)
    check(lib().js2t_log_softmax(_p(x), dt_code(x), _p(y), dt_code(y), C.c_int64(rows), C.c_int64(V), _stream()),
          "js2t_log_softmax")
    return y


def train_stats(stats6, total, nll, ctc, n_correct, inv_norm: float, nseqs: float, ntokens: float):
    _dev(stats6, total, nll, ctc, n_correct)
    assert stats6.dtype == torch.float64 and stats6.numel() == 6 and total.dtype == torch.float32
    assert n_correct is None or n_correct.dtype == torch.int64
    norm = torch.empty((), dtype=torch.float32, device=total.device)
    check(lib().js2t_train_stats(_p(stats6), _p(total), _p(nll), _p(ctc), _p(n_correct), C.c_double(inv_norm), C.c_double(nseqs),
                                 C.c_double(ntokens), _p(norm), _stream()), "js2t_train_stats")
    return norm


class LinComb2Fn(torch.autograd.Function):

    @staticmethod
    def forward(ctx, x, y, a: float, b: float):
        ctx.ab = (a, b)
        return axpby(x, a, y, b)

    @staticmethod
    def backward(ctx, g):
        a, b = ctx.ab
        g = g.contiguous()
        return axpby(g, a), axpby(g, b), None, None


def sum_f32(x: torch.Tensor) -> torch.Tensor:
    _dev(x)
    out = torch.empty((), dtype=torch.float32, device=x.device)
    check(lib().js2t_sum_f32(_p(x), C.c_int64(x.numel()), _p(out), _stream()), "js2t_sum_f32")
    return out


def xent_fwd(logits2d, trg1d, pad_idx: int, smoothing: float):
    _dev(logits2d, trg1d)
    rows, V = logits2d.shape
    dev = logits2d.device
    loss_rows = torch.empty((rows,), dtype=torch.float32, device=dev)
    correct_rows = torch.empty((rows,), dtype=torch.float32, device=dev)
    lse = torch.empty((rows,), dtype=torch.float32, device=dev)
    check(lib().js2t_xent_fwd(_p(logits2d), dt_code(logits2d), _p(trg1d), _p(loss_rows), _p(correct_rows), _p(lse),
                              C.c_int64(rows), C.c_int64(V), C.c_int64(pad_idx), C.c_float(smoothing), _stream()),
          "js2t_xent_fwd")
    return loss_rows, correct_rows, lse


def xent_bwd(logits2d, trg1d, lse, g_dev, scale: float, pad_idx: int, smoothing: float, out_dtype=None):
    _dev(logits2d, trg1d, lse, g_dev)
    rows, V = logits2d.shape
    d = torch.empty(logits2d.shape, dtype=out_dtype or logits2d.dtype, device=logits2d.device)
    check(lib().js2t_xent_bwd_as(_p(logits2d), dt_code(logits2d), _p(trg1d), _p(lse), _p(g_dev), C.c_float(scale), _p(d), dt_code(d),
                                 C.c_int64(rows), C.c_int64(V), C.c_int64(pad_idx), C.c_float(smoothing), _stream()),
          "js2t_xent_bwd_as")
    return d


def _ctc_geometry(logits, pack):
    if pack is None:
        B, T, V = logits.shape
        return B, T, V, None
    if logits.dim() != 2 or logits.shape[0] != pack.rows or not logits.is_contiguous():
        raise Js2tError(f"CTC over packed rows: contiguous [{pack.rows}, V] logits expected, got {tuple(logits.shape)}")
    _dev(pack.seg)
    return pack.B, pack.T, logits.shape[1], C.c_void_p(pack.seg.data_ptr())


def ctc_alpha(logits3d, lse, targets, in_len, tgt_len, blank: int, zero_infinity: bool, with_beta: bool = False, pack: "PackedRows" = None):
    _dev(logits3d, lse, targets, in_len, tgt_len)
    B, T, V, roff = _ctc_geometry(logits3d, pack)
    Lmax = targets.shape[1]
    dev = logits3d.device
    alpha = torch.empty((B, T, 2 * Lmax + 1), dtype=torch.float32, device=dev)
    beta = torch.empty_like(alpha) if with_beta else None
    nll = torch.empty((B,), dtype=torch.float32, device=dev)
    loss_rows = torch.empty((B,), dtype=torch.float32, device=dev)
    check(lib().js2t_ctc_alpha(_p(logits3d), dt_code(logits3d), _p(lse), _p(targets), _p(in_len), _p(tgt_len), _p(alpha), _p(beta),
                               _p(nll), _p(loss_rows), C.c_int64(B), C.c_int64(T), C.c_int64(V), C.c_int64(Lmax),
                               C.c_int64(blank), int(zero_infinity), roff, _stream()), "js2t_ctc_alpha")
    return alpha, nll, loss_rows, beta


def ctc_bwd(logits3d, lse, targets, in_len, tgt_len, alpha, nll, g_dev, scale: float, blank: int, zero_infinity: bool, beta=None,
            pack: "PackedRows" = None):
    _dev(logits3d, lse, targets, in_len, tgt_len, alpha, nll, g_dev, beta)
    B, T, V, roff = _ctc_geometry(logits3d, pack)
    Lmax = targets.shape[1]
    ready = beta is not None
    if beta is None:
        beta = torch.empty_like(alpha)
    d = torch.empty_like(logits3d)
    check(lib().js2t_ctc_bwd(_p(logits3d), dt_code(logits3d), _p(lse), _p(targets), _p(in_len), _p(tgt_len), _p(alpha),
                             _p(beta), _p(nll), _p(g_dev), C.c_float(scale), _p(d), C.c_int64(B), C.c_int64(T), C.c_int64(V),
                             C.c_int64(Lmax), C.c_int64(blank), int(zero_infinity), int(ready), roff,
# ... 289 lines not shown
```

joeys2t_amd/training.py:

```python
import os
from typing import Dict, Optional

import torch

from joeys2t_amd import functional, ops
from joeys2t_amd.batch import Batch
from joeys2t_amd.builders import FlatAdamW, WarmupInverseSquareRootScheduler
from joeys2t_amd.helpers_for_ddp import FlatGradReducer, use_ddp
from joeys2t_amd.model import Model
from joeys2t_amd.runtime import WgradQueue


EARLY_EXCHANGE = os.environ.get("JS2T_EARLY_EXCHANGE", "1") != "0"


class TrainStep:
    def __init__(self, model: Model, *, learning_rate: float = 2.0e-3, adam_betas=(0.9, 0.98), weight_decay: float = 0.0,
                 clip_grad_norm: Optional[float] = 10.0, scheduling: Optional[str] = "warmupinversesquareroot",
                 learning_rate_warmup: int = 10000, learning_rate_min: float = 1.0e-6, normalization: str = "batch",
                 batch_multiplier: int = 1, n_gpu: int = 1, n_buckets: int = 4, sync_every_backward: bool = False,
                 defer_wgrads: bool = True, overlap_ctc: bool = False, comm_dtype: Optional[torch.dtype] = None, comm=None,
                 deterministic: bool = False):
        self.model = model
        from joeys2t_amd._lib import Context
# ... 49 lines not shown
        self._grad_seeds: Dict[float, torch.Tensor] = {}
        self.external_lr = False

    def exchange_and_flush(self, plan=None):
        q = self.rt.wgrad_queue
        with self.ctx:
            if plan is None:
                plan = q.take() if q is not None else []
            if self.reducer is None:
                WgradQueue.run(plan)
                return
            self.reducer.exchange_begin(plan)
            WgradQueue.run(plan, self.reducer.entries_done)
            self.reducer.finish()

    def micro_step(self, batch: Batch, sort: bool = True, update: bool = True, overlap: bool = True, flush: bool = True, cut_hook=None):
        with self.ctx, torch.autograd.set_multithreading_enabled(False):
            return self._micro_step(batch, sort, update, overlap, flush, cut_hook)

    def _micro_step(self, batch: Batch, sort: bool, update: bool, overlap: bool, flush: bool, cut_hook):
        model = self.model
        model.train()
        self.rt.rng.begin_step()
        functional.reset_handover()
        if sort:
            batch.sort_by_src_length()
        last = (self.micro + 1) % self.batch_multiplier == 0
        q = self.rt.wgrad_queue
        if q is not None and q.cand is not None:
            q.first = self.micro % self.batch_multiplier == 0
            collect = last and self.reducer is None and self.clip_grad_norm is not None and self.clip_grad_norm > 0
            if collect and self.optimizer.collector is None:
                from joeys2t_amd.builders import SumsqCollector
                self.optimizer.collector = SumsqCollector(self.store.flat_grad, self.store.total)
            q.collector = self.optimizer.collector if collect else None
        exchange = self.reducer is not None and overlap and (last or self.sync_every_backward)
        use_hooks = exchange and self.rt.wgrad_queue is None
        if use_hooks:
            self.reducer.begin(armed=True)
        functional.begin_memory_chain()
        try:
            total, nll, ctc, n_correct = model(return_type="loss", **vars(batch))
        except BaseException:
            functional.end_memory_chain(check=False)
            raise
        inv_norm = self._inv_normalizer(batch)
        seed = self._grad_seeds.get(inv_norm)
        if seed is None:
            seed = torch.full((), inv_norm, dtype=torch.float32, device=total.device)
            if not torch.cuda.is_current_stream_capturing():
                self._grad_seeds[inv_norm] = seed
        enc_out = getattr(model, "_cut_tensor", None)
        model._cut_tensor = None
        can_cut = (EARLY_EXCHANGE and enc_out is not None and enc_out.grad_fn is not None and bool(self.store.late_ranges) and
                   self.rt.wgrad_queue is not None)
        cut = can_cut and (cut_hook is not None or (exchange and not use_hooks and self.reducer.armed_for_exchange()))
        try:
            if cut:
                torch.autograd.backward(total, grad_tensors=seed, inputs=[enc_out] + self._late_leaves)
                functional.end_memory_chain()
                if cut_hook is not None:
                    cut_hook()
                else:
                    plan = self.rt.wgrad_queue.take(final=False)
                    self.reducer.exchange_begin(plan, partial=True)
                    WgradQueue.run(plan, self.reducer.entries_done)
                g_enc, enc_out.grad = enc_out.grad, None
                enc_out.backward(g_enc)
            else:
                total.backward(gradient=seed)
        except BaseException:
            functional.end_memory_chain(check=False)
            raise
        if not cut:
            functional.end_memory_chain()
        if self.rt.grad_copies is not None:
            self.rt.grad_copies.fold()
        if use_hooks:
            self.reducer.finish()
        elif exchange:
            self.exchange_and_flush()
        elif flush:
            self.rt.flush_wgrads()
        with torch.no_grad():
            norm = ops.train_stats(self.stats, total.detach(), None if nll is None else nll.detach(), None if ctc is None else ctc.detach(),
                                   n_correct, inv_norm, batch.nseqs, batch.ntokens or 0)
        self.rt.rng.advance()
        self.micro += 1
        if last and update:
            self.update()
        return norm

    def _inv_normalizer(self, batch: Batch) -> float:
        if self.normalization == "sum":
            return 1.0
        f = 1.0 / {"batch": batch.nseqs, "tokens": batch.ntokens, "none": 1}[self.normalization]
        if self.n_gpu > 1:
            f /= self.n_gpu
        if self.batch_multiplier > 1:
            f /= self.batch_multiplier
        return f

    def update(self):
        with self.ctx:
            self.optimizer.clip_and_step(self.clip_grad_norm, zero_grad=True)
        if torch.cuda.is_current_stream_capturing():
            return
        self.after_update()

    def after_update(self):
        if self.scheduler is not None:
            self.scheduler.step(self.steps)
            if not self.external_lr:
                self.optimizer.lr_dev.fill_(self.optimizer.param_groups[0]["lr"])
        self.steps += 1

    def state_for_checkpoint(self) -> Dict:
        params = list(self.model.parameters())
        stats = dict(zip(["loss", "nll", "ctc", "n_correct", "nseqs", "ntokens"], self.stats.tolist()))
        return {"model_state": self.model.state_dict(), "optimizer_state": self.optimizer.torch_state_dict(params), "scaler_state": None,
                "scheduler_state": None if self.scheduler is None else {"step": self.scheduler._step, "rate": self.scheduler._rate},
                "train_iter_state": getattr(self, "train_iter_state", None) if getattr(self, "train_iter_state", None) is not None
                else torch.Generator().get_state(),
                "stats_state": {"epochs": getattr(self, "epochs", 1), "steps": self.steps, "total_tokens": int(stats.get("ntokens", 0)),
                                "total_correct": int(stats.get("n_correct", 0)), "best_ckpt_score": float("inf"), "best_ckpt_iter": 0}}

    def save_checkpoint(self, path):
        torch.save(self.state_for_checkpoint(), str(path))

    def init_from_checkpoint(self, path, reset_scheduler: bool = False, reset_optimizer: bool = False, map_location="cpu"):
        from joeys2t_amd.helpers import load_checkpoint
        ckpt = load_checkpoint(path, map_location)
        self.model.load_state_dict(ckpt["model_state"])
        if not reset_optimizer:
            self.optimizer.load_torch_state_dict(ckpt["optimizer_state"], list(self.model.parameters()))
        if not reset_scheduler and ckpt.get("scheduler_state") is not None and self.scheduler is not None:
            self.scheduler.load_state_dict(ckpt["scheduler_state"])
            self.optimizer.param_groups[0]["lr"] = ckpt["optimizer_state"]["param_groups"][0]["lr"] if not reset_optimizer else self.scheduler._rate
        self.optimizer.lr_dev.fill_(self.optimizer.param_groups[0]["lr"])
        self.steps = int(ckpt.get("stats_state", {}).get("steps", ckpt.get("steps", 0)))
        self.micro = 0

    def read_stats(self, reset: bool = True) -> Dict[str, float]:
        s = self.stats.clone()
        if use_ddp():
            torch.distributed.all_reduce(s)
        vals = s.tolist()
        if reset:
            self.stats.zero_()
        keys = ["loss", "nll", "ctc", "n_correct", "nseqs", "ntokens"]
        out = dict(zip(keys, vals))
        out["grad_norm"] = float(self.optimizer.norm_clip[0])
        out["lr"] = self.optimizer.param_groups[0]["lr"]
        return out
```

joeys2t_amd/transformer_layers.py:

```python
import math
from typing import Optional, Tuple

import torch
from torch import Tensor, nn

from joeys2t_amd import functional as Fn
from joeys2t_amd.builders import build_activation
from joeys2t_amd.runtime import runtime_of


def _rng(rt, x: Tensor):
    if rt.device is None:
        from joeys2t_amd.ops import dropout_rng
        return dropout_rng(x.device)
    return rt.rng


def _layer_norm(rt, ln: nn.LayerNorm, x: Tensor) -> Tensor:
    sk = rt.sinks({"g": [ln.weight], "b": [ln.bias]})
    return Fn.LayerNormFn.apply(x, ln.weight, ln.bias, None if sk is None else (sk["g"], sk["b"], sk.get("_copies")), rt.grads_ready)


class MultiHeadedAttention(nn.Module):

# ... 75 lines not shown
        if pack is not None:
            if kind != "self":
                raise NotImplementedError("packed rows: self-attention blocks only")
            wts["pack"] = pack
        if mem_pack is not None:
            if memory_kv is None:
                raise NotImplementedError("packed encoder states: grouped K | V projections only")
            wts["mem_pack"] = mem_pack
        if memory_kv is not None:
            wts["kv_off"] = int(memory_kv[1])
            wts["notify_skip"] = {id(k_.weight), id(v_.weight), id(k_.bias), id(v_.bias)}
        rng = _rng(rt, x) if cfg.any_dropout else None
        if mask is not None and not mask.is_contiguous():
            mask = mask.contiguous()
        out = Fn.ResidualBlockFn.apply(cfg, rng, x, memory, mask, wts, *params)
        return out if kind == "cross" else (out, None)

    def forward(self, k: Tensor, v: Tensor, q: Tensor, mask: Optional[Tensor] = None,
                return_weights: Optional[bool] = None):
        if k is not v:
            raise NotImplementedError("MultiHeadedAttention: k and v must be the same tensor on the HIP path")
        memory = None if q is k else k
        out, att = self.run_block(q, memory, mask, ln=None, ln_mode="none", alpha=0.0, out_dropout=0.0,
                                  need_weights=bool(return_weights))
        if return_weights and memory is None:
            raise NotImplementedError("attention weights are only exported for cross-attention (decoders.py:606-615)")
        return out, att


class PositionwiseFeedForward(nn.Module):

    def __init__(self, input_size: int, ff_size: int, dropout: float = 0.1, alpha: float = 1.0,
                 layer_norm: str = "post", activation: str = "relu") -> None:
        super().__init__()
        activation_fnc = build_activation(activation=activation)
        self.layer_norm = nn.LayerNorm(input_size, eps=1e-6)
        self.pwff_layer = nn.Sequential(
            nn.Linear(input_size, ff_size),
            activation_fnc(),
            nn.Dropout(dropout),
            nn.Linear(ff_size, input_size),
            nn.Dropout(dropout),
        )
        self.alpha = alpha
        self._layer_norm_position = layer_norm
        self._activation = activation
        assert self._layer_norm_position in {"pre", "post"}

    def forward(self, x: Tensor) -> Tensor:
        rt = runtime_of(self)
        x = rt.act_in(x)
        l1, l2 = self.pwff_layer[0], self.pwff_layer[3]
        p = self.pwff_layer[2].p
        cfg = Fn.BlockCfg(kind="ffn", alpha=self.alpha, ln_mode=self._layer_norm_position, act=self._activation,
                          training=self.training, attn_dropout=p, out_dropout=p)
        wts = {"w1": rt.weight([l1.weight]), "b1": rt.bias([l1.bias]), "w2": rt.weight([l2.weight]),
               "b2": rt.bias([l2.bias]), "ln_g": self.layer_norm.weight.data, "ln_b": self.layer_norm.bias.data,
               "w1_t": rt.weight_t([l1.weight]), "w2_t": rt.weight_t([l2.weight]),
               "fold": rt.ln_fold([l1.weight], [l1.bias], self.layer_norm)
               if (self._layer_norm_position == "pre" and self._activation == "relu" and Fn.LN_FOLD) else None,
               "emit_stats": self._layer_norm_position == "pre" and rt.store is not None and rt.compute_dtype == torch.bfloat16,
               "sink": rt.sinks({"w1": [l1.weight], "b1": [l1.bias], "w2": [l2.weight], "b2": [l2.bias],
                                 "ln_g": [self.layer_norm.weight], "ln_b": [self.layer_norm.bias]}),
               "notify": rt.grads_ready}
        rng = _rng(rt, x) if cfg.any_dropout else None
        return Fn.ResidualBlockFn.apply(cfg, rng, x, None, None, wts, l1.weight, l1.bias, l2.weight, l2.bias,
                                        self.layer_norm.weight, self.layer_norm.bias)


class PositionalEncoding(nn.Module):

    def __init__(self, size: int = 0, max_len: int = 5000) -> None:
        if size % 2 != 0:
            raise ValueError(f"Cannot use sin/cos positional encoding with odd dim (got dim={size})")
        super().__init__()
        position = torch.arange(0, max_len).unsqueeze(1).float()
        div_term = torch.exp(torch.arange(0, size, 2, dtype=torch.float) * -(math.log(10000.0) / size))
        pe = torch.zeros(max_len, size)
        pe[:, 0::2] = torch.sin(position * div_term)
        pe[:, 1::2] = torch.cos(position * div_term)
        self.register_buffer("pe", pe.unsqueeze(0))
        self.dim = size

    def forward(self, emb: Tensor, extra: Optional[Tensor] = None, dropout: float = 0.0, training: bool = False) -> Tensor:
        rt = runtime_of(self)
        emb = rt.act_in(emb)
        if emb.size(1) > self.pe.size(1):
            raise ValueError(f"sequence length {emb.size(1)} exceeds positional table {self.pe.size(1)}")
        p = dropout if training else 0.0
        rng = _rng(rt, emb) if p > 0 else None
        if extra is not None:
            extra = rt.act_in(extra)
        return Fn.AddPeDropoutFn.apply(emb, self.pe[0], extra, p, rng)


class TransformerEncoderLayer(nn.Module):

    def __init__(self, size: int = 0, ff_size: int = 0, num_heads: int = 0, dropout: float = 0.1, alpha: float = 1.0,
                 layer_norm: str = "post", activation: str = "relu") -> None:
        super().__init__()
        self.layer_norm = nn.LayerNorm(size, eps=1e-6)
        self.src_src_att = MultiHeadedAttention(num_heads, size, dropout=dropout)
        self.feed_forward = PositionwiseFeedForward(size, ff_size=ff_size, dropout=dropout, alpha=alpha,
                                                    layer_norm=layer_norm, activation=activation)
        self.dropout = nn.Dropout(dropout)
        self.size = size
        self.alpha = alpha
        self._layer_norm_position = layer_norm
        assert self._layer_norm_position in {"pre", "post"}

    def forward(self, x: Tensor, mask: Tensor, pack=None) -> Tensor:
        h, _ = self.src_src_att.run_block(x, None, mask, ln=self.layer_norm, ln_mode=self._layer_norm_position,
                                          alpha=self.alpha, out_dropout=self.dropout.p, pack=pack)
        return self.feed_forward(h)


class TransformerDecoderLayer(nn.Module):

    def __init__(self, size: int = 0, ff_size: int = 0, num_heads: int = 0, dropout: float = 0.1, alpha: float = 1.0,
                 layer_norm: str = "post", activation: str = "relu") -> None:
        super().__init__()
        self.size = size
        self.trg_trg_att = MultiHeadedAttention(num_heads, size, dropout=dropout)
        self.src_trg_att = MultiHeadedAttention(num_heads, size, dropout=dropout)
        self.feed_forward = PositionwiseFeedForward(size, ff_size=ff_size, dropout=dropout, alpha=alpha,
                                                    layer_norm=layer_norm, activation=activation)
        self.x_layer_norm = nn.LayerNorm(size, eps=1e-6)
        self.dec_layer_norm = nn.LayerNorm(size, eps=1e-6)
        self.dropout = nn.Dropout(dropout)
        self.alpha = alpha
        self._layer_norm_position = layer_norm
        assert self._layer_norm_position in {"pre", "post"}

    def forward(self, x: Tensor, memory: Tensor, src_mask: Tensor, trg_mask: Tensor, return_attention: bool = False,
                memory_kv: Optional[Tuple[Tensor, int]] = None, **kwargs):
        h1, _ = self.trg_trg_att.run_block(x, None, trg_mask, ln=self.x_layer_norm, ln_mode=self._layer_norm_position,
                                           alpha=self.alpha, out_dropout=self.dropout.p)
        h2, att = self.src_trg_att.run_block(h1, memory, src_mask, ln=self.dec_layer_norm,
                                             ln_mode=self._layer_norm_position, alpha=self.alpha,
                                             out_dropout=self.dropout.p, need_weights=return_attention, memory_kv=memory_kv,
                                             mem_pack=kwargs.get("mem_pack"))
        out = self.feed_forward(h2)
        return out, (att if return_attention else None)


class ConvolutionModule(nn.Module):

    def __init__(self, hidden_size: int, channels: int, depthwise_kernel_size: int, dropout: float):
        super().__init__()
        assert (depthwise_kernel_size - 1) % 2 == 0, "kernel_size should be a odd number for 'SAME' padding"
        self.layer_norm = nn.LayerNorm(hidden_size, eps=1e-6)
        self.pointwise_conv1 = nn.Conv1d(hidden_size, 2 * channels, kernel_size=1, stride=1, padding=0)
        self.glu = nn.GLU(dim=1)
        self.depthwise_conv = nn.Conv1d(channels, channels, depthwise_kernel_size, stride=1,
                                        padding=(depthwise_kernel_size - 1) // 2, groups=channels)
        self.batch_norm = nn.BatchNorm1d(channels)
        self.swish = nn.Hardswish()
        self.pointwise_conv2 = nn.Conv1d(channels, hidden_size, kernel_size=1, stride=1, padding=0)
        self.dropout = nn.Dropout(dropout)

    def forward(self, x: Tensor) -> Tensor:
        rt = runtime_of(self)
        x = rt.act_in(x)
        x = _layer_norm(rt, self.layer_norm, x)
        bn = self.batch_norm
        p = self.dropout.p
        rng = _rng(rt, x) if (self.training and p > 0) else None
        if self.training:
            bn.num_batches_tracked += 1
        lp = rt.store is not None and rt.compute_dtype != torch.float32
        return Fn.ConvModuleFn.apply(x, self.pointwise_conv1.weight, self.pointwise_conv1.bias, self.depthwise_conv.weight,
                                     self.depthwise_conv.bias, bn.weight, bn.bias, bn.running_mean, bn.running_var,
                                     self.pointwise_conv2.weight, self.pointwise_conv2.bias, p, rng, self.training, rt.compute_dtype,
                                     rt.weight([self.pointwise_conv1.weight]) if lp else None,
                                     rt.weight([self.pointwise_conv2.weight]) if lp else None,
                                     rt.sinks({"w1": [self.pointwise_conv1.weight], "b1": [self.pointwise_conv1.bias],
# ... 37 lines not shown
```

Before: 4.257 million frames/s.

## Fuse dropout backward and loss/stat glue into neighboring kernels

Folds the dropout mask regeneration into the GLU and embedding backward kernels, so no separate dropout-backward pass runs over those activations. Adds a single-kernel loss reduction (xent, accuracy and CTC sums plus weighted total) with a matching tiny backward kernel. Moves the RNG-offset advance and the optimizer step counter into the train-stats kernel, removing several small launches and elementwise passes per step. The fused paths are on by default behind an environment flag, and they add coupling between the RNG state layout and the stats kernel.

```diff
diff --git a/include/joeys2t_hip.h b/include/joeys2t_hip.h
--- a/include/joeys2t_hip.h
+++ b/include/joeys2t_hip.h
@@ -89,6 +89,8 @@
 int js2t_glu_fwd_crop(const void* x, void* y, int64_t rows, int64_t C, int64_t T, const int64_t* valid_t, int dt, js2t_stream stream);
 int js2t_glu_bwd_crop(const void* x, const void* dy, void* dx, int64_t rows, int64_t C, int64_t T, const int64_t* valid_t, int dt,
                       js2t_stream stream);
+int js2t_glu_bwd_mask(const void* x, const void* dy, void* dx, int64_t rows, int64_t C, int64_t T, const int64_t* valid_t, int dt,
+                      float p, const uint64_t* rng_state, uint32_t rng_stream, js2t_stream stream);
 
 int js2t_transpose_groups(const void* src, void* dst, const int64_t* table, int32_t n_groups, int64_t total_tiles, js2t_stream stream);
 
@@ -106,6 +108,8 @@
                    int64_t n_ids, int64_t D, int64_t vocab, float scale, js2t_stream stream);
 int js2t_embed_bwd(const int64_t* ids, const void* dout, int dout_dt, float* dtable, int64_t n_ids,
                    int64_t D, int64_t vocab, float scale, int64_t pad_idx, js2t_stream stream);
+int js2t_embed_bwd_mask(const int64_t* ids, const void* dout, int dout_dt, float* dtable, int64_t n_ids, int64_t D, int64_t vocab,
+                        float scale, int64_t pad_idx, float p, const uint64_t* rng_state, uint32_t rng_stream, js2t_stream stream);
 
 int64_t js2t_colsum_partial_rows(int64_t rows);
 int js2t_colsum(const void* x, int dt, float* out, float* partial, int64_t rows, int64_t cols, int accumulate,
@@ -181,7 +185,16 @@
 int js2t_train_stats(double* stats6, const float* total, const float* nll, const float* ctc, const int64_t* n_correct,
                      double inv_norm, double nseqs, double ntokens, float* norm_out, js2t_stream stream);
 
+int js2t_train_stats_count(double* stats6, const float* total, const float* nll, const float* ctc, const int64_t* n_correct,
+                           double inv_norm, double nseqs, double ntokens, float* norm_out, int64_t* counter_a, int64_t* counter_b,
+                           js2t_stream stream);
+
 int js2t_sum_f32(const float* x, int64_t n, float* out, js2t_stream stream);
+
+int js2t_loss_finish(const float* xent_rows, const float* correct_rows, int64_t n_rows, const float* ctc_rows, int64_t n_ctc,
+                     float wa, float wb, float* out3, int64_t* n_correct, js2t_stream stream);
+int js2t_loss_finish_bwd(const float* g_total, const float* g_nll, const float* g_ctc, float wa, float wb, float* out2,
+                         js2t_stream stream);
 
 int js2t_ctc_alpha(const void* logits, int dt, const float* lse, const int64_t* targets, const int64_t* in_len,
                    const int64_t* tgt_len, float* alpha, float* beta, float* nll, float* loss_rows, int64_t B, int64_t T,
diff --git a/joeys2t_amd/builders.py b/joeys2t_amd/builders.py
--- a/joeys2t_amd/builders.py
+++ b/joeys2t_amd/builders.py
@@ -129,7 +129,7 @@
         self.collector: Optional[SumsqCollector] = None
 
 
-    def clip_and_step(self, max_norm: Optional[float], grad_scale: float = 1.0, zero_grad: bool = True):
+    def clip_and_step(self, max_norm: Optional[float], grad_scale: float = 1.0, zero_grad: bool = True, step_counted: bool = False):
         from joeys2t_amd import ops
         from joeys2t_amd._lib import check, lib
         st, g = self.store, self.param_groups[0]
@@ -147,7 +147,8 @@
         lp = st.flat_lp
         lr_dev = step_dev = None
         if self.device_schedule:
-            self.step_dev.add_(1)
+            if not step_counted:
+                self.step_dev.add_(1)
             lr_dev, step_dev = self.lr_dev, self.step_dev
         plan = self._fused_plan()
         if plan is not None:
diff --git a/joeys2t_amd/csrc/elementwise.hip b/joeys2t_amd/csrc/elementwise.hip
--- a/joeys2t_amd/csrc/elementwise.hip
+++ b/joeys2t_amd/csrc/elementwise.hip
@@ -66,13 +66,26 @@
   }
 }
 template <typename T>
+__device__ __forceinline__ float round_as(float v) {
+  T t;
+  io<T>::st(&t, v);
+  return io<T>::ld(&t);
+}
+template <typename T>
 __global__ void glu_bwd_kernel(const T* __restrict__ x, const T* __restrict__ dy, T* __restrict__ dx, int64_t rows,
-                               int64_t C, int64_t T_, const int64_t* __restrict__ valid_t) {
+                               int64_t C, int64_t T_, const int64_t* __restrict__ valid_t, float p, const uint64_t* rng, uint32_t stream) {
   const int64_t total = rows * C, vt = valid_t ? *valid_t : T_;
+  const float sc = p > 0.f ? 1.f / (1.f - p) : 1.f;
+  const uint32_t dkey = p > 0.f ? dropout_key(rng, stream) : 0u;
   for (int64_t i = blockIdx.x * (int64_t)blockDim.x + threadIdx.x; i < total; i += (int64_t)gridDim.x * blockDim.x) {
     const int64_t r = i / C, c = i - r * C;
     const float a = io<T>::ld(x + r * 2 * C + c), b = io<T>::ld(x + r * 2 * C + C + c);
-    const float g = (r % T_) < vt ? io<T>::ld(dy + i) : 0.f;
+    float g = io<T>::ld(dy + i);
+    if (p > 0.f) {
+      const uint32_t keep = dropout_keep4_key(dkey, (uint32_t)r, (uint32_t)(c >> 2), p);
+      g = ((keep >> (c & 3)) & 1u) ? round_as<T>(g * sc) : 0.f;
+    }
+    if ((r % T_) >= vt) g = 0.f;
     const float s = 1.f / (1.f + __expf(-b));
     io<T>::st(dx + r * 2 * C + c, g * s);
     io<T>::st(dx + r * 2 * C + C + c, g * a * s * (1.f - s));
@@ -147,22 +160,34 @@
   }
 }
 template <typename T>
+__device__ __forceinline__ float masked_grad(const T* g, uint32_t dkey, int64_t r, int64_t c, float p, float sc) {
+  const float v = io<T>::ld(g);
+  if (p <= 0.f) return v;
+  const uint32_t keep = dropout_keep4_key(dkey, (uint32_t)r, (uint32_t)(c >> 2), p);
+  return ((keep >> (c & 3)) & 1u) ? round_as<T>(v * sc) : 0.f;
+}
+template <typename T>
 __global__ void embed_bwd_kernel(const int64_t* __restrict__ ids, const T* __restrict__ dout, float* __restrict__ dtable,
-                                 int64_t n_ids, int64_t D, int64_t vocab, float scale, int64_t pad_idx) {
+                                 int64_t n_ids, int64_t D, int64_t vocab, float scale, int64_t pad_idx, float p, const uint64_t* rng,
+                                 uint32_t stream) {
   const int64_t total = n_ids * D;
+  const float sc = p > 0.f ? 1.f / (1.f - p) : 1.f;
+  const uint32_t dkey = p > 0.f ? dropout_key(rng, stream) : 0u;
   for (int64_t i = blockIdx.x * (int64_t)blockDim.x + threadIdx.x; i < total; i += (int64_t)gridDim.x * blockDim.x) {
     const int64_t r = i / D, c = i - r * D;
     const int64_t id = ids[r];
     if (id < 0 || id >= vocab || id == pad_idx) continue;
-    atomicAdd(dtable + id * D + c, scale * io<T>::ld(dout + i));
+    atomicAdd(dtable + id * D + c, scale * masked_grad<T>(dout + i, dkey, r, c, p, sc));
   }
 }
 
 template <typename T>
 __global__ __launch_bounds__(256) void embed_bwd_ordered_kernel(const int64_t* __restrict__ ids, const T* __restrict__ dout,
                                                                 float* __restrict__ dtable, int64_t n_ids, int64_t D, int64_t vocab,
-                                                                float scale, int64_t pad_idx) {
+                                                                float scale, int64_t pad_idx, float p, const uint64_t* rng, uint32_t stream) {
   __shared__ int earlier;
+  const float sc = p > 0.f ? 1.f / (1.f - p) : 1.f;
+  const uint32_t dkey = p > 0.f ? dropout_key(rng, stream) : 0u;
   const int64_t r = blockIdx.x, id = ids[r];
   if (id < 0 || id >= vocab || id == pad_idx) return;
   if (threadIdx.x == 0) earlier = 0;
@@ -174,7 +199,7 @@
   for (int64_t c = threadIdx.x; c < D; c += blockDim.x) {
     float acc = dtable[id * D + c];
     for (int64_t q = r; q < n_ids; ++q)
-      if (ids[q] == id) acc += scale * io<T>::ld(dout + q * D + c);
+      if (ids[q] == id) acc += scale * masked_grad<T>(dout + q * D + c, dkey, q, c, p, sc);
     dtable[id * D + c] = acc;
   }
 }
@@ -426,14 +451,20 @@
 extern "C" int js2t_glu_fwd(const void* x, void* y, int64_t rows, int64_t C, int dt, js2t_stream stream) {
   return js2t_glu_fwd_crop(x, y, rows, C, rows > 0 ? rows : 1, nullptr, dt, stream);
 }
+extern "C" int js2t_glu_bwd_mask(const void* x, const void* dy, void* dx, int64_t rows, int64_t C, int64_t T_, const int64_t* valid_t,
+                                 int dt, float p, const uint64_t* rng_state, uint32_t rng_stream, js2t_stream stream) {
+  if (rows * C == 0) return JS2T_OK;
+  JS2T_CHECK(x && dy && dx && rows > 0 && C > 0 && T_ > 0 && rows % T_ == 0, "glu_bwd: bad arguments");
+  JS2T_CHECK(p >= 0.f && p < 1.f && (p == 0.f || rng_state), "glu_bwd: bad dropout arguments");
+  DISPATCH_DT(dt, T, hipLaunchKernelGGL((glu_bwd_kernel<T>), dim3(ew_grid(rows * C)), dim3(EW_THREADS), 0,
+                                        (hipStream_t)stream, (const T*)x, (const T*)dy, (T*)dx, rows, C, T_, valid_t, p, rng_state,
+                                        rng_stream));
+  JS2T_LAUNCH_CHECK();
+  return JS2T_OK;
+}
 extern "C" int js2t_glu_bwd_crop(const void* x, const void* dy, void* dx, int64_t rows, int64_t C, int64_t T_, const int64_t* valid_t,
                                  int dt, js2t_stream stream) {
-  if (rows * C == 0) return JS2T_OK;
-  JS2T_CHECK(x && dy && dx && rows > 0 && C > 0 && T_ > 0 && rows % T_ == 0, "glu_bwd: bad arguments");
-  DISPATCH_DT(dt, T, hipLaunchKernelGGL((glu_bwd_kernel<T>), dim3(ew_grid(rows * C)), dim3(EW_THREADS), 0,
-                                        (hipStream_t)stream, (const T*)x, (const T*)dy, (T*)dx, rows, C, T_, valid_t));
-  JS2T_LAUNCH_CHECK();
-  return JS2T_OK;
+  return js2t_glu_bwd_mask(x, dy, dx, rows, C, T_, valid_t, dt, 0.f, nullptr, 0u, stream);
 }
 extern "C" int js2t_glu_bwd(const void* x, const void* dy, void* dx, int64_t rows, int64_t C, int dt, js2t_stream stream) {
   return js2t_glu_bwd_crop(x, dy, dx, rows, C, rows > 0 ? rows : 1, nullptr, dt, stream);
@@ -483,20 +514,27 @@
   JS2T_LAUNCH_CHECK();
   return JS2T_OK;
 }
+extern "C" int js2t_embed_bwd_mask(const int64_t* ids, const void* dout, int dout_dt, float* dtable, int64_t n_ids, int64_t D,
+                                   int64_t vocab, float scale, int64_t pad_idx, float p, const uint64_t* rng_state, uint32_t rng_stream,
+                                   js2t_stream stream) {
+  if (n_ids * D == 0) return JS2T_OK;
+  JS2T_CHECK(ids && dout && dtable, "embed_bwd: null pointer");
+  JS2T_CHECK(p >= 0.f && p < 1.f && (p == 0.f || rng_state), "embed_bwd: bad dropout arguments");
+  if (g_js2t_deterministic) {
+    DISPATCH_DT(dout_dt, T, hipLaunchKernelGGL((embed_bwd_ordered_kernel<T>), dim3((unsigned)n_ids), dim3(256), 0, (hipStream_t)stream, ids,
+                                               (const T*)dout, dtable, n_ids, D, vocab, scale, pad_idx, p, rng_state, rng_stream));
+    JS2T_LAUNCH_CHECK();
+    return JS2T_OK;
+  }
+  DISPATCH_DT(dout_dt, T, hipLaunchKernelGGL((embed_bwd_kernel<T>), dim3(ew_grid(n_ids * D)), dim3(EW_THREADS), 0,
+                                             (hipStream_t)stream, ids, (const T*)dout, dtable, n_ids, D, vocab, scale, pad_idx, p, rng_state,
+                                             rng_stream));
+  JS2T_LAUNCH_CHECK();
+  return JS2T_OK;
+}
 extern "C" int js2t_embed_bwd(const int64_t* ids, const void* dout, int dout_dt, float* dtable, int64_t n_ids, int64_t D,
                               int64_t vocab, float scale, int64_t pad_idx, js2t_stream stream) {
-  if (n_ids * D == 0) return JS2T_OK;
-  JS2T_CHECK(ids && dout && dtable, "embed_bwd: null pointer");
-  if (g_js2t_deterministic) {
-    DISPATCH_DT(dout_dt, T, hipLaunchKernelGGL((embed_bwd_ordered_kernel<T>), dim3((unsigned)n_ids), dim3(256), 0, (hipStream_t)stream, ids,
-                                               (const T*)dout, dtable, n_ids, D, vocab, scale, pad_idx));
-    JS2T_LAUNCH_CHECK();
-    return JS2T_OK;
-  }
-  DISPATCH_DT(dout_dt, T, hipLaunchKernelGGL((embed_bwd_kernel<T>), dim3(ew_grid(n_ids * D)), dim3(EW_THREADS), 0,
-                                             (hipStream_t)stream, ids, (const T*)dout, dtable, n_ids, D, vocab, scale, pad_idx));
-  JS2T_LAUNCH_CHECK();
-  return JS2T_OK;
+  return js2t_embed_bwd_mask(ids, dout, dout_dt, dtable, n_ids, D, vocab, scale, pad_idx, 0.f, nullptr, 0u, stream);
 }
 
 extern "C" int64_t js2t_colsum_partial_rows(int64_t rows) { return (rows + CS_ROWS_PER_BLOCK - 1) / CS_ROWS_PER_BLOCK; }
diff --git a/joeys2t_amd/csrc/loss.hip b/joeys2t_amd/csrc/loss.hip
--- a/joeys2t_amd/csrc/loss.hip
+++ b/joeys2t_amd/csrc/loss.hip
@@ -291,6 +291,42 @@
   for (int64_t i = threadIdx.x; i < n; i += 1024) s += x[i];
   s = block_sum(s, red);
   if (threadIdx.x == 0) out[0] = s;
+}
+
+__global__ __launch_bounds__(1024) void loss_finish_kernel(const float* __restrict__ xent_rows, const float* __restrict__ correct_rows,
+                                                           int64_t n_rows, const float* __restrict__ ctc_rows, int64_t n_ctc, float wa,
+                                                           float wb, float* __restrict__ out3, int64_t* __restrict__ n_correct) {
+  __shared__ float red[16];
+  float s = 0.f;
+  for (int64_t i = threadIdx.x; i < n_rows; i += 1024) s += xent_rows[i];
+  const float nll = block_sum(s, red);
+  s = 0.f;
+  for (int64_t i = threadIdx.x; i < n_rows; i += 1024) s += correct_rows[i];
+  const float ok = block_sum(s, red);
+  float ctc = 0.f;
+  if (ctc_rows) {
+    s = 0.f;
+    for (int64_t i = threadIdx.x; i < n_ctc; i += 1024) s += ctc_rows[i];
+    ctc = block_sum(s, red);
+  }
+  if (threadIdx.x == 0) {
+    const float v = ctc_rows ? __fmaf_rn(wb, ctc, __fmul_rn(wa, nll)) : nll;
+    out3[0] = v;
+    out3[1] = nll;
+    out3[2] = ctc;
+    n_correct[0] = (int64_t)ok;
+  }
+}
+__global__ void loss_finish_bwd_kernel(const float* __restrict__ g_total, const float* __restrict__ g_nll, const float* __restrict__ g_ctc,
+                                       float wa, float wb, float* __restrict__ out2) {
+#pragma clang fp contract(off)
+  if (threadIdx.x != 0 || blockIdx.x != 0) return;
+  const float g = g_total ? g_total[0] : 0.f;
+  float a = wa * g, b = wb * g;
+  if (g_nll) a += g_nll[0];
+  if (g_ctc) b += g_ctc[0];
+  out2[0] = a;
+  out2[1] = b;
 }
 
 constexpr int CTC_THREADS = 256;
@@ -729,7 +765,8 @@
 }
 
 __global__ void train_stats_kernel(double* __restrict__ stats, const float* total, const float* nll, const float* ctc,
-                                   const int64_t* n_correct, double inv_norm, double nseqs, double ntokens, float* norm_out) {
+                                   const int64_t* n_correct, double inv_norm, double nseqs, double ntokens, float* norm_out,
+                                   int64_t* counter_a, int64_t* counter_b) {
   if (threadIdx.x != 0 || blockIdx.x != 0) return;
   const double t = (double)total[0] * inv_norm;
   stats[0] += t;
@@ -739,12 +776,35 @@
   stats[4] += nseqs;
   stats[5] += ntokens;
   if (norm_out) norm_out[0] = (float)t;
+  if (counter_a) counter_a[0] += 1;
+  if (counter_b) counter_b[0] += 1;
+}
+extern "C" int js2t_train_stats_count(double* stats6, const float* total, const float* nll, const float* ctc, const int64_t* n_correct,
+                                      double inv_norm, double nseqs, double ntokens, float* norm_out, int64_t* counter_a,
+                                      int64_t* counter_b, js2t_stream stream) {
+  JS2T_CHECK(stats6 && total, "train_stats: null pointer");
+  hipLaunchKernelGGL(train_stats_kernel, dim3(1), dim3(64), 0, (hipStream_t)stream, stats6, total, nll, ctc, n_correct, inv_norm, nseqs,
+                     ntokens, norm_out, counter_a, counter_b);
+  JS2T_LAUNCH_CHECK();
+  return JS2T_OK;
 }
 extern "C" int js2t_train_stats(double* stats6, const float* total, const float* nll, const float* ctc, const int64_t* n_correct,
                                 double inv_norm, double nseqs, double ntokens, float* norm_out, js2t_stream stream) {
-  JS2T_CHECK(stats6 && total, "train_stats: null pointer");
-  hipLaunchKernelGGL(train_stats_kernel, dim3(1), dim3(64), 0, (hipStream_t)stream, stats6, total, nll, ctc, n_correct, inv_norm, nseqs,
-                     ntokens, norm_out);
+  return js2t_train_stats_count(stats6, total, nll, ctc, n_correct, inv_norm, nseqs, ntokens, norm_out, nullptr, nullptr, stream);
+}
+
+extern "C" int js2t_loss_finish(const float* xent_rows, const float* correct_rows, int64_t n_rows, const float* ctc_rows, int64_t n_ctc,
+                                float wa, float wb, float* out3, int64_t* n_correct, js2t_stream stream) {
+  JS2T_CHECK(xent_rows && correct_rows && out3 && n_correct && n_rows >= 0 && n_ctc >= 0, "loss_finish: bad arguments");
+  hipLaunchKernelGGL(loss_finish_kernel, dim3(1), dim3(1024), 0, (hipStream_t)stream, xent_rows, correct_rows, n_rows, ctc_rows, n_ctc, wa,
+                     wb, out3, n_correct);
+  JS2T_LAUNCH_CHECK();
+  return JS2T_OK;
+}
+extern "C" int js2t_loss_finish_bwd(const float* g_total, const float* g_nll, const float* g_ctc, float wa, float wb, float* out2,
+                                    js2t_stream stream) {
+  JS2T_CHECK(out2 && (g_total || g_nll || g_ctc), "loss_finish_bwd: bad arguments");
+  hipLaunchKernelGGL(loss_finish_bwd_kernel, dim3(1), dim3(64), 0, (hipStream_t)stream, g_total, g_nll, g_ctc, wa, wb, out2);
   JS2T_LAUNCH_CHECK();
   return JS2T_OK;
 }
diff --git a/joeys2t_amd/decoders.py b/joeys2t_amd/decoders.py
--- a/joeys2t_amd/decoders.py
+++ b/joeys2t_amd/decoders.py
@@ -83,7 +83,7 @@
         assert trg_mask is not None, "trg_mask required for Transformer"
         rt = runtime_of(self)
         x = self.pe(trg_embed, extra=kwargs.get("trg_prompt_mask", None), dropout=self.emb_dropout.p,
-                    training=self.training)
+                    training=self.training, sole_consumer=True)
         L = trg_embed.size(1)
         trg_mask = (trg_mask & subsequent_mask(L, device=trg_mask.device)).contiguous()
         last_layer = len(self.layers) - 1
diff --git a/joeys2t_amd/encoders.py b/joeys2t_amd/encoders.py
--- a/joeys2t_amd/encoders.py
+++ b/joeys2t_amd/encoders.py
@@ -95,7 +95,7 @@
         if mask is None:
             mask = lengths_to_padding_mask(src_length, src_embed.size(1)).unsqueeze(1)
         x = self.pe(src_embed, extra=kwargs.get("src_prompt_mask", None), dropout=self.emb_dropout.p,
-                    training=self.training)
+                    training=self.training, sole_consumer=self.subsample)
         pack = self._packing(x, mask, kwargs)
         self.last_pack = pack
         if pack is not None:
diff --git a/joeys2t_amd/functional.py b/joeys2t_amd/functional.py
--- a/joeys2t_amd/functional.py
+++ b/joeys2t_amd/functional.py
@@ -780,8 +780,19 @@
 
     @staticmethod
     def backward(ctx, dy):
+        if getattr(ctx, "mask_deferred", False):
+            return dy, None, None, None, None
         dx = ops.dropout_bwd(dy, ctx.p, ctx.rng, ctx.site) if ctx.p > 0 else dy
         return dx, None, (dx if ctx.has_extra else None), None, None
+
+
+def defer_dropout_bwd(y: torch.Tensor, x: torch.Tensor) -> None:
+    node, src = y.grad_fn, x.grad_fn
+    if (not ops.FUSED_GLUE or node is None or src is None or not getattr(src, "takes_mask", False) or not getattr(node, "p", 0) > 0 or
+            node.has_extra or y.shape != x.shape):
+        return
+    src.load_mask = (node.p, node.rng, node.site)
+    node.mask_deferred = True
 
 
 class EmbedFn(torch.autograd.Function):
@@ -790,11 +801,12 @@
     def forward(ctx, ids, table, scale, pad_idx, out_dtype, sink=None, notify=None):
         ctx.ids, ctx.scale, ctx.pad_idx, ctx.vocab = ids, scale, pad_idx, table.shape[0]
         ctx.sink, ctx.notify, ctx.leaf = sink, notify, table
+        ctx.takes_mask = True
         return ops.embed_fwd(ids, table, scale, out_dtype)
 
     @staticmethod
     def backward(ctx, dout):
-        dt = ops.embed_bwd(ctx.ids, dout, ctx.vocab, ctx.scale, ctx.pad_idx, out=ctx.sink)
+        dt = ops.embed_bwd(ctx.ids, dout, ctx.vocab, ctx.scale, ctx.pad_idx, out=ctx.sink, mask=getattr(ctx, "load_mask", None))
         if ctx.sink is not None:
             if ctx.notify is not None:
                 ctx.notify((ctx.leaf, ))
@@ -908,6 +920,7 @@
         y = ops.glu_fwd(pre, Tout, valid_t)
         ctx.x, ctx.wp, ctx.pre, ctx.conv, ctx.col = (x if col is None else None), wp, pre, conv, col
         ctx.dims = (B, T, Cin, Cout, K, Tout)
+        ctx.takes_mask = True
         return y.view(B, Tout, Cout // 2)
 
     @staticmethod
@@ -918,7 +931,7 @@
         dy2 = dy.reshape(M, Cout // 2)
         if not dy2.is_contiguous():
             dy2 = dy2.contiguous()
-        dpre = ops.glu_bwd(pre, dy2, Tout, ctx.valid_t)
+        dpre = ops.glu_bwd(pre, dy2, Tout, ctx.valid_t, mask=getattr(ctx, "load_mask", None))
         sink = ctx.sink or {}
         db = ops.colsum(dpre, out=sink.get("b"), accumulate=True) if sink else ops.colsum(dpre)
         sk = wgrad_split(K * Cin, Cout, M)
diff --git a/joeys2t_amd/loss.py b/joeys2t_amd/loss.py
--- a/joeys2t_amd/loss.py
+++ b/joeys2t_amd/loss.py
@@ -9,9 +9,17 @@
 _NAN = {}
 
 
+def _uniform(g: Tensor) -> Tensor:
+    if g.numel() == 1:
+        return g.reshape(())
+    if all(st == 0 for st in g.stride()):
+        return g.as_strided((), (), g.storage_offset())
+    raise ops.Js2tError("the per-row losses take one gradient for all rows (loss.LossTailFn); got a tensor that varies by row")
+
+
 class _XentFn(torch.autograd.Function):
     @staticmethod
-    def forward(ctx, logits, trg, pad_index, smoothing):
+    def forward(ctx, logits, trg, pad_index, smoothing, rows=False):
         V = logits.shape[-1]
         l2 = logits.reshape(-1, V)
         if not l2.is_contiguous():
@@ -20,6 +28,10 @@
         loss_rows, correct_rows, lse = ops.xent_fwd(l2, t1, pad_index, smoothing)
         ctx.l2, ctx.t1, ctx.lse = l2, t1, lse
         ctx.pad_index, ctx.smoothing, ctx.shape = pad_index, smoothing, logits.shape
+        ctx.rows = rows
+        if rows:
+            ctx.mark_non_differentiable(correct_rows)
+            return loss_rows, correct_rows
         loss = ops.sum_f32(loss_rows)
         n_correct = ops.sum_f32(correct_rows)
         ctx.mark_non_differentiable(n_correct)
@@ -27,7 +39,7 @@
 
     @staticmethod
     def backward(ctx, g, _g2):
-        g = g.contiguous().float()
+        g = (_uniform(g) if ctx.rows else g).contiguous().float()
         from joeys2t_amd import functional as Fn
         want = Fn.LOGIT_GRAD_DTYPE.pop(ctx.l2.data_ptr(), None)
         if want is not None and want != ctx.l2.dtype and ctx.l2.dtype == torch.float32:
@@ -39,16 +51,16 @@
             if len(Fn.LOGIT_GRAD_READY) > 16:
                 Fn.LOGIT_GRAD_READY.clear()
             Fn.LOGIT_GRAD_READY[ctx.l2.data_ptr()] = (d, ph)
-            return ph, None, None, None
+            return ph, None, None, None, None
         d = ops.xent_bwd(ctx.l2, ctx.t1, ctx.lse, g, 1.0, ctx.pad_index, ctx.smoothing)
-        return d.view(ctx.shape), None, None, None
+        return d.view(ctx.shape), None, None, None, None
 
 
 class _CtcFn(torch.autograd.Function):
 
     @staticmethod
-    def forward(ctx, logits, targets, in_len, tgt_len, blank, zero_infinity, pack=None):
-        ctx.pack, ctx.shape = pack, tuple(logits.shape)
+    def forward(ctx, logits, targets, in_len, tgt_len, blank, zero_infinity, pack=None, rows=False):
+        ctx.pack, ctx.shape, ctx.rows = pack, tuple(logits.shape), rows
         if pack is None:
             B, T, V = logits.shape
             l3 = logits.contiguous()
@@ -66,14 +78,39 @@
                                                     with_beta=logits.requires_grad, pack=pack)
         ctx.saved = (l3, lse, targets, in_len, tgt_len, alpha, nll, beta)
         ctx.blank, ctx.zero_infinity = blank, zero_infinity
-        return ops.sum_f32(loss_rows)
+        return loss_rows if rows else ops.sum_f32(loss_rows)
 
     @staticmethod
     def backward(ctx, g):
         l3, lse, targets, in_len, tgt_len, alpha, nll, beta = ctx.saved
-        g = g.contiguous().float()
+        g = (_uniform(g) if ctx.rows else g).contiguous().float()
         d = ops.ctc_bwd(l3, lse, targets, in_len, tgt_len, alpha, nll, g, 1.0, ctx.blank, ctx.zero_infinity, beta=beta, pack=ctx.pack)
-        return d.view(ctx.shape), None, None, None, None, None, None
+        return d.view(ctx.shape), None, None, None, None, None, None, None
+
+
+class LossTailFn(torch.autograd.Function):
+
+    @staticmethod
+    def forward(ctx, xent_rows, correct_rows, ctc_rows, wa: float, wb: float):
+        out3, n_correct = ops.loss_finish(xent_rows, correct_rows, ctc_rows, wa, wb)
+        ctx.w = (wa, wb)
+        ctx.n = (xent_rows.shape, None if ctc_rows is None else ctc_rows.shape)
+        ctx.set_materialize_grads(False)
+        ctx.mark_non_differentiable(n_correct)
+        if ctc_rows is None:
+            return out3[0], out3[1], None, n_correct
+        return out3[0], out3[1], out3[2], n_correct
+
+    @staticmethod
+    def backward(ctx, g_total, g_nll, g_ctc, _g4):
+        (wa, wb), (nx, nc) = ctx.w, ctx.n
+        if nc is None and (g_total is None or g_nll is None):
+            g = g_total if g_nll is None else g_nll
+            return (None if g is None else g.expand(nx)), None, None, None, None
+        if g_total is None and g_nll is None and g_ctc is None:
+            return None, None, None, None, None
+        out2 = ops.loss_finish_bwd(g_total, g_nll, g_ctc if nc is not None else None, 1.0 if nc is None else wa, wb)
+        return out2[0].expand(nx), None, (None if nc is None else out2[1].expand(nc)), None, None
 
 
 class XentLoss(nn.Module):
@@ -85,8 +122,8 @@
         self.require_ctc_layer = False
         self.takes_logits = True
 
-    def xent(self, logits: Tensor, trg: Tensor) -> Tuple[Tensor, Tensor]:
-        return _XentFn.apply(logits, trg, int(self.pad_index), float(max(self.smoothing, 0.0)))
+    def xent(self, logits: Tensor, trg: Tensor, rows: bool = False) -> Tuple[Tensor, Tensor]:
+        return _XentFn.apply(logits, trg, int(self.pad_index), float(max(self.smoothing, 0.0)), rows)
 
     def forward(self, logits: Tensor, **kwargs) -> Tuple[Tensor]:
         assert "trg" in kwargs
@@ -107,8 +144,8 @@
         self.ctc_weight = ctc_weight
         self.zero_infinity = zero_infinity
 
-    def ctc(self, ctc_logits: Tensor, trg: Tensor, input_lengths: Tensor, target_lengths: Tensor, pack=None) -> Tensor:
-        return _CtcFn.apply(ctc_logits, trg, input_lengths, target_lengths, int(self.bos_index), bool(self.zero_infinity), pack)
+    def ctc(self, ctc_logits: Tensor, trg: Tensor, input_lengths: Tensor, target_lengths: Tensor, pack=None, rows: bool = False) -> Tensor:
+        return _CtcFn.apply(ctc_logits, trg, input_lengths, target_lengths, int(self.bos_index), bool(self.zero_infinity), pack, rows)
 
     def forward(self, logits: Tensor, **kwargs) -> Tuple[Tensor, Tensor, Tensor]:
         assert "trg" in kwargs and "trg_length" in kwargs and "src_mask" in kwargs and "ctc_logits" in kwargs
diff --git a/joeys2t_amd/model.py b/joeys2t_amd/model.py
--- a/joeys2t_amd/model.py
+++ b/joeys2t_amd/model.py
@@ -9,7 +9,7 @@
 from joeys2t_amd.embeddings import Embeddings
 from joeys2t_amd.encoders import ConformerEncoder, Encoder, TransformerEncoder
 from joeys2t_amd.initialization import initialize_model
-from joeys2t_amd.loss import XentCTCLoss, XentLoss
+from joeys2t_amd.loss import LossTailFn, XentCTCLoss, XentLoss
 from joeys2t_amd.runtime import ParamStore, Runtime, install_runtime
 
 
@@ -117,25 +117,32 @@
             assert "trg" in kwargs and "trg_mask" in kwargs
             lf = self.loss_function
             ctc_loss = None
+            tail = ops.FUSED_GLUE
             if (self.overlap_ctc and return_type == "loss" and lf.require_ctc_layer and kwargs["src"].is_cuda and
                     getattr(self.decoder, "ctc_output_layer", None) is not None):
-                out, ctc_out, src_mask, ctc_loss = self._encode_decode_ctc_aside(lf, **kwargs)
+                out, ctc_out, src_mask, ctc_loss = self._encode_decode_ctc_aside(lf, loss_rows=tail, **kwargs)
             else:
                 out, ctc_out, src_mask = self._encode_decode(pack_ctc=(return_type == "loss" and lf.require_ctc_layer), **kwargs)
-            xent_loss, n_correct = lf.xent(out, kwargs["trg"])
+            xent_loss, n_correct = lf.xent(out, kwargs["trg"], rows=tail)
             ret = [None, None, None, None]
             if lf.require_ctc_layer and isinstance(ctc_out, Tensor):
                 if ctc_loss is None:
                     in_len = _mask_row_sums(src_mask)
-                    ctc_loss = lf.ctc(ctc_out, kwargs["trg"], in_len, kwargs["trg_length"], pack=self._ctc_pack)
+                    ctc_loss = lf.ctc(ctc_out, kwargs["trg"], in_len, kwargs["trg_length"], pack=self._ctc_pack, rows=tail)
                 else:
                     torch.cuda.current_stream().wait_stream(self.runtime.side_stream())
                     ctc_loss.record_stream(torch.cuda.current_stream())
-                ret[0] = ops.LinComb2Fn.apply(xent_loss, ctc_loss, 1.0 - lf.ctc_weight, lf.ctc_weight)
-                ret[1], ret[2] = xent_loss, ctc_loss
+                if tail:
+                    ret[0], ret[1], ret[2], ret[3] = LossTailFn.apply(xent_loss, n_correct, ctc_loss, 1.0 - lf.ctc_weight, lf.ctc_weight)
+                else:
+                    ret[0] = ops.LinComb2Fn.apply(xent_loss, ctc_loss, 1.0 - lf.ctc_weight, lf.ctc_weight)
+                    ret[1], ret[2] = xent_loss, ctc_loss
+            elif tail:
+                ret[0], _, _, ret[3] = LossTailFn.apply(xent_loss, n_correct, None, 1.0, 0.0)
             else:
                 ret[0] = xent_loss
-            ret[3] = n_correct.long()
+            if not tail:
+                ret[3] = n_correct.long()
             if return_type == "loss_probs":
                 ret[1] = ops.log_softmax(out.detach())
                 ret[2] = ops.log_softmax(ctc_out.detach()) if isinstance(ctc_out, Tensor) else None
@@ -172,7 +179,7 @@
         return decoder_output, ctc_output, src_mask
 
     def _encode_decode_ctc_aside(self, lf, src: Tensor, trg_input: Tensor, src_mask: Tensor, src_length: Tensor, trg_mask: Tensor = None,
-                                 **kwargs):
+                                 loss_rows: bool = False, **kwargs):
         encoder_output, encoder_hidden, src_mask = self._encode(src=src, src_length=src_length, src_mask=src_mask, **kwargs)
         encoder_output = self._mark_cut(encoder_output)
         cur, side = torch.cuda.current_stream(), self.runtime.side_stream()
@@ -186,7 +193,7 @@
             else:
                 ctc_out = self.decoder.project(self.decoder.ctc_output_layer, encoder_output, self.runtime.compute_dtype)
             in_len = _mask_row_sums(src_mask)
-            ctc_loss = lf.ctc(ctc_out, kwargs["trg"], in_len, kwargs["trg_length"], pack=pk)
+            ctc_loss = lf.ctc(ctc_out, kwargs["trg"], in_len, kwargs["trg_length"], pack=pk, rows=loss_rows)
         for tns in (encoder_output, src_mask, kwargs["trg"], kwargs["trg_length"]):
             tns.record_stream(side)
         decoder_output, _, _, _, _ = self._decode(encoder_output=encoder_output, encoder_hidden=encoder_hidden, src_mask=src_mask,
diff --git a/joeys2t_amd/ops.py b/joeys2t_amd/ops.py
--- a/joeys2t_amd/ops.py
+++ b/joeys2t_amd/ops.py
@@ -66,6 +66,10 @@
         _rngs[key] = DropoutRng(device)
     return _rngs[key]
 
+
+import os as _os
+
+FUSED_GLUE = _os.environ.get("JS2T_FUSED_GLUE", "1") != "0"
 
 GEMM_TIMER = None
 
@@ -259,11 +263,13 @@
     return y
 
 
-def glu_bwd(x: torch.Tensor, dy: torch.Tensor, T: Optional[int] = None, valid_t: Optional[torch.Tensor] = None) -> torch.Tensor:
+def glu_bwd(x: torch.Tensor, dy: torch.Tensor, T: Optional[int] = None, valid_t: Optional[torch.Tensor] = None, mask=None) -> torch.Tensor:
     _dev(x, dy, valid_t)
     dx = torch.empty_like(x)
-    check(lib().js2t_glu_bwd_crop(_p(x), _p(dy), _p(dx), C.c_int64(x.shape[0]), C.c_int64(x.shape[1] // 2),
-                                  C.c_int64(T if valid_t is not None else max(x.shape[0], 1)), _p(valid_t), dt_code(x), _stream()), "js2t_glu_bwd")
+    p, rng, site = mask if mask is not None else (0.0, None, 0)
+    check(lib().js2t_glu_bwd_mask(_p(x), _p(dy), _p(dx), C.c_int64(x.shape[0]), C.c_int64(x.shape[1] // 2),
+                                  C.c_int64(T if valid_t is not None else max(x.shape[0], 1)), _p(valid_t), dt_code(x), C.c_float(p),
+                                  _p(rng.state) if p > 0 else None, C.c_uint32(site), _stream()), "js2t_glu_bwd")
     return dx
 
 
@@ -306,14 +312,15 @@
     return out
 
 
-def embed_bwd(ids, dout, vocab: int, scale: float, pad_idx: int, out: Optional[torch.Tensor] = None):
+def embed_bwd(ids, dout, vocab: int, scale: float, pad_idx: int, out: Optional[torch.Tensor] = None, mask=None):
     _dev(ids, dout, out)
     ids, dout = ids.contiguous(), dout.contiguous()
     D = dout.shape[-1]
     dtable = out if out is not None else torch.zeros((vocab, D), dtype=torch.float32, device=dout.device)
-    check(lib().js2t_embed_bwd(_p(ids), _p(dout), dt_code(dout), _p(dtable), C.c_int64(ids.numel()), C.c_int64(D),
-                               C.c_int64(vocab), C.c_float(scale), C.c_int64(-1 if pad_idx is None else pad_idx), _stream()),
-          "js2t_embed_bwd")
+    p, rng, site = mask if mask is not None else (0.0, None, 0)
+    check(lib().js2t_embed_bwd_mask(_p(ids), _p(dout), dt_code(dout), _p(dtable), C.c_int64(ids.numel()), C.c_int64(D),
+                                    C.c_int64(vocab), C.c_float(scale), C.c_int64(-1 if pad_idx is None else pad_idx), C.c_float(p),
+                                    _p(rng.state) if p > 0 else None, C.c_uint32(site), _stream()), "js2t_embed_bwd")
     return dtable
 
 
@@ -640,14 +647,38 @@
     return y
 
 
-def train_stats(stats6, total, nll, ctc, n_correct, inv_norm: float, nseqs: float, ntokens: float):
-    _dev(stats6, total, nll, ctc, n_correct)
+def train_stats(stats6, total, nll, ctc, n_correct, inv_norm: float, nseqs: float, ntokens: float, counters=()):
+    _dev(stats6, total, nll, ctc, n_correct, *counters)
     assert stats6.dtype == torch.float64 and stats6.numel() == 6 and total.dtype == torch.float32
     assert n_correct is None or n_correct.dtype == torch.int64
+    assert len(counters) <= 2 and all(c.dtype == torch.int64 and c.numel() == 1 for c in counters)
+    ca, cb = (tuple(counters) + (None, None))[:2]
     norm = torch.empty((), dtype=torch.float32, device=total.device)
-    check(lib().js2t_train_stats(_p(stats6), _p(total), _p(nll), _p(ctc), _p(n_correct), C.c_double(inv_norm), C.c_double(nseqs),
-                                 C.c_double(ntokens), _p(norm), _stream()), "js2t_train_stats")
+    check(lib().js2t_train_stats_count(_p(stats6), _p(total), _p(nll), _p(ctc), _p(n_correct), C.c_double(inv_norm), C.c_double(nseqs),
+                                       C.c_double(ntokens), _p(norm), _p(ca), _p(cb), _stream()), "js2t_train_stats")
     return norm
+
+
+def loss_finish(xent_rows, correct_rows, ctc_rows, wa: float, wb: float):
+    _dev(xent_rows, correct_rows, ctc_rows)
+    rows = [None if t is None else t.contiguous() for t in (xent_rows, correct_rows, ctc_rows)]
+    assert all(t is None or t.dtype == torch.float32 for t in rows) and rows[0].numel() == rows[1].numel()
+    out3 = torch.empty((3, ), dtype=torch.float32, device=xent_rows.device)
+    n_correct = torch.empty((), dtype=torch.int64, device=xent_rows.device)
+    check(lib().js2t_loss_finish(_p(rows[0]), _p(rows[1]), C.c_int64(rows[0].numel()), _p(rows[2]),
+                                 C.c_int64(0 if rows[2] is None else rows[2].numel()), C.c_float(wa), C.c_float(wb), _p(out3), _p(n_correct),
+                                 _stream()), "js2t_loss_finish")
+    return out3, n_correct
+
+
+def loss_finish_bwd(g_total, g_nll, g_ctc, wa: float, wb: float):
+    gs = [None if g is None else g.contiguous().float() for g in (g_total, g_nll, g_ctc)]
+    _dev(*gs)
+    dev = next(g.device for g in gs if g is not None)
+    out2 = torch.empty((2, ), dtype=torch.float32, device=dev)
+    check(lib().js2t_loss_finish_bwd(_p(gs[0]), _p(gs[1]), _p(gs[2]), C.c_float(wa), C.c_float(wb), _p(out2), _stream()),
+          "js2t_loss_finish_bwd")
+    return out2
 
 
 class LinComb2Fn(torch.autograd.Function):
diff --git a/joeys2t_amd/training.py b/joeys2t_amd/training.py
--- a/joeys2t_amd/training.py
+++ b/joeys2t_amd/training.py
@@ -155,13 +155,16 @@
             self.exchange_and_flush()
         elif flush:
             self.rt.flush_wgrads()
+        count_step = ops.FUSED_GLUE and last and update and self.optimizer.device_schedule
+        counters = ([self.rt.rng.state[1:2]] + ([self.optimizer.step_dev] if count_step else [])) if ops.FUSED_GLUE else []
         with torch.no_grad():
             norm = ops.train_stats(self.stats, total.detach(), None if nll is None else nll.detach(), None if ctc is None else ctc.detach(),
-                                   n_correct, inv_norm, batch.nseqs, batch.ntokens or 0)
-        self.rt.rng.advance()
+                                   n_correct, inv_norm, batch.nseqs, batch.ntokens or 0, counters=counters)
+        if not ops.FUSED_GLUE:
+            self.rt.rng.advance()
         self.micro += 1
         if last and update:
-            self.update()
+            self.update(step_counted=count_step)
         return norm
 
     def _inv_normalizer(self, batch: Batch) -> float:
@@ -174,9 +177,9 @@
             f /= self.batch_multiplier
         return f
 
-    def update(self):
+    def update(self, step_counted: bool = False):
         with self.ctx:
-            self.optimizer.clip_and_step(self.clip_grad_norm, zero_grad=True)
+            self.optimizer.clip_and_step(self.clip_grad_norm, zero_grad=True, step_counted=step_counted)
         if torch.cuda.is_current_stream_capturing():
             return
         self.after_update()
diff --git a/joeys2t_amd/transformer_layers.py b/joeys2t_amd/transformer_layers.py
--- a/joeys2t_amd/transformer_layers.py
+++ b/joeys2t_amd/transformer_layers.py
@@ -181,7 +181,8 @@
         self.register_buffer("pe", pe.unsqueeze(0))
         self.dim = size
 
-    def forward(self, emb: Tensor, extra: Optional[Tensor] = None, dropout: float = 0.0, training: bool = False) -> Tensor:
+    def forward(self, emb: Tensor, extra: Optional[Tensor] = None, dropout: float = 0.0, training: bool = False,
+                sole_consumer: bool = False) -> Tensor:
         rt = runtime_of(self)
         emb = rt.act_in(emb)
         if emb.size(1) > self.pe.size(1):
@@ -190,7 +191,10 @@
         rng = _rng(rt, emb) if p > 0 else None
         if extra is not None:
             extra = rt.act_in(extra)
-        return Fn.AddPeDropoutFn.apply(emb, self.pe[0], extra, p, rng)
+        y = Fn.AddPeDropoutFn.apply(emb, self.pe[0], extra, p, rng)
+        if sole_consumer and p > 0 and extra is None:
+            Fn.defer_dropout_bwd(y, emb)
+        return y
 
 
 class TransformerEncoderLayer(nn.Module):
```

Result: no change. 4.272 million frames/s, median of 6 (+0.3%).
